# MiniMax-AI/VTP

Hardware: AMD Instinct MI355X
Metric: images/sec/node VTP-B f16d64 256x256 train step (higher is better)
Workload: dtype bf16

## Files before the change

include/vtp_hip.h:

```cpp
#ifndef VTP_HIP_H
#define VTP_HIP_H
#ifdef __cplusplus
extern "C" {
#endif

#define VTP_ABI_VERSION 1

int vtp_abi_version(void);
const char* vtp_last_error(void);

enum { VTP_EPI_BF16 = 0, VTP_EPI_F32 = 1, VTP_EPI_SWIGLU = 2, VTP_EPI_GELU = 3, VTP_EPI_F32_ATOMIC = 4, VTP_EPI_F32_SLAB = 5,
       VTP_EPI_QUICK_GELU = 8 };
int vtp_gemm_splits(int K, int splits);
int vtp_gemm_tn_splits(int M, int N, int K);
int vtp_gemm_tn(const void* A, int lda, const void* B, int ldb, void* C, int ldc, int ldc2, const float* resid, int M, int N,
                int K, int epilogue, int a_grp, int a_pre, int b_grp, int b_pre, int c_grp, int c_pre, int splits,
                float* a_colsum, void* stream);
int vtp_gemm_tn_grouped(const void* probs, int nprob, int ntiles, int K, int splits, void* part, void* ticket, void* stream);
int vtp_gemm_tn_grouped_items(const void* probs, int nprob, int ntiles, int K, const void* items, int nitems, int slots, void* part,
                              void* ticket, void* stream);
int vtp_set_gemm_tuning(int force_cfg, int xcd_swizzle);
int vtp_set_gemm_dynamic(int on);
int vtp_gemm_debug(void* timing, int grid_limit, int delay_ticks);
int vtp_cu_thief(int nwg, int ticks, void* out, void* stream);
int vtp_attn_debug(void* timing, int lds_pad, int waves_per_wg, int stagger_ticks);
int vtp_gemm_nt_config(int M, int N, int K, int epilogue);
int vtp_gemm_nt(const void* A, int lda, const void* B, int ldb, void* C, int ldc, void* C2, int ldc2,
                const float* bias, const float* gamma, const float* resid, int M, int N, int K, int epilogue,
                int a_grp, int a_pre, int c_grp, int c_pre, int splits, float alpha, void* stream);

int vtp_gemm_qkv_rope(const void* A, int lda, const void* W, int ldb, const float* bias, void* C, int ldc, int M, int N, int K,
                      const int* rope_pos, const void* rope_sin, const void* rope_cos, int rope_cols, void* stream);

int vtp_gather_image_rows(const float* src, const int* img_idx, float* dst, void* dst_bf16, int n_img, long N, int D, float scale,
                          void* stream);
int vtp_scatter_image_rows(const float* src, const int* img_idx, float* dst, int n_img, long N, int D, float alpha, int accumulate,
                           void* stream);
int vtp_layerscale_wgrad(const float* G, const float* W, const float* bias, const float* colsum, const float* gamma, float* dW,
                         float* db, float* dgamma, int N, int K, void* stream);
int vtp_scaled_transpose(const float* W, const float* gamma, void* dstT, int N, int K, void* stream);
int vtp_qk_norm_fwd(const void* qkv, const float* wq, const float* wk, void* out, float* inv, long M, int D, float eps, void* stream);
int vtp_qk_norm_bwd(void* dqkv, const void* qkv, const float* inv, const float* wq, const float* wk, float* dwq, float* dwk, long M, int D,
                    void* stream);

int vtp_norm_fwd(const float* x, const float* w, const float* b, void* y, float* stats, int M, int D, float eps,
                 int kind, void* stream);
int vtp_norm_bwd(const void* dy, const float* x, const float* w, const float* stats, const float* dres, float* dx,
                 void* dx_bf16, float* dw, float* db, float* dx_colsum, int M, int D, int kind, void* stream);
int vtp_norm_bwd_pvec(const void* dy, const float* x, const float* w, const float* stats, const float* dres, float* dx,
                      void* dx_bf16, float* dw, float* db, float* dx_colsum, const float* pvec, int prow0, int pB, int pN, int M,
                      int D, int kind, void* stream);
int vtp_pool_patch_rows(const void* x, float* out, int B, int N, int D, float scale, void* stream);

int vtp_rope_qk(void* qkv, const void* sin, const void* cos, int B, int N, int heads, int prefix, int inverse,
                void* stream);

int vtp_attn_fwd(const void* q, const void* k, const void* v, void* o, float* lse, int B, int N, int heads,
                 long sb_qkv, long sn_qkv, long sb_o, long sn_o, float scale, int causal, void* stream);
int vtp_attn_bwd(const void* q, const void* k, const void* v, const void* o, const void* d_o, const float* lse,
                 float* delta, void* dq, void* dk, void* dv, const void* rope_sin, const void* rope_cos, int rope_prefix,
                 int B, int N, int heads, long sb_qkv, long sn_qkv, long sb_o, long sn_o, float scale, int causal,
                 void* stream);

int vtp_im2col16(const float* img, void* patches, int B, int H, int W, void* stream);
int vtp_im2col16_rows(const float* img, void* rows, int B, int H, int W, int prefix, void* stream);
int vtp_col2im16(const float* dpatches, float* dimg, int B, int H, int W, void* stream);

int vtp_assemble_tokens(float* x, const float* cls, const float* mask_token, const unsigned char* masks, int B, int N,
                        int D, void* stream);

int vtp_transpose_bf16(const void* in, int ld_in, void* out, int ld_out, float* colsum, int colsum_swiglu_h, int in_grp,
                       int in_pre, int R, int C, void* stream);
int vtp_colsum_bf16(const void* in, int ld, float* out, int colsum_swiglu_h, int in_grp, int in_pre, int R, int C, void* stream);
int vtp_colsum_bf16_rows(const void* in, int ld, float* out, const int* n_rows_dev, int R_max, int C, void* stream);
int vtp_mask_rows_bwd(const float* dx, void* dx_bf16, const unsigned char* masks, float* d_mask_token, int B, int N, int D,
                      void* stream);
int vtp_token_rows_bwd(const float* dx, void* dx_bf16, const unsigned char* masks, float* d_mask_token, float* d_cls_token, int B, int N,
                       int D, void* stream);
int vtp_strided_rowsum(const float* in, long stride, float* out, int B, int D, void* stream);

int vtp_cast_f32_bf16(const float* in, void* out, long n, void* stream);
int vtp_cast_transpose_f32_bf16(const float* in, void* out, int R, int C, void* stream);
int vtp_prep_weights(const void* descs, int n, int total_tiles, void* stream);
int vtp_prep_weights_range(const void* descs, int n, int tile_base, int n_tiles, void* stream);

int vtp_swiglu_bwd(const void* dh, const void* x12, void* dx12, float* db12, int M, int H, void* stream);
int vtp_gemm_dgrad_swiglu(const void* A, int lda, const void* WT, int ldb, const void* x12, int ldx, void* dx12, int ldc, int M, int H,
                          int K, void* stream);
int vtp_gelu_bwd(const void* dy, const void* pre, void* dx, long n, void* stream);
int vtp_quick_gelu_bwd(const void* dy, const void* pre, void* dx, long n, void* stream);

int vtp_pixel_shuffle16(const void* t, float* img, int B, int h, int w, void* stream);
int vtp_pixel_unshuffle16(const float* d_img, void* dt, int B, int h, int w, void* stream);
int vtp_l1_loss_fwd_bwd(const void* t, const float* target, void* dt, float* loss_sum, int B, int h, int w,
                        float gscale, void* stream);

int vtp_adamw(float* p, const float* g, float* m, float* v, void* p_bf16, long n, float lr, float beta1, float beta2,
              float eps, float weight_decay, int step, float grad_scale, void* stream);
int vtp_adamw_dev(float* p, const float* g, float* m, float* v, void* p_bf16, long n, const float* hyper, void* stream);
int vtp_adamw_dev_masked(float* p, const float* g, float* m, float* v, void* p_bf16, const void* nodecay4, long n, const float* hyper,
                         void* stream);
int vtp_reduce_slabs(const float* slabs, long stride, int S, float* dst, long n, int accumulate, void* stream);
int vtp_ema(float* t, const float* s, long n, float momentum, void* stream);
int vtp_ema_dev(float* t, const float* s, long n, const float* momentum , void* stream);
int vtp_adamw_ema_dev(float* p, const float* g, float* m, float* v, float* teacher, const void* nodecay4, long n, const float* hyper,
                      void* stream);
int vtp_adamw_dev_grouped(float* p, const float* g, float* m, float* v, void* p_bf16, const void* group4, const float* group_tab,
                          int ngroups, long n, const float* hyper, void* stream);
int vtp_adamw_ema_dev_grouped(float* p, const float* g, float* m, float* v, float* teacher, const void* group4, const float* group_tab,
                              int ngroups, long n, const float* hyper, void* stream);
int vtp_sumsq_partials_count(long n);
int vtp_sumsq_partials(const float* g, long n, double* partials, void* stream);
int vtp_sum_partials(const double* partials, int count, double* sum, void* stream);
int vtp_grad_clip_finalize(const double* partials, int count, float* hyper, float* total_norm, float* coef, void* stream);
int vtp_grad_clip_finalize_guarded(const double* partials, int count, float* hyper, float* total_norm, float* coef, int* state,
                                   const double* betas, void* stream);
int vtp_adamw_dev_guarded(float* p, const float* g, float* m, float* v, void* p_bf16, const void* idx4, const float* group_tab,
                          int ngroups, long n, const float* hyper, const int* skip, void* stream);
int vtp_adamw_ema_dev_guarded(float* p, const float* g, float* m, float* v, float* teacher, const void* idx4, const float* group_tab,
                              int ngroups, long n, const float* hyper, const int* skip, void* stream);
int vtp_ema_dev_guarded(float* t, const float* s, long n, const float* momentum, const int* skip, void* stream);

int vtp_embed_tokens(const long* ids, const float* table, const float* pos, float* x, int* eot, int B, int T, int D,
                     void* stream);
int vtp_embed_tokens_bwd(const long* ids, const float* dx, float* d_table, float* d_pos, int B, int T, int D, void* stream);
int vtp_gather_rows(const float* x, const int* idx, float* out, int B, int T, int D, void* stream);
int vtp_scatter_rows(const float* dy, const int* idx, float* dx, void* dx_bf16, int B, int T, int D, void* stream);
int vtp_l2norm_fwd(const float* x, float* y, float* inv_norm, int B, int D, float eps, void* stream);
int vtp_l2norm_bwd(const float* dy, const float* y, const float* inv_norm, float* dx, int B, int D, void* stream);
int vtp_clip_loss(const float* img_local, const float* txt_local, const float* img_all, const float* txt_all,
                  const float* logit_scale, int B_local, int B_all, int D, int label_offset, float* loss_sum,
                  float* d_img_local, float* d_txt_local, float* d_img_all, float* d_txt_all, float* d_logit_scale,
                  float* scratch, void* stream);

int vtp_clip_logits(const float* A, const float* B, const float* logit_scale, float* logits, int M, int N, int D, void* stream);
int vtp_clip_grad_rows(const float* G, const float* B, const float* logit_scale, float* out, int M, int N, int D, int accumulate,
                       void* stream);
int vtp_clip_grad_cols(const float* G, const float* A, const float* logit_scale, float* out, int M, int N, int D, int accumulate,
                       void* stream);
int vtp_siglip_pairs(float* logits, const float* logit_bias, int B_local, int B_all, int label_offset, float weight,
                     float* loss_sum, float* d_logit_scale, float* d_logit_bias, void* stream);
int vtp_koleo(const float* xn, int* nn_scratch, float* d_xn, float* loss_sum, int B, int D, float weight, float eps, void* stream);
int vtp_sinkhorn_knopp(const void* logits, float inv_temp, void* probs, float* u, float* v, float* scratch, int T, int K, float count,
                       const float* count_dev, const int* n_rows_dev, int n_iters, int phase, void* stream);

int vtp_norm_fwd_e4m3(const float* x, const float* w, const float* b, void* y8, const float* q_scale, float* stats, int M, int D,
                      float eps, int kind, void* stream);
int vtp_quantize_e4m3(const void* src, int src_is_f32, void* dst, long n, const float* scale_dev, float scale, void* stream);
int vtp_amax(const void* src, int src_is_f32, long n, float* amax, void* stream);
int vtp_dequantize_e4m3(const void* src, float* dst, long n, float inv_scale, void* stream);
int vtp_gemm_nt_fp8(const void* A8, int lda, const void* B8, int ldb, void* C, int ldc, void* C2, int ldc2, const float* bias,
                    const float* resid, int M, int N, int K, int epilogue, float alpha, const int* rope_pos, const void* rope_sin,
                    const void* rope_cos, int rope_cols, void* stream);

int vtp_u8_to_images(const void* u8_nhwc, float* img_nchw, long B, int H, int W, const float* mean3, const float* std3, int flip,
                     void* stream);
int vtp_images_to_u8(const float* img_nchw, void* u8_nhwc, long B, int H, int W, const float* sub3, const float* div3, void* stream);
int vtp_latent_channel_stats(const float* latents, double* sums, long B, int C, int hw, void* stream);

int vtp_gather_token_rows(const void* src, const int* idx, void* dst, int T, int D, void* stream);
int vtp_scatter_token_rows(const void* d_dst, const int* idx, void* d_src, int T, int D, void* stream);
int vtp_weight_norm_prep(const float* v, const float* g, void* weff, void* weffT, float* inv_norm, int K, int C, void* stream);
int vtp_weight_norm_bwd(const float* dW, const float* v, const float* g, const float* inv_norm, float* dv, float* dg, int K, int C,
                        void* stream);
int vtp_softmax_center(const void* logits, const float* center, float inv_temp, void* probs, int T, int K, void* stream);
int vtp_softmax_center_dev(const void* logits, const float* center, const float* inv_temp, void* probs, int T, int K, void* stream);
int vtp_dino_ce(const void* student_logits, const void* teacher_probs, const int* t_idx0, const int* t_idx1,
                const float* row_weight, float inv_temp, float* loss_sum, void* d_student_logits, int T, int K, void* stream);
int vtp_center_ema(float* center, const float* col_sum, float inv_count, const float* count_ptr, float momentum, int K,
                   void* stream);

int vtp_conv3x3(const void* x, const void* w, const float* bias, void* y, const void* relu_mask, int NB, int H, int W, int Cin,
                int Cout, int taps, int mode, void* stream);
int vtp_lpips_unfold3(const void* tok, const float* img, void* out, int n, int H, int W, const float* shift, const float* scale,
                      void* stream);
int vtp_lpips_fold3_bwd(const void* dA, void* dt, int n, int H, int W, const float* scale, void* stream);
int vtp_maxpool2_fwd(const void* in, void* out, int NB, int H, int W, int C, void* stream);
int vtp_maxpool2_bwd(const void* Y, const void* dP, const void* tap, void* dY, int NB, int H, int W, int C, void* stream);
int vtp_lpips_tap(const void* f0, const void* f1, const float* w, float* val, void* df0, int n, int H, int W, int C,
                  float gscale, void* stream);

#ifdef __cplusplus
}
#endif
#endif
```

vtp_amd/_lib.py:

```python
import ctypes
import os
from ctypes import c_char_p, c_float, c_int, c_long, c_void_p

_HERE = os.path.dirname(os.path.abspath(__file__))
LIB_PATH = os.environ.get("VTP_HIP_LIB") or os.path.join(_HERE, "lib", "libvtp_hip.so")

_P, _I, _L, _F = c_void_p, c_int, c_long, c_float

SIGNATURES = {
    "vtp_gemm_nt": [_P, _I, _P, _I, _P, _I, _P, _I, _P, _P, _P, _I, _I, _I, _I, _I, _I, _I, _I, _I, _F, _P],
    "vtp_norm_fwd": [_P, _P, _P, _P, _P, _I, _I, _F, _I, _P],
    "vtp_norm_bwd": [_P, _P, _P, _P, _P, _P, _P, _P, _P, _P, _I, _I, _I, _P],
    "vtp_norm_bwd_pvec": [_P, _P, _P, _P, _P, _P, _P, _P, _P, _P, _P, _I, _I, _I, _I, _I, _I, _P],
    "vtp_pool_patch_rows": [_P, _P, _I, _I, _I, _F, _P],
    "vtp_rope_qk": [_P, _P, _P, _I, _I, _I, _I, _I, _P],
    "vtp_attn_fwd": [_P, _P, _P, _P, _P, _I, _I, _I, _L, _L, _L, _L, _F, _I, _P],
    "vtp_attn_bwd": [_P, _P, _P, _P, _P, _P, _P, _P, _P, _P, _P, _P, _I, _I, _I, _I, _L, _L, _L, _L, _F, _I, _P],
    "vtp_im2col16": [_P, _P, _I, _I, _I, _P],
    "vtp_im2col16_rows": [_P, _P, _I, _I, _I, _I, _P],
    "vtp_col2im16": [_P, _P, _I, _I, _I, _P],
    "vtp_assemble_tokens": [_P, _P, _P, _P, _I, _I, _I, _P],
    "vtp_transpose_bf16": [_P, _I, _P, _I, _P, _I, _I, _I, _I, _I, _P],
    "vtp_strided_rowsum": [_P, _L, _P, _I, _I, _P],
    "vtp_mask_rows_bwd": [_P, _P, _P, _P, _I, _I, _I, _P],
    "vtp_token_rows_bwd": [_P, _P, _P, _P, _P, _I, _I, _I, _P],
    "vtp_cast_f32_bf16": [_P, _P, _L, _P],
    "vtp_cast_transpose_f32_bf16": [_P, _P, _I, _I, _P],
    "vtp_prep_weights": [_P, _I, _I, _P],
    "vtp_prep_weights_range": [_P, _I, _I, _I, _P],
    "vtp_swiglu_bwd": [_P, _P, _P, _P, _I, _I, _P],
    "vtp_gemm_dgrad_swiglu": [_P, _I, _P, _I, _P, _I, _P, _I, _I, _I, _I, _P],
    "vtp_gelu_bwd": [_P, _P, _P, _L, _P],
    "vtp_quick_gelu_bwd": [_P, _P, _P, _L, _P],
    "vtp_pixel_shuffle16": [_P, _P, _I, _I, _I, _P],
    "vtp_pixel_unshuffle16": [_P, _P, _I, _I, _I, _P],
    "vtp_l1_loss_fwd_bwd": [_P, _P, _P, _P, _I, _I, _I, _F, _P],
    "vtp_adamw": [_P, _P, _P, _P, _P, _L, _F, _F, _F, _F, _F, _I, _F, _P],
    "vtp_adamw_dev": [_P, _P, _P, _P, _P, _L, _P, _P],
    "vtp_adamw_dev_masked": [_P, _P, _P, _P, _P, _P, _L, _P, _P],
    "vtp_reduce_slabs": [_P, _L, _I, _P, _L, _I, _P],
    "vtp_gemm_splits": [_I, _I],
    "vtp_gemm_tn_splits": [_I, _I, _I],
    "vtp_gemm_qkv_rope": [_P, _I, _P, _I, _P, _P, _I, _I, _I, _I, _P, _P, _P, _I, _P],
    "vtp_gemm_tn": [_P, _I, _P, _I, _P, _I, _I, _P, _I, _I, _I, _I, _I, _I, _I, _I, _I, _I, _I, _P, _P],
    "vtp_gemm_tn_grouped": [_P, _I, _I, _I, _I, _P, _P, _P],
    "vtp_gemm_tn_grouped_items": [_P, _I, _I, _I, _P, _I, _I, _P, _P, _P],
    "vtp_colsum_bf16": [_P, _I, _P, _I, _I, _I, _I, _I, _P],
    "vtp_colsum_bf16_rows": [_P, _I, _P, _P, _I, _I, _P],
    "vtp_gather_image_rows": [_P, _P, _P, _P, _I, _L, _I, _F, _P],
    "vtp_scatter_image_rows": [_P, _P, _P, _I, _L, _I, _F, _I, _P],
    "vtp_layerscale_wgrad": [_P, _P, _P, _P, _P, _P, _P, _P, _I, _I, _P],
    "vtp_scaled_transpose": [_P, _P, _P, _I, _I, _P],
    "vtp_qk_norm_fwd": [_P, _P, _P, _P, _P, _L, _I, _F, _P],
    "vtp_qk_norm_bwd": [_P, _P, _P, _P, _P, _P, _P, _L, _I, _P],
    "vtp_set_gemm_tuning": [_I, _I],
    "vtp_gemm_nt_config": [_I, _I, _I, _I],
    "vtp_gemm_debug": [_P, _I, _I],
    "vtp_attn_debug": [_P, _I, _I, _I],
    "vtp_cu_thief": [_I, _I, _P, _P],
    "vtp_set_gemm_dynamic": [_I],
    "vtp_norm_fwd_e4m3": [_P, _P, _P, _P, _P, _P, _I, _I, _F, _I, _P],
    "vtp_quantize_e4m3": [_P, _I, _P, _L, _P, _F, _P],
    "vtp_amax": [_P, _I, _L, _P, _P],
    "vtp_dequantize_e4m3": [_P, _P, _L, _F, _P],
    "vtp_gemm_nt_fp8": [_P, _I, _P, _I, _P, _I, _P, _I, _P, _P, _I, _I, _I, _I, _F, _P, _P, _P, _I, _P],
    "vtp_u8_to_images": [_P, _P, _L, _I, _I, _P, _P, _I, _P],
    "vtp_images_to_u8": [_P, _P, _L, _I, _I, _P, _P, _P],
    "vtp_latent_channel_stats": [_P, _P, _L, _I, _I, _P],
    "vtp_ema": [_P, _P, _L, _F, _P],
    "vtp_gather_token_rows": [_P, _P, _P, _I, _I, _P],
    "vtp_scatter_token_rows": [_P, _P, _P, _I, _I, _P],
    "vtp_weight_norm_prep": [_P, _P, _P, _P, _P, _I, _I, _P],
    "vtp_weight_norm_bwd": [_P, _P, _P, _P, _P, _P, _I, _I, _P],
    "vtp_softmax_center": [_P, _P, _F, _P, _I, _I, _P],
    "vtp_softmax_center_dev": [_P, _P, _P, _P, _I, _I, _P],
    "vtp_dino_ce": [_P, _P, _P, _P, _P, _F, _P, _P, _I, _I, _P],
    "vtp_center_ema": [_P, _P, _F, _P, _F, _I, _P],
    "vtp_conv3x3": [_P, _P, _P, _P, _P, _I, _I, _I, _I, _I, _I, _I, _P],
    "vtp_lpips_unfold3": [_P, _P, _P, _I, _I, _I, _P, _P, _P],
    "vtp_lpips_fold3_bwd": [_P, _P, _I, _I, _I, _P, _P],
    "vtp_maxpool2_fwd": [_P, _P, _I, _I, _I, _I, _P],
    "vtp_maxpool2_bwd": [_P, _P, _P, _P, _I, _I, _I, _I, _P],
    "vtp_lpips_tap": [_P, _P, _P, _P, _P, _I, _I, _I, _I, _F, _P],
    "vtp_ema_dev": [_P, _P, _L, _P, _P],
    "vtp_adamw_ema_dev": [_P, _P, _P, _P, _P, _P, _L, _P, _P],
    "vtp_adamw_dev_grouped": [_P, _P, _P, _P, _P, _P, _P, _I, _L, _P, _P],
    "vtp_adamw_ema_dev_grouped": [_P, _P, _P, _P, _P, _P, _P, _I, _L, _P, _P],
    "vtp_sumsq_partials_count": [_L],
    "vtp_sumsq_partials": [_P, _L, _P, _P],
    "vtp_sum_partials": [_P, _I, _P, _P],
    "vtp_grad_clip_finalize": [_P, _I, _P, _P, _P, _P],
    "vtp_grad_clip_finalize_guarded": [_P, _I, _P, _P, _P, _P, _P, _P],
    "vtp_adamw_dev_guarded": [_P, _P, _P, _P, _P, _P, _P, _I, _L, _P, _P, _P],
    "vtp_adamw_ema_dev_guarded": [_P, _P, _P, _P, _P, _P, _P, _I, _L, _P, _P, _P],
    "vtp_ema_dev_guarded": [_P, _P, _L, _P, _P, _P],
    "vtp_embed_tokens": [_P, _P, _P, _P, _P, _I, _I, _I, _P],
    "vtp_embed_tokens_bwd": [_P, _P, _P, _P, _I, _I, _I, _P],
    "vtp_gather_rows": [_P, _P, _P, _I, _I, _I, _P],
    "vtp_scatter_rows": [_P, _P, _P, _P, _I, _I, _I, _P],
    "vtp_l2norm_fwd": [_P, _P, _P, _I, _I, _F, _P],
    "vtp_l2norm_bwd": [_P, _P, _P, _P, _I, _I, _P],
    "vtp_clip_logits": [_P, _P, _P, _P, _I, _I, _I, _P],
    "vtp_clip_grad_rows": [_P, _P, _P, _P, _I, _I, _I, _I, _P],
    "vtp_clip_grad_cols": [_P, _P, _P, _P, _I, _I, _I, _I, _P],
    "vtp_siglip_pairs": [_P, _P, _I, _I, _I, _F, _P, _P, _P, _P],
    "vtp_koleo": [_P, _P, _P, _P, _I, _I, _F, _F, _P],
    "vtp_sinkhorn_knopp": [_P, _F, _P, _P, _P, _P, _I, _I, _F, _P, _P, _I, _I, _P],
    "vtp_clip_loss": [_P, _P, _P, _P, _P, _I, _I, _I, _I, _P, _P, _P, _P, _P, _P, _P, _P],
}

_lib = None


def load():
    global _lib
    if _lib is not None:
        return _lib
    if not os.path.exists(LIB_PATH):
        raise RuntimeError(
            f"vtp_amd: {LIB_PATH} not found. The HIP library is mandatory (there is no fallback path): "
            "run `python -c 'import __graft_entry__ as g; g.build()'` or `python vtp_amd/build.py`.")
    try:
        import torch
        if torch.cuda.is_available():
            torch.cuda.init()
    except ImportError:
        pass
    lib = ctypes.CDLL(LIB_PATH)
    lib.vtp_abi_version.restype = c_int
    lib.vtp_last_error.restype = c_char_p
    for name, args in SIGNATURES.items():
        fn = getattr(lib, name)
        fn.argtypes = args
        fn.restype = c_int
    if lib.vtp_abi_version() != 1:
        raise RuntimeError("vtp_amd: ABI version mismatch between vtp_amd/_lib.py and libvtp_hip.so")
    _lib = lib
    return lib


def check(rc: int, what: str):
    if rc != 0:
        msg = _lib.vtp_last_error().decode(errors="replace") if _lib is not None else ""
        raise RuntimeError(f"{what} failed (rc={rc}): {msg}")
```

vtp_amd/csrc/elementwise.hip:

```cpp
#include "common.h"
#include "vtp_hip.h"

namespace vtp {

template <bool INVERSE>
__global__ __launch_bounds__(256) void rope_qk_kernel(bf16* __restrict__ qkv, const bf16* __restrict__ sin_t,
                                                      const bf16* __restrict__ cos_t, int B, int N, int heads,
                                                      int prefix) {
  const int D = heads * 64;
  const long per_row = 2L * heads * 4;
  const long total = (long)B * N * per_row;
  for (long idx = blockIdx.x * 256L + threadIdx.x; idx < total; idx += (long)gridDim.x * 256L) {
    const long row = idx / per_row;
    const int rem = (int)(idx - row * per_row);
    const int n = (int)(row % N);
    if (n < prefix) continue;
    const int part = rem / (heads * 4);
    const int h = (rem / 4) % heads;
    const int g = rem & 3;
    bf16* p = qkv + row * (3L * D) + (long)part * D + h * 64 + g * 8;
    const long t = (long)(n - prefix) * 64 + g * 8;
    bf16x8 x1 = *(const bf16x8*)p, x2 = *(const bf16x8*)(p + 32);
    bf16x8 c1 = *(const bf16x8*)(cos_t + t), c2 = *(const bf16x8*)(cos_t + t + 32);
    bf16x8 s1 = *(const bf16x8*)(sin_t + t), s2 = *(const bf16x8*)(sin_t + t + 32);
// ... 79 lines not shown
        *(f32x4*)(img + ioff + 4 * q) = v;
      } else {
        f32x4 tg = *(const f32x4*)(target + ioff + 4 * q);
        f32x4 g;
#pragma unroll
        for (int e = 0; e < 4; ++e) {
          const float d = v[e] - tg[e];
          local += fabsf(d);
          g[e] = d > 0.f ? gscale : (d < 0.f ? -gscale : 0.f);
        }
        *(bf16x4*)(dt + toff + 4 * q) = __builtin_convertvector(g, bf16x4);
      }
    }
  }
  if (MODE == 1) {
    __shared__ float red[4];
    const float s = block_sum<4>(local, red);
    if (threadIdx.x == 0) unsafeAtomicAdd(loss_sum, s);
  }
}

__global__ __launch_bounds__(256) void assemble_tokens_kernel(float* __restrict__ x, const float* __restrict__ cls,
                                                              const float* __restrict__ mask_token,
                                                              const unsigned char* __restrict__ masks, int B, int N, int D) {
  const int d4 = D / 4;
  const long total = (long)B * N * d4;
  for (long idx = blockIdx.x * 256L + threadIdx.x; idx < total; idx += (long)gridDim.x * 256L) {
    const int c = (int)(idx % d4);
    const long row = idx / d4;
    const int n = (int)(row % N);
    const long b = row / N;
    if (n == 0) {
      *(f32x4*)(x + row * D + 4 * c) = *(const f32x4*)(cls + 4 * c);
    } else if (masks && masks[b * (N - 1) + (n - 1)]) {
      *(f32x4*)(x + row * D + 4 * c) = *(const f32x4*)(mask_token + 4 * c);
    }
  }
}

__global__ __launch_bounds__(256) void transpose_bf16_kernel(const bf16* __restrict__ in, int ld_in,
                                                             bf16* __restrict__ out, int ld_out,
                                                             float* __restrict__ colsum, int R, int C, int csum_H, int in_grp, int in_pre) {
  __shared__ bf16 tile[64][72];
  __shared__ float csum[64];
  const int r0 = blockIdx.y * 64, c0 = blockIdx.x * 64;
  const int tid = threadIdx.x;
  if (tid < 64) csum[tid] = 0.f;
  __syncthreads();
#pragma unroll
  for (int it = 0; it < 2; ++it) {
    const int chunk = tid + it * 256;
    const int r = chunk >> 3, cc = (chunk & 7) * 8;
    bf16x8 v;
    if (r0 + r < R && c0 + cc < C) {
      const int rr_ = r0 + r;
      const int rin = in_grp > 0 ? rr_ + (rr_ / in_grp + 1) * in_pre : rr_;
      v = *(const bf16x8*)(in + (size_t)rin * ld_in + c0 + cc);
    } else {
#pragma unroll
      for (int e = 0; e < 8; ++e) v[e] = (bf16)0.f;
    }
#pragma unroll
    for (int e = 0; e < 8; ++e) tile[cc + e][r] = v[e];
    if (colsum) {
#pragma unroll
      for (int e = 0; e < 8; ++e) {
        float s = bf2f(v[e]);
        s += __shfl_xor(s, 8, 64);
        s += __shfl_xor(s, 16, 64);
        s += __shfl_xor(s, 32, 64);
        if ((tid & 63) < 8) atomicAdd(&csum[cc + e], s);
      }
    }
  }
  __syncthreads();
#pragma unroll
  for (int it = 0; it < 2; ++it) {
    const int chunk = tid + it * 256;
    const int c = chunk >> 3, rr = (chunk & 7) * 8;
    if (c0 + c < C && r0 + rr < ld_out) {
      *(bf16x8*)(out + (size_t)(c0 + c) * ld_out + r0 + rr) = *(const bf16x8*)&tile[c][rr];
    }
  }
  if (colsum && tid < 64 && c0 + tid < C) {
    const int c = c0 + tid;
    const int dst = csum_H > 0 ? ((c >> 4) << 3) + (c & 7) + ((c & 8) ? csum_H : 0) : c;
    unsafeAtomicAdd(colsum + dst, csum[tid]);
  }
}

__global__ __launch_bounds__(256) void colsum_bf16_kernel(const bf16* __restrict__ in, int ld, float* __restrict__ out,
                                                          int R, int C, int csum_H, int in_grp, int in_pre,
                                                          const int* __restrict__ rows_dev) {
  __shared__ float part[32][65];
  if (rows_dev) R = min(R, rows_dev[0]);
  const int c0 = blockIdx.x * 64, r0 = blockIdx.y * 256;
  const int tid = threadIdx.x;
  const int cc = (tid & 7) * 8, rr = tid >> 3;
  float acc[8] = {0.f, 0.f, 0.f, 0.f, 0.f, 0.f, 0.f, 0.f};
  if (c0 + cc < C) {
#pragma unroll
    for (int k = 0; k < 8; ++k) {
      const int r = r0 + rr + 32 * k;
      if (r < R) {
        const int rin = in_grp > 0 ? r + (r / in_grp + 1) * in_pre : r;
        bf16x8 v = *(const bf16x8*)(in + (size_t)rin * ld + c0 + cc);
#pragma unroll
        for (int e = 0; e < 8; ++e) acc[e] += bf2f(v[e]);
      }
    }
  }
#pragma unroll
  for (int e = 0; e < 8; ++e) part[rr][cc + e] = acc[e];
  __syncthreads();
  if (tid < 64 && c0 + tid < C) {
    float s = 0.f;
#pragma unroll
    for (int k = 0; k < 32; ++k) s += part[k][tid];
    const int c = c0 + tid;
    const int dst = csum_H > 0 ? ((c >> 4) << 3) + (c & 7) + ((c & 8) ? csum_H : 0) : c;
    unsafeAtomicAdd(out + dst, s);
  }
}

__global__ __launch_bounds__(256) void cast_f32_bf16_kernel(const float* __restrict__ in, bf16* __restrict__ out, long n) {
  const long n4 = n / 4;
  for (long i = blockIdx.x * 256L + threadIdx.x; i < n4; i += (long)gridDim.x * 256L)
    *(bf16x4*)(out + 4 * i) = __builtin_convertvector(*(const f32x4*)(in + 4 * i), bf16x4);
  if (blockIdx.x == 0 && threadIdx.x < (n & 3)) out[n4 * 4 + threadIdx.x] = f2bf(in[n4 * 4 + threadIdx.x]);
}

__global__ __launch_bounds__(256) void cast_transpose_kernel(const float* __restrict__ in, bf16* __restrict__ out, int R, int C) {
  __shared__ float tile[64][65];
  const int r0 = blockIdx.y * 64, c0 = blockIdx.x * 64;
  const int tx = threadIdx.x & 63, ty = threadIdx.x >> 6;
  for (int r = ty; r < 64; r += 4)
    tile[r][tx] = (r0 + r < R && c0 + tx < C) ? in[(size_t)(r0 + r) * C + c0 + tx] : 0.f;
  __syncthreads();
  for (int c = ty; c < 64; c += 4)
    if (c0 + c < C && r0 + tx < R) out[(size_t)(c0 + c) * R + r0 + tx] = f2bf(tile[tx][c]);
}


struct PrepDesc {
  const float* src;
  const float* src2;
  void* dst;
  void* dstT;
  long R, C;
  long mode;
  long tile_start;
};

__global__ __launch_bounds__(256) void prep_weights_kernel(const PrepDesc* __restrict__ descs, int n, int tile_base) {
  __shared__ float tile[64][65];
  const long tile_id = (long)blockIdx.x + tile_base;
  int lo = 0, hi = n - 1;
  while (lo < hi) {
    const int mid = (lo + hi + 1) >> 1;
    if (descs[mid].tile_start <= tile_id) lo = mid; else hi = mid - 1;
  }
  const PrepDesc d = descs[lo];
  const int t = (int)(tile_id - d.tile_start);
  const int R = (int)d.R, C = (int)d.C;
  if (d.mode == 2) {
    const int g = t * 256 + threadIdx.x;
    if (g < R) {
      const int j = (g >> 4) * 8 + (g & 7);
      ((float*)d.dst)[g] = (g & 8) ? d.src2[j] : d.src[j];
    }
    return;
  }
  const int tiles_c = (C + 63) / 64;
  const int r0 = (t / tiles_c) * 64, c0 = (t % tiles_c) * 64;
  bf16* dst = (bf16*)d.dst;
  bf16* dstT = (bf16*)d.dstT;
  const bool aligned = ((((uintptr_t)d.src | (uintptr_t)d.src2) & 15) | (((uintptr_t)dst | (uintptr_t)dstT) & 7)) == 0;
  if ((C & 3) == 0 && (R & 3) == 0 && aligned) {
    const int q = threadIdx.x & 15, rr = threadIdx.x >> 4;
#pragma unroll
    for (int pass = 0; pass < 4; ++pass) {
      const int r = pass * 16 + rr, g = r0 + r, c = c0 + 4 * q;
      f32x4 v = {0.f, 0.f, 0.f, 0.f};
      if (g < R && c < C) {
        const float* src = d.src;
        int j = g;
        if (d.mode == 1) {
          j = (g >> 4) * 8 + (g & 7);
          src = (g & 8) ? d.src2 : d.src;
        }
        v = *(const f32x4*)(src + (size_t)j * C + c);
        if (dst) *(bf16x4*)(dst + (size_t)g * C + c) = __builtin_convertvector(v, bf16x4);
      }
#pragma unroll
      for (int e = 0; e < 4; ++e) tile[r][4 * q + e] = v[e];
    }
    if (!dstT) return;
    __syncthreads();
#pragma unroll
    for (int pass = 0; pass < 4; ++pass) {
      const int c = pass * 16 + rr, r = 4 * q;
      if (c0 + c < C && r0 + r < R) {
        const f32x4 v = {tile[r][c], tile[r + 1][c], tile[r + 2][c], tile[r + 3][c]};
        *(bf16x4*)(dstT + (size_t)(c0 + c) * R + r0 + r) = __builtin_convertvector(v, bf16x4);
      }
    }
    return;
  }
  const int tx = threadIdx.x & 63, ty = threadIdx.x >> 6;
  for (int r = ty; r < 64; r += 4) {
    float v = 0.f;
    const int g = r0 + r;
    if (g < R && c0 + tx < C) {
      if (d.mode == 1) {
        const int j = (g >> 4) * 8 + (g & 7);
        v = ((g & 8) ? d.src2 : d.src)[(size_t)j * C + c0 + tx];
      } else {
        v = d.src[(size_t)g * C + c0 + tx];
      }
      if (dst) dst[(size_t)g * C + c0 + tx] = f2bf(v);
    }
    tile[r][tx] = v;
  }
  if (!dstT) return;
  __syncthreads();
  for (int c = ty; c < 64; c += 4)
    if (c0 + c < C && r0 + tx < R) dstT[(size_t)(c0 + c) * R + r0 + tx] = f2bf(tile[tx][c]);
}

__global__ __launch_bounds__(256) void swiglu_bwd_kernel(const bf16* __restrict__ dh, const bf16* __restrict__ x12,
                                                         bf16* __restrict__ dx12, int M, int H) {
  const int g8 = H / 8;
  const long total = (long)M * g8;
  for (long idx = blockIdx.x * 256L + threadIdx.x; idx < total; idx += (long)gridDim.x * 256L) {
    const int g = (int)(idx % g8);
    const long m = idx / g8;
    bf16x8 d = *(const bf16x8*)(dh + m * H + 8 * g);
    bf16x8 x1 = *(const bf16x8*)(x12 + m * 2L * H + 16 * g);
    bf16x8 x2 = *(const bf16x8*)(x12 + m * 2L * H + 16 * g + 8);
    bf16x8 o1, o2;
    swiglu_bwd8(x1, x2, d, o1, o2);
    *(bf16x8*)(dx12 + m * 2L * H + 16 * g) = o1;
    *(bf16x8*)(dx12 + m * 2L * H + 16 * g + 8) = o2;
  }
}

__global__ __launch_bounds__(256) void swiglu_bwd_rows_kernel(const bf16* __restrict__ dh, const bf16* __restrict__ x12,
                                                              bf16* __restrict__ dx12, float* __restrict__ db12, int M, int H) {
  __shared__ float red[4][64 * 16];
  const int lane = threadIdx.x & 63, wv = threadIdx.x >> 6;
  const int g = blockIdx.y * 64 + lane;
  const bool live = g < H / 8;
  float s1[8], s2[8];
#pragma unroll
  for (int e = 0; e < 8; ++e) s1[e] = s2[e] = 0.f;
  const int step = gridDim.x * 4;
  if (live) {
    for (int m0 = blockIdx.x * 4 + wv; m0 < M; m0 += 2 * step) {
      bf16x8 d[2], x1[2], x2[2];
#pragma unroll
      for (int r = 0; r < 2; ++r) {
        const long m = min(m0 + r * step, M - 1);
        d[r] = *(const bf16x8*)(dh + m * H + 8 * g);
        x1[r] = *(const bf16x8*)(x12 + m * 2L * H + 16 * g);
        x2[r] = *(const bf16x8*)(x12 + m * 2L * H + 16 * g + 8);
      }
#pragma unroll
      for (int r = 0; r < 2; ++r) {
        const long m = m0 + r * step;
        if (m >= M) break;
        bf16x8 o1, o2;
        swiglu_bwd8(x1[r], x2[r], d[r], o1, o2);
#pragma unroll
        for (int e = 0; e < 8; ++e) {
          s1[e] += bf2f(o1[e]);
          s2[e] += bf2f(o2[e]);
        }
        *(bf16x8*)(dx12 + m * 2L * H + 16 * g) = o1;
        *(bf16x8*)(dx12 + m * 2L * H + 16 * g + 8) = o2;
      }
    }
  }
#pragma unroll
  for (int e = 0; e < 8; ++e) {
    red[wv][lane * 16 + e] = s1[e];
    red[wv][lane * 16 + 8 + e] = s2[e];
  }
  __syncthreads();
  for (int i = threadIdx.x; i < 64 * 16; i += 256) {
    const int l = i >> 4, e = i & 15, gg = blockIdx.y * 64 + l;
    if (gg < H / 8) {
      const float t = red[0][i] + red[1][i] + red[2][i] + red[3][i];
      unsafeAtomicAdd(db12 + (e < 8 ? 8 * gg + e : H + 8 * gg + e - 8), t);
    }
  }
}

template <bool QUICK>
__global__ __launch_bounds__(256) void gelu_bwd_kernel(const bf16* __restrict__ dy, const bf16* __restrict__ pre,
                                                       bf16* __restrict__ dx, long n) {
  const long n8 = n / 8;
  for (long i = blockIdx.x * 256L + threadIdx.x; i < n8; i += (long)gridDim.x * 256L) {
    bf16x8 g = *(const bf16x8*)(dy + 8 * i), p = *(const bf16x8*)(pre + 8 * i), o;
#pragma unroll
    for (int e = 0; e < 8; ++e) o[e] = f2bf(bf2f(g[e]) * (QUICK ? quick_gelu_grad(bf2f(p[e])) : gelu_erf_grad(bf2f(p[e]))));
    *(bf16x8*)(dx + 8 * i) = o;
  }
}

__device__ __forceinline__ float2 fold_group_row(float2 row, float lr, float wd, float bc1) {
  const float lr_g = lr * row.x, wd_g = wd * row.y;
  return make_float2(1.f - lr_g * wd_g, lr_g / bc1);
}

template <bool TABLE>
__global__ __launch_bounds__(256) void adamw_kernel(float* __restrict__ p, const float* __restrict__ g,
                                                    float* __restrict__ m, float* __restrict__ v,
                                                    bf16* __restrict__ pb, long n, float lr, float b1, float b2, float eps,
                                                    float wd, float bc1, float bc2_sqrt, float gs,
                                                    const float* __restrict__ hyper, const uint8_t* __restrict__ idx4,
                                                    const float2* __restrict__ group_tab, int ngroups,
                                                    const int* __restrict__ skip) {
  __shared__ float2 tab[TABLE ? 256 : 1];
  if (skip && *skip) return;
  if (TABLE || hyper) {
    lr = hyper[0]; b1 = hyper[1]; b2 = hyper[2]; eps = hyper[3]; wd = hyper[4]; bc1 = hyper[5]; bc2_sqrt = hyper[6]; gs = hyper[7];
  }
  if constexpr (TABLE) {
    if ((int)threadIdx.x < ngroups) tab[threadIdx.x] = fold_group_row(group_tab[threadIdx.x], lr, wd, bc1);
    __syncthreads();
  }
  const long n4 = n / 4;
  for (long i = blockIdx.x * 256L + threadIdx.x; i < n4; i += (long)gridDim.x * 256L) {
    f32x4 pv = *(const f32x4*)(p + 4 * i), gv = *(const f32x4*)(g + 4 * i);
    f32x4 mv = *(const f32x4*)(m + 4 * i), vv = *(const f32x4*)(v + 4 * i);
    float keep, step;
    if constexpr (TABLE) {
      const float2 row = tab[min((int)idx4[i], ngroups - 1)];
      keep = row.x, step = row.y;
    } else {
      keep = (idx4 && idx4[i]) ? 1.f : 1.f - lr * wd, step = lr / bc1;
    }
#pragma unroll
    for (int e = 0; e < 4; ++e) {
      const float gg = gv[e] * gs;
      pv[e] *= keep;
      mv[e] = b1 * mv[e] + (1.f - b1) * gg;
      vv[e] = b2 * vv[e] + (1.f - b2) * gg * gg;
      const float denom = sqrtf(vv[e]) / bc2_sqrt + eps;
      pv[e] -= step * (mv[e] / denom);
    }
    *(f32x4*)(p + 4 * i) = pv;
    *(f32x4*)(m + 4 * i) = mv;
    *(f32x4*)(v + 4 * i) = vv;
    if (pb) *(bf16x4*)(pb + 4 * i) = __builtin_convertvector(pv, bf16x4);
  }
}

__global__ __launch_bounds__(256) void reduce_slabs_kernel(const float* __restrict__ slabs, long stride, int S,
                                                           float* __restrict__ dst, long n, int accumulate) {
  const long n4 = n / 4;
  for (long i = blockIdx.x * 256L + threadIdx.x; i < n4; i += (long)gridDim.x * 256L) {
    f32x4 a = accumulate ? *(const f32x4*)(dst + 4 * i) : (f32x4){0.f, 0.f, 0.f, 0.f};
    for (int s = 0; s < S; ++s) a += *(const f32x4*)(slabs + (long)s * stride + 4 * i);
    *(f32x4*)(dst + 4 * i) = a;
  }
}

__global__ __launch_bounds__(256) void ema_kernel(float* __restrict__ t, const float* __restrict__ s, long n, float mom,
                                                  const float* __restrict__ mom_ptr, const int* __restrict__ skip) {
  if (skip && *skip) return;
  if (mom_ptr) mom = mom_ptr[0];
  const long n4 = n / 4;
  for (long i = blockIdx.x * 256L + threadIdx.x; i < n4; i += (long)gridDim.x * 256L) {
    f32x4 tv = *(const f32x4*)(t + 4 * i), sv = *(const f32x4*)(s + 4 * i);
    *(f32x4*)(t + 4 * i) = tv * mom + sv * (1.f - mom);
  }
}

template <bool TABLE>
__global__ __launch_bounds__(256) void adamw_ema_kernel(float* __restrict__ p, const float* __restrict__ g, float* __restrict__ m,
                                                        float* __restrict__ v, float* __restrict__ t, long n4,
                                                        const float* __restrict__ hyper, const uint8_t* __restrict__ idx4,
                                                        const float2* __restrict__ group_tab, int ngroups,
                                                        const int* __restrict__ skip) {
  __shared__ float2 tab[TABLE ? 256 : 1];
  if (skip && *skip) return;
  const float lr = hyper[0], b1 = hyper[1], b2 = hyper[2], eps = hyper[3], wd = hyper[4], bc1 = hyper[5], bc2_sqrt = hyper[6], gs = hyper[7];
  const float mom = hyper[9];
  const long base = blockIdx.x * 1024L + threadIdx.x;
  float2 row = make_float2(1.f, 1.f);
  if constexpr (TABLE)
    if ((int)threadIdx.x < ngroups) row = group_tab[threadIdx.x];
  f32x4 pv[4], gv[4], mv[4], vv[4], tv[4];
  int gi[4];
  bool nd[4];
#pragma unroll
  for (int u = 0; u < 4; ++u) {
    const long i = base + u * 256;
    if (i < n4) {
      pv[u] = *(const f32x4*)(p + 4 * i);
      gv[u] = *(const f32x4*)(g + 4 * i);
      mv[u] = *(const f32x4*)(m + 4 * i);
      vv[u] = *(const f32x4*)(v + 4 * i);
      if (t) tv[u] = *(const f32x4*)(t + 4 * i);
      if constexpr (TABLE) gi[u] = idx4[i];
      else nd[u] = idx4 && idx4[i];
    }
  }
  if constexpr (TABLE) {
    if ((int)threadIdx.x < ngroups) tab[threadIdx.x] = fold_group_row(row, lr, wd, bc1);
    __syncthreads();
  }
#pragma unroll
  for (int u = 0; u < 4; ++u) {
    const long i = base + u * 256;
    if (i >= n4) continue;
    float keep, step;
    if constexpr (TABLE) {
      const float2 r = tab[min(gi[u], ngroups - 1)];
      keep = r.x, step = r.y;
    } else {
      keep = nd[u] ? 1.f : 1.f - lr * wd, step = lr / bc1;
    }
#pragma unroll
    for (int e = 0; e < 4; ++e) {
      const float gg = gv[u][e] * gs;
      pv[u][e] *= keep;
      mv[u][e] = b1 * mv[u][e] + (1.f - b1) * gg;
      vv[u][e] = b2 * vv[u][e] + (1.f - b2) * gg * gg;
      const float denom = sqrtf(vv[u][e]) / bc2_sqrt + eps;
      pv[u][e] -= step * (mv[u][e] / denom);
    }
    *(f32x4*)(p + 4 * i) = pv[u];
    *(f32x4*)(m + 4 * i) = mv[u];
    *(f32x4*)(v + 4 * i) = vv[u];
    if (t) *(f32x4*)(t + 4 * i) = tv[u] * mom + pv[u] * (1.f - mom);
  }
}

__global__ __launch_bounds__(256) void strided_rowsum_kernel(const float* __restrict__ in, long stride, float* __restrict__ out, int B, int D) {
  __shared__ float part[4][64];
  const int lane = threadIdx.x & 63, wave = threadIdx.x >> 6;
  const int d = blockIdx.x * 64 + lane;
  float s = 0.f;
  if (d < D)
    for (int b = wave; b < B; b += 4) s += in[(long)b * stride + d];
  part[wave][lane] = s;
  __syncthreads();
  if (wave == 0 && d < D) out[d] += (part[0][lane] + part[1][lane]) + (part[2][lane] + part[3][lane]);
}

__global__ __launch_bounds__(256) void token_rows_bwd_kernel(const float* __restrict__ dx, bf16* __restrict__ dxb,
                                                             const unsigned char* __restrict__ masks, float* __restrict__ d_mask,
                                                             float* __restrict__ d_cls, int B, int N, int D, int rpb) {
  extern __shared__ float part[];
  const int lane = threadIdx.x & 63, wave = threadIdx.x >> 6;
  const long rows = (long)B * N;
  const int rpw = (rpb + 3) >> 2;
  const long w0 = (long)blockIdx.x * rpb + (long)wave * rpw;
  long w1 = w0 + rpw;
  const long b1 = (long)(blockIdx.x + 1) * rpb;
  if (w1 > b1) w1 = b1;
  if (w1 > rows) w1 = rows;
  bool f_mask = false, f_cls = false;
  {
    const long r = w0 + lane;
    if (r < w1) {
      const int n = (int)(r % N);
      f_cls = d_cls != nullptr && n == 0;
      f_mask = masks != nullptr && n != 0 && masks[(r / N) * (N - 1) + (n - 1)] != 0;
    }
  }
  const unsigned long long hit[2] = {__ballot(f_mask), __ballot(f_cls)};
#pragma unroll
  for (int k = 0; k < 2; ++k) {
    float* out = part + (size_t)k * 4 * D + (size_t)wave * D;
    for (int d0 = 0; d0 < D; d0 += 1024) {
      float acc[16];
#pragma unroll
      for (int c = 0; c < 16; ++c) acc[c] = 0.f;
      unsigned long long m = hit[k];
      while (m) {
        const int i = __builtin_ctzll(m);
        m &= m - 1;
        const long o = (w0 + i) * D + d0 + lane;
        float v[16];
#pragma unroll
        for (int c = 0; c < 16; ++c) v[c] = (d0 + c * 64 + lane < D) ? dx[o + c * 64] : 0.f;
#pragma unroll
        for (int c = 0; c < 16; ++c) {
          acc[c] += v[c];
          if (d0 + c * 64 + lane < D) dxb[o + c * 64] = (bf16)0.f;
        }
      }
#pragma unroll
      for (int c = 0; c < 16; ++c)
        if (d0 + c * 64 + lane < D) out[d0 + c * 64 + lane] = acc[c];
    }
  }
  __syncthreads();
  const bool any_mask = __syncthreads_or(hit[0] != 0ull), any_cls = __syncthreads_or(hit[1] != 0ull);
  if (any_mask)
    for (int d = threadIdx.x; d < D; d += 256) unsafeAtomicAdd(d_mask + d, (part[d] + part[D + d]) + (part[2 * D + d] + part[3 * D + d]));
  if (any_cls) {
    const float* pc = part + (size_t)4 * D;
    for (int d = threadIdx.x; d < D; d += 256) unsafeAtomicAdd(d_cls + d, (pc[d] + pc[D + d]) + (pc[2 * D + d] + pc[3 * D + d]));
  }
}

static inline int grid_for(long items, int cap = 4096) {
  long b = (items + 255) / 256;
  if (b > cap) b = cap;
  if (b < 1) b = 1;
  return (int)b;
}

}
using namespace vtp;

extern "C" int vtp_rope_qk(void* qkv, const void* sin, const void* cos, int B, int N, int heads, int prefix,
                           int inverse, void* stream) {
  VTP_REQUIRE(qkv && sin && cos, "vtp_rope_qk: null pointer");
  VTP_REQUIRE(B > 0 && N > 0 && heads > 0 && prefix >= 0 && prefix <= N, "vtp_rope_qk: bad shape (prefix must be in [0,N])");
  const long items = (long)B * N * 2 * heads * 4;
  if (inverse)
    hipLaunchKernelGGL(rope_qk_kernel<true>, dim3(grid_for(items)), dim3(256), 0, (hipStream_t)stream, (bf16*)qkv,
                       (const bf16*)sin, (const bf16*)cos, B, N, heads, prefix);
  else
    hipLaunchKernelGGL(rope_qk_kernel<false>, dim3(grid_for(items)), dim3(256), 0, (hipStream_t)stream, (bf16*)qkv,
                       (const bf16*)sin, (const bf16*)cos, B, N, heads, prefix);
  return check_launch("rope_qk");
}

extern "C" int vtp_im2col16(const float* img, void* patches, int B, int H, int W, void* stream) {
  VTP_REQUIRE(img && patches, "vtp_im2col16: null pointer");
  VTP_REQUIRE(B > 0 && H > 0 && W > 0 && H % 16 == 0 && W % 16 == 0, "vtp_im2col16: H and W must be positive multiples of 16");
  const long items = (long)B * (H / 16) * (W / 16) * 48;
  hipLaunchKernelGGL(im2col16_kernel, dim3(grid_for(items)), dim3(256), 0, (hipStream_t)stream, img, (bf16*)patches, B, H, W, 0);
  return check_launch("im2col16");
}

extern "C" int vtp_im2col16_rows(const float* img, void* rows, int B, int H, int W, int prefix, void* stream) {
  VTP_REQUIRE(img && rows, "vtp_im2col16_rows: null pointer");
  VTP_REQUIRE(B > 0 && H > 0 && W > 0 && H % 16 == 0 && W % 16 == 0 && prefix >= 0, "vtp_im2col16_rows: H and W must be positive multiples of 16, prefix >= 0");
  const long items = (long)B * (H / 16) * (W / 16) * 48;
  hipLaunchKernelGGL(im2col16_kernel, dim3(grid_for(items)), dim3(256), 0, (hipStream_t)stream, img, (bf16*)rows, B, H, W, prefix);
  return check_launch("im2col16_rows");
}

extern "C" int vtp_col2im16(const float* dpatches, float* dimg, int B, int H, int W, void* stream) {
  VTP_REQUIRE(dpatches && dimg, "vtp_col2im16: null pointer");
  VTP_REQUIRE(B > 0 && H > 0 && W > 0 && H % 16 == 0 && W % 16 == 0, "vtp_col2im16: H and W must be positive multiples of 16");
  const long items = (long)B * (H / 16) * (W / 16) * 48;
  hipLaunchKernelGGL(col2im16_kernel, dim3(grid_for(items)), dim3(256), 0, (hipStream_t)stream, dpatches, dimg, B, H, W);
  return check_launch("col2im16");
}

extern "C" int vtp_assemble_tokens(float* x, const float* cls, const float* mask_token, const unsigned char* masks,
                                   int B, int N, int D, void* stream) {
  VTP_REQUIRE(x && cls, "vtp_assemble_tokens: null pointer");
  VTP_REQUIRE(!masks || mask_token, "vtp_assemble_tokens: masks given without mask_token");
  VTP_REQUIRE(B > 0 && N > 1 && D % 4 == 0, "vtp_assemble_tokens: bad shape");
  const long items = (long)B * N * (D / 4);
  hipLaunchKernelGGL(assemble_tokens_kernel, dim3(grid_for(items)), dim3(256), 0, (hipStream_t)stream, x, cls, mask_token, masks, B, N, D);
  return check_launch("assemble_tokens");
}

extern "C" int vtp_transpose_bf16(const void* in, int ld_in, void* out, int ld_out, float* colsum, int colsum_swiglu_h,
                                  int in_grp, int in_pre, int R, int C, void* stream) {
  VTP_REQUIRE(in && out, "vtp_transpose_bf16: null pointer");
  VTP_REQUIRE(R > 0 && C > 0 && C % 8 == 0 && ld_in % 8 == 0 && ld_out % 8 == 0 && ld_out >= R && ld_in >= C,
              "vtp_transpose_bf16: need C, ld_in, ld_out multiples of 8, ld_out >= R");
  dim3 grid(cdiv(C, 64), cdiv(ld_out, 64));
  hipLaunchKernelGGL(transpose_bf16_kernel, grid, dim3(256), 0, (hipStream_t)stream, (const bf16*)in, ld_in, (bf16*)out, ld_out, colsum, R, C, colsum_swiglu_h, in_grp, in_pre);
  return check_launch("transpose_bf16");
}

extern "C" int vtp_colsum_bf16(const void* in, int ld, float* out, int colsum_swiglu_h, int in_grp, int in_pre, int R, int C,
                               void* stream) {
  VTP_REQUIRE(in && out && R > 0 && C > 0 && C % 8 == 0 && ld % 8 == 0, "vtp_colsum_bf16: bad argument (C, ld %% 8 == 0)");
  hipLaunchKernelGGL(colsum_bf16_kernel, dim3(cdiv(C, 64), cdiv(R, 256)), dim3(256), 0, (hipStream_t)stream, (const bf16*)in, ld,
                     out, R, C, colsum_swiglu_h, in_grp, in_pre, (const int*)nullptr);
  return check_launch("colsum_bf16");
}

extern "C" int vtp_colsum_bf16_rows(const void* in, int ld, float* out, const int* n_rows_dev, int R_max, int C, void* stream) {
  VTP_REQUIRE(in && out && n_rows_dev && R_max > 0 && C > 0 && C % 8 == 0 && ld % 8 == 0, "vtp_colsum_bf16_rows: bad argument");
  hipLaunchKernelGGL(colsum_bf16_kernel, dim3(cdiv(C, 64), cdiv(R_max, 256)), dim3(256), 0, (hipStream_t)stream, (const bf16*)in,
                     ld, out, R_max, C, 0, 0, 0, n_rows_dev);
// ... 65 lines not shown
    hipLaunchKernelGGL(swiglu_bwd_rows_kernel, dim3(gx, gy), dim3(256), 0, (hipStream_t)stream, (const bf16*)dh,
                       (const bf16*)x12, (bf16*)dx12, db12, M, H);
  else
    hipLaunchKernelGGL(swiglu_bwd_kernel, dim3(grid_for((long)M * (H / 8))), dim3(256), 0, (hipStream_t)stream,
                       (const bf16*)dh, (const bf16*)x12, (bf16*)dx12, M, H);
  return check_launch("swiglu_bwd");
}

extern "C" int vtp_gelu_bwd(const void* dy, const void* pre, void* dx, long n, void* stream) {
  VTP_REQUIRE(dy && pre && dx && n > 0 && n % 8 == 0, "vtp_gelu_bwd: bad argument (n %% 8 == 0)");
  hipLaunchKernelGGL(gelu_bwd_kernel<false>, dim3(grid_for(n / 8)), dim3(256), 0, (hipStream_t)stream, (const bf16*)dy, (const bf16*)pre, (bf16*)dx, n);
  return check_launch("gelu_bwd");
}

extern "C" int vtp_quick_gelu_bwd(const void* dy, const void* pre, void* dx, long n, void* stream) {
  VTP_REQUIRE(dy && pre && dx && n > 0 && n % 8 == 0, "vtp_quick_gelu_bwd: bad argument (n %% 8 == 0)");
  hipLaunchKernelGGL(gelu_bwd_kernel<true>, dim3(grid_for(n / 8)), dim3(256), 0, (hipStream_t)stream, (const bf16*)dy, (const bf16*)pre, (bf16*)dx, n);
  return check_launch("quick_gelu_bwd");
}

extern "C" int vtp_pixel_shuffle16(const void* t, float* img, int B, int h, int w, void* stream) {
  VTP_REQUIRE(t && img && B > 0 && h > 0 && w > 0, "vtp_pixel_shuffle16: bad argument");
  hipLaunchKernelGGL(shuffle16_kernel<0>, dim3(grid_for((long)B * h * w * 48)), dim3(256), 0, (hipStream_t)stream,
                     (const bf16*)t, img, nullptr, nullptr, nullptr, B, h, w, 0.f);
  return check_launch("pixel_shuffle16");
}

extern "C" int vtp_pixel_unshuffle16(const float* d_img, void* dt, int B, int h, int w, void* stream) {
  VTP_REQUIRE(d_img && dt && B > 0 && h > 0 && w > 0, "vtp_pixel_unshuffle16: bad argument");
  hipLaunchKernelGGL(shuffle16_kernel<2>, dim3(grid_for((long)B * h * w * 48)), dim3(256), 0, (hipStream_t)stream,
                     (const bf16*)nullptr, const_cast<float*>(d_img), nullptr, (bf16*)dt, nullptr, B, h, w, 0.f);
  return check_launch("pixel_unshuffle16");
}

extern "C" int vtp_l1_loss_fwd_bwd(const void* t, const float* target, void* dt, float* loss_sum, int B, int h, int w,
                                   float gscale, void* stream) {
  VTP_REQUIRE(t && target && dt && loss_sum && B > 0 && h > 0 && w > 0, "vtp_l1_loss_fwd_bwd: bad argument");
  hipLaunchKernelGGL(shuffle16_kernel<1>, dim3(grid_for((long)B * h * w * 48, 1024)), dim3(256), 0, (hipStream_t)stream,
                     (const bf16*)t, nullptr, target, (bf16*)dt, loss_sum, B, h, w, gscale);
  return check_launch("l1_loss_fwd_bwd");
}

extern "C" int vtp_adamw(float* p, const float* g, float* m, float* v, void* p_bf16, long n, float lr, float beta1,
                         float beta2, float eps, float weight_decay, int step, float grad_scale, void* stream) {
  VTP_REQUIRE(p && g && m && v && n > 0 && n % 4 == 0 && step >= 1, "vtp_adamw: bad argument (n %% 4 == 0, step >= 1)");
  const float bc1 = 1.f - powf(beta1, (float)step);
  const float bc2s = sqrtf(1.f - powf(beta2, (float)step));
  hipLaunchKernelGGL(adamw_kernel<false>, dim3(grid_for(n / 4)), dim3(256), 0, (hipStream_t)stream, p, g, m, v, (bf16*)p_bf16, n, lr,
                     beta1, beta2, eps, weight_decay, bc1, bc2s, grad_scale, (const float*)nullptr, (const uint8_t*)nullptr,
                     (const float2*)nullptr, 0, (const int*)nullptr);
  return check_launch("adamw");
}

extern "C" int vtp_adamw_dev(float* p, const float* g, float* m, float* v, void* p_bf16, long n, const float* hyper,
                             void* stream) {
  VTP_REQUIRE(p && g && m && v && hyper && n > 0 && n % 4 == 0, "vtp_adamw_dev: bad argument (n %% 4 == 0)");
  hipLaunchKernelGGL(adamw_kernel<false>, dim3(grid_for(n / 4)), dim3(256), 0, (hipStream_t)stream, p, g, m, v, (bf16*)p_bf16, n, 0.f,
                     0.f, 0.f, 0.f, 0.f, 1.f, 1.f, 1.f, hyper, (const uint8_t*)nullptr, (const float2*)nullptr, 0, (const int*)nullptr);
  return check_launch("adamw_dev");
}

extern "C" int vtp_adamw_dev_masked(float* p, const float* g, float* m, float* v, void* p_bf16, const void* nodecay4, long n,
                                    const float* hyper, void* stream) {
  VTP_REQUIRE(p && g && m && v && hyper && nodecay4 && n > 0 && n % 4 == 0, "vtp_adamw_dev_masked: bad argument (n %% 4 == 0)");
  hipLaunchKernelGGL(adamw_kernel<false>, dim3(grid_for(n / 4)), dim3(256), 0, (hipStream_t)stream, p, g, m, v, (bf16*)p_bf16, n, 0.f,
                     0.f, 0.f, 0.f, 0.f, 1.f, 1.f, 1.f, hyper, (const uint8_t*)nodecay4, (const float2*)nullptr, 0, (const int*)nullptr);
  return check_launch("adamw_dev_masked");
}

extern "C" int vtp_reduce_slabs(const float* slabs, long stride, int S, float* dst, long n, int accumulate, void* stream) {
  VTP_REQUIRE(slabs && dst && S >= 1 && n > 0 && n % 4 == 0 && stride % 4 == 0, "vtp_reduce_slabs: bad argument (n, stride %% 4 == 0)");
  hipLaunchKernelGGL(reduce_slabs_kernel, dim3(grid_for(n / 4, 2048)), dim3(256), 0, (hipStream_t)stream, slabs, stride, S, dst, n, accumulate);
  return check_launch("reduce_slabs");
}

extern "C" int vtp_ema(float* t, const float* s, long n, float momentum, void* stream) {
  VTP_REQUIRE(t && s && n > 0 && n % 4 == 0, "vtp_ema: bad argument (n %% 4 == 0)");
  hipLaunchKernelGGL(ema_kernel, dim3(grid_for(n / 4)), dim3(256), 0, (hipStream_t)stream, t, s, n, momentum, (const float*)nullptr,
                     (const int*)nullptr);
  return check_launch("ema");
}

extern "C" int vtp_ema_dev(float* t, const float* s, long n, const float* momentum, void* stream) {
  VTP_REQUIRE(t && s && momentum && n > 0 && n % 4 == 0, "vtp_ema_dev: bad argument (n %% 4 == 0)");
  hipLaunchKernelGGL(ema_kernel, dim3(grid_for(n / 4)), dim3(256), 0, (hipStream_t)stream, t, s, n, 0.f, momentum,
                     (const int*)nullptr);
  return check_launch("ema_dev");
}

extern "C" int vtp_adamw_ema_dev(float* p, const float* g, float* m, float* v, float* teacher, const void* nodecay4, long n,
                                 const float* hyper, void* stream) {
  VTP_REQUIRE(p && g && m && v && hyper && n > 0 && n % 4 == 0, "vtp_adamw_ema_dev: bad argument (n %% 4 == 0)");
  VTP_REQUIRE(n / 4096 < 0x7fffffffL, "vtp_adamw_ema_dev: range too long for one launch");
  hipLaunchKernelGGL(adamw_ema_kernel<false>, dim3((unsigned)((n / 4 + 1023) / 1024)), dim3(256), 0, (hipStream_t)stream, p, g, m, v,
                     teacher, n / 4, hyper, (const uint8_t*)nodecay4, (const float2*)nullptr, 0, (const int*)nullptr);
  return check_launch("adamw_ema_dev");
}

extern "C" int vtp_adamw_dev_grouped(float* p, const float* g, float* m, float* v, void* p_bf16, const void* group4,
                                     const float* group_tab, int ngroups, long n, const float* hyper, void* stream) {
  VTP_REQUIRE(p && g && m && v && hyper && n > 0 && n % 4 == 0, "vtp_adamw_dev_grouped: bad argument (n %% 4 == 0)");
  VTP_REQUIRE(group4 && group_tab && ngroups >= 1 && ngroups <= 256, "vtp_adamw_dev_grouped: bad group table (1 <= ngroups <= 256)");
  hipLaunchKernelGGL(adamw_kernel<true>, dim3(grid_for(n / 4)), dim3(256), 0, (hipStream_t)stream, p, g, m, v, (bf16*)p_bf16, n, 0.f,
                     0.f, 0.f, 0.f, 0.f, 1.f, 1.f, 1.f, hyper, (const uint8_t*)group4, (const float2*)group_tab, ngroups, (const int*)nullptr);
  return check_launch("adamw_dev_grouped");
}

extern "C" int vtp_adamw_ema_dev_grouped(float* p, const float* g, float* m, float* v, float* teacher, const void* group4,
                                         const float* group_tab, int ngroups, long n, const float* hyper, void* stream) {
  VTP_REQUIRE(p && g && m && v && hyper && n > 0 && n % 4 == 0, "vtp_adamw_ema_dev_grouped: bad argument (n %% 4 == 0)");
  VTP_REQUIRE(group4 && group_tab && ngroups >= 1 && ngroups <= 256, "vtp_adamw_ema_dev_grouped: bad group table (1 <= ngroups <= 256)");
  VTP_REQUIRE(n / 4096 < 0x7fffffffL, "vtp_adamw_ema_dev_grouped: range too long for one launch");
  hipLaunchKernelGGL(adamw_ema_kernel<true>, dim3((unsigned)((n / 4 + 1023) / 1024)), dim3(256), 0, (hipStream_t)stream, p, g, m, v,
                     teacher, n / 4, hyper, (const uint8_t*)group4, (const float2*)group_tab, ngroups, (const int*)nullptr);
  return check_launch("adamw_ema_dev_grouped");
}

extern "C" int vtp_adamw_dev_guarded(float* p, const float* g, float* m, float* v, void* p_bf16, const void* idx4,
                                     const float* group_tab, int ngroups, long n, const float* hyper, const int* skip, void* stream) {
  VTP_REQUIRE(p && g && m && v && hyper && skip && n > 0 && n % 4 == 0, "vtp_adamw_dev_guarded: bad argument (n %% 4 == 0)");
  if (group_tab) {
    VTP_REQUIRE(idx4 && ngroups >= 1 && ngroups <= 256, "vtp_adamw_dev_guarded: bad group table (1 <= ngroups <= 256)");
    hipLaunchKernelGGL(adamw_kernel<true>, dim3(grid_for(n / 4)), dim3(256), 0, (hipStream_t)stream, p, g, m, v, (bf16*)p_bf16, n, 0.f,
                       0.f, 0.f, 0.f, 0.f, 1.f, 1.f, 1.f, hyper, (const uint8_t*)idx4, (const float2*)group_tab, ngroups, skip);
  } else {
    hipLaunchKernelGGL(adamw_kernel<false>, dim3(grid_for(n / 4)), dim3(256), 0, (hipStream_t)stream, p, g, m, v, (bf16*)p_bf16, n, 0.f,
                       0.f, 0.f, 0.f, 0.f, 1.f, 1.f, 1.f, hyper, (const uint8_t*)idx4, (const float2*)nullptr, 0, skip);
  }
  return check_launch("adamw_dev_guarded");
}

extern "C" int vtp_adamw_ema_dev_guarded(float* p, const float* g, float* m, float* v, float* teacher, const void* idx4,
                                         const float* group_tab, int ngroups, long n, const float* hyper, const int* skip,
                                         void* stream) {
  VTP_REQUIRE(p && g && m && v && hyper && skip && n > 0 && n % 4 == 0, "vtp_adamw_ema_dev_guarded: bad argument (n %% 4 == 0)");
  VTP_REQUIRE(n / 4096 < 0x7fffffffL, "vtp_adamw_ema_dev_guarded: range too long for one launch");
  const dim3 grid((unsigned)((n / 4 + 1023) / 1024));
  if (group_tab) {
    VTP_REQUIRE(idx4 && ngroups >= 1 && ngroups <= 256, "vtp_adamw_ema_dev_guarded: bad group table (1 <= ngroups <= 256)");
    hipLaunchKernelGGL(adamw_ema_kernel<true>, grid, dim3(256), 0, (hipStream_t)stream, p, g, m, v, teacher, n / 4, hyper,
                       (const uint8_t*)idx4, (const float2*)group_tab, ngroups, skip);
  } else {
    hipLaunchKernelGGL(adamw_ema_kernel<false>, grid, dim3(256), 0, (hipStream_t)stream, p, g, m, v, teacher, n / 4, hyper,
                       (const uint8_t*)idx4, (const float2*)nullptr, 0, skip);
  }
  return check_launch("adamw_ema_dev_guarded");
}

extern "C" int vtp_ema_dev_guarded(float* t, const float* s, long n, const float* momentum, const int* skip, void* stream) {
  VTP_REQUIRE(t && s && momentum && skip && n > 0 && n % 4 == 0, "vtp_ema_dev_guarded: bad argument (n %% 4 == 0)");
  hipLaunchKernelGGL(ema_kernel, dim3(grid_for(n / 4)), dim3(256), 0, (hipStream_t)stream, t, s, n, 0.f, momentum, skip);
  return check_launch("ema_dev_guarded");
}
```

vtp_amd/engine.py:

```python
from __future__ import annotations

import math
import os
from typing import Dict, List, NamedTuple, Optional, Tuple

import torch

from . import ops
from .ops import EPI_BF16, EPI_F32, EPI_F32_SLAB, EPI_GELU, EPI_SWIGLU


class Lin:
    __slots__ = ("N", "K", "w", "wT", "bias", "gw", "gb", "w32", "wTs")


class SwiGLULin:
    __slots__ = ("H", "K", "w12", "w12T", "b12", "gw1", "gb1")


def _flat_order(names: List[str]) -> List[str]:
    out, seen = [], set()
    for n in names:
        if n in seen:
            continue
        if n.endswith("mlp.w1.weight") or n.endswith("mlp.w1.bias"):
            sib = n.replace("mlp.w1.", "mlp.w2.")
            out += [n, sib]
            seen.update((n, sib))
        else:
            out.append(n)
            seen.add(n)
    return out


class ParamStore:
    def __init__(self, module: torch.nn.Module, device: torch.device):
        self.device = device
        params = dict(module.named_parameters())
        order = _flat_order(list(params.keys()))
        self.offsets: Dict[str, Tuple[int, int]] = {}
        off = 0
        for n in order:
            k = params[n].numel()
            self.offsets[n] = (off, k)
            off += (k + 3) // 4 * 4
        self.numel = off
        self.flat_p = torch.zeros(off, dtype=torch.float32, device=device)
        self.flat_g = torch.zeros(off, dtype=torch.float32, device=device)
        self.params = params
        with torch.no_grad():
            for n in order:
                o, k = self.offsets[n]
                prm = params[n]
                view = self.flat_p[o:o + k].view(prm.shape)
                view.copy_(prm.detach().to(device=device, dtype=torch.float32))
                prm.data = view
                prm.grad = self.flat_g[o:o + k].view(prm.shape)
        self._descs: List[List[int]] = []
        self._bf16_elems = 0
        self._bf16_allocs: List[Tuple[object, str, int, tuple]] = []
        self._f32_extra: List[Tuple[object, str, int]] = []
        self._desc_dev = None
        self._tiles = 0
        self._keep = []

    def p(self, name: str) -> torch.Tensor:
        o, k = self.offsets[name]
        return self.flat_p[o:o + k]

    def g(self, name: str) -> torch.Tensor:
        o, k = self.offsets[name]
        return self.flat_g[o:o + k]

    def has(self, name: str) -> bool:
        return name in self.offsets

    def _want_bf16(self, obj, attr, n_elems, shape):
        self._bf16_allocs.append((obj, attr, self._bf16_elems, shape))
        self._bf16_elems += (n_elems + 7) // 8 * 8

    def lin(self, wname: str, bname: Optional[str], N: int, K: int, need_T: bool = True) -> Lin:
        L = Lin()
        L.N, L.K = N, K
        assert self.offsets[wname][1] == N * K, (wname, N, K)
        L.bias = self.p(bname) if bname and self.has(bname) else None
        L.gw = self.g(wname)
        L.gb = self.g(bname) if bname and self.has(bname) else None
        L.wT = None
        L.w32, L.wTs = self.p(wname).view(N, K), None
        self._want_bf16(L, "w", N * K, (N, K))
        if need_T:
            self._want_bf16(L, "wT", N * K, (K, N))
        self._descs.append(["lin", L, wname, need_T])
        return L

    def swiglu(self, prefix: str, H: int, K: int) -> SwiGLULin:
        S = SwiGLULin()
        S.H, S.K = H, K
        o1, k1 = self.offsets[prefix + "w1.weight"]
        o2, _ = self.offsets[prefix + "w2.weight"]
        assert o2 == o1 + k1 and k1 == H * K
        ob1, kb1 = self.offsets[prefix + "w1.bias"]
        ob2, _ = self.offsets[prefix + "w2.bias"]
        assert ob2 == ob1 + kb1 and kb1 == H
        S.gw1 = self.flat_g[o1:o1 + 2 * k1]
        S.gb1 = self.flat_g[ob1:ob1 + 2 * H]
        self._want_bf16(S, "w12", 2 * H * K, (2 * H, K))
        self._want_bf16(S, "w12T", 2 * H * K, (K, 2 * H))
        self._descs.append(["swiglu", S, prefix])
        return S

    def finalize(self):
        self.flat_bf16 = torch.zeros(max(self._bf16_elems, 8), dtype=torch.bfloat16, device=self.device)
        for obj, attr, off, shape in self._bf16_allocs:
            n = shape[0] * shape[1]
            setattr(obj, attr, self.flat_bf16[off:off + n].view(shape))
        rows, tiles = [], 0
        self._desc_src = []

        def add(src, src2, dst, dstT, R, C, mode, name):
            nonlocal tiles
            rows.append([src, src2, dst, dstT, R, C, mode, tiles])
            self._desc_src.append(self.offsets[name][0])
            tiles += (R + 255) // 256 if mode == 2 else ((R + 63) // 64) * ((C + 63) // 64)

        for d in self._descs:
            if d[0] == "lin":
                _, L, wname, need_T = d
                add(self.p(wname).data_ptr(), 0, L.w.data_ptr(), L.wT.data_ptr() if need_T else 0, L.N, L.K, 0, wname)
            else:
                _, S, prefix = d
                b12 = torch.zeros(2 * S.H, dtype=torch.float32, device=self.device)
                S.b12 = b12
                self._keep.append(b12)
                add(self.p(prefix + "w1.weight").data_ptr(), self.p(prefix + "w2.weight").data_ptr(), S.w12.data_ptr(),
                    S.w12T.data_ptr(), 2 * S.H, S.K, 1, prefix + "w1.weight")
                add(self.p(prefix + "w1.bias").data_ptr(), self.p(prefix + "w2.bias").data_ptr(), b12.data_ptr(), 0,
                    2 * S.H, 1, 2, prefix + "w1.bias")
        self._desc_dev = torch.tensor(rows, dtype=torch.int64, device=self.device)
        self._ndesc = len(rows)
        self._tiles = tiles
        self._desc_tile0 = [r[7] for r in rows] + [tiles]
        self.prep()

    def prep(self):
        ops.prep_weights(self._desc_dev, self._ndesc, self._tiles)
        for hook in getattr(self, "prep_hooks", ()):
            hook()
        self._prepped_version = self.flat_p._version

    def desc_runs(self, ranges):
        hit = [i for i, o in enumerate(self._desc_src) if any(lo <= o < hi for lo, hi in ranges)]
        runs = []
        for i in hit:
            if runs and runs[-1][1] == i:
                runs[-1][1] = i + 1
            else:
                runs.append([i, i + 1])
        return [tuple(r) for r in runs]

    def prep_runs(self, runs):
        for d0, d1 in runs:
            ops.prep_weights_range(self._desc_dev[d0:], d1 - d0, self._desc_tile0[d0], self._desc_tile0[d1] - self._desc_tile0[d0])

    def mark_prepped(self, done=()):
        for hook in getattr(self, "prep_hooks", ()):
            if hook not in done:
                hook()
        self._prepped_version = self.flat_p._version

    def ensure_fresh(self):
        if self.flat_p._version != self._prepped_version:
            self.prep()

    def zero_grad(self):
        self.flat_g.zero_()

    def sync_grad_views(self):
        for n, prm in self.params.items():
            if prm.grad is None and prm.requires_grad:
                o, k = self.offsets[n]
                view = self.flat_g[o:o + k].view(prm.shape)
                view.zero_()
                prm.grad = view


class Workspace:

    def __init__(self, device):
        self.device = device
        self._bufs: Dict[tuple, torch.Tensor] = {}

    def get(self, name: str, shape, dtype, zero: bool = False) -> torch.Tensor:
        key = (name, tuple(shape), dtype)
        t = self._bufs.get(key)
        if t is None:
            t = (torch.zeros if zero else torch.empty)(shape, dtype=dtype, device=self.device)
            self._bufs[key] = t
        return t

    def nbytes(self) -> int:
        return sum(t.numel() * t.element_size() for t in self._bufs.values())


BF, F32 = torch.bfloat16, torch.float32


def _env_flag(name: str, default: str = "1") -> bool:
    return os.environ.get(name, default) not in ("0", "false", "off")


class Overlap:

    enabled = _env_flag("VTP_OVERLAP")

    def __init__(self):
        self._sides = {}
        self._lane = 0
        self._deferred = []

    @property
    def side(self):
        return self._sides.get(self._lane)

    def _side(self):
        if self._lane not in self._sides:
            self._sides[self._lane] = torch.cuda.Stream()
        return self._sides[self._lane]

    def fork(self):
        self._side().wait_stream(torch.cuda.current_stream())

    def join(self):
        self.run_deferred()
        if self.side is not None:
            torch.cuda.current_stream().wait_stream(self.side)

    def defer(self, fn):
        self._deferred.append(fn)

    def run_deferred(self):
        while self._deferred:
            self._deferred.pop(0)()

    def lane(self, k: int):
        import contextlib

        @contextlib.contextmanager
        def ctx():
            prev, self._lane = self._lane, k
            try:
                yield
            finally:
                self._lane = prev
        return ctx()


OVERLAP = Overlap()


def linear_bwd(ws: Workspace, tag: str, L, dy_b, x_b, M: int, d_in, *, need_dx: bool = True, dy_remap=(0, 0),
               x_remap=(0, 0), dx_remap=(0, 0), gw=None, gb=None, N=None, K=None, wT=None, swiglu_h: int = 0,
               bias_grad_done: bool = False, ls=None, dgrad_swiglu=None, defer=None):
    if L is not None:
        N = L.N if N is None else N
        K = L.K if K is None else K
        gw = L.gw if gw is None else gw
        gb = L.gb if gb is None else gb
        wT = L.wT if wT is None else wT
    if ls is not None:
        gamma, g_gamma = ls
        assert L is not None and not swiglu_h and dy_remap == (0, 0) and x_remap == (0, 0)
        cs = ws.get("T.ls_cs", (N,), F32)
        cs.zero_()
        G = ws.get("T.ls_G", (N * K,), F32)

        def wgrad_ls():
            kw = dict(M=N, N=K, K=M, lda=dy_b.stride(0), ldb=x_b.stride(0), ldc=K, a_colsum=cs)
            St = ops.gemm_tn_splits(N, K, M)
            if St == 1:
                ops.gemm_tn(dy_b, x_b, G, epi=EPI_F32, **kw)
            else:
                slab = ws.get("T.slab", (St * N * K,), F32)
                ops.gemm_tn(dy_b, x_b, slab, ldc2=N * K // 4, epi=EPI_F32_SLAB, splits=St, **kw)
                ops.reduce_slabs(slab, N * K, St, G, N * K, accumulate=False)
            ops.layerscale_wgrad(G, L.w32, L.bias, cs, gamma, gw, gb, g_gamma, N, K)

        OVERLAP.join()
        wgrad_ls()
        if need_dx:
            ops.gemm_nt(dy_b, L.wTs, d_in, M=M, N=K, K=N, lda=dy_b.stride(0), ldb=N, ldc=d_in.stride(0), epi=EPI_BF16,
                        c_remap=dx_remap)
        return
    if bias_grad_done:
        gb = None
    c_remap = (-1, swiglu_h) if swiglu_h else (0, 0)

    def wgrad():
        if gb is not None:
            ops.colsum_bf16(dy_b, dy_b.stride(0), gb, M, N, swiglu_h=swiglu_h, in_remap=dy_remap)
        kw = dict(M=N, N=K, K=M, lda=dy_b.stride(0), ldb=x_b.stride(0), ldc=K, a_remap=dy_remap, b_remap=x_remap, c_remap=c_remap)
        St = ops.gemm_tn_splits(N, K, M)
        if St == 1:
            ops.gemm_tn(dy_b, x_b, gw, resid=gw, epi=EPI_F32, **kw)
        else:
            n_el = N * K
            slab = ws.get("T.slab", (St * n_el,), F32)
            ops.gemm_tn(dy_b, x_b, slab, ldc2=n_el // 4, epi=EPI_F32_SLAB, splits=St, **kw)
            ops.reduce_slabs(slab, n_el, St, gw, n_el, accumulate=True)

    if defer is not None:
        assert dy_remap == (0, 0) and x_remap == (0, 0)
        defer.append(dict(dy=dy_b, x=x_b, gw=gw, gb=gb, N=N, K=K, swiglu_h=swiglu_h))
    elif OVERLAP.enabled and need_dx:
        OVERLAP.join()
        OVERLAP.fork()
        with torch.cuda.stream(OVERLAP.side):
            wgrad()
    else:
        OVERLAP.join()
        wgrad()
    if need_dx and dgrad_swiglu is not None:
        assert dy_remap == (0, 0) and dx_remap == (0, 0)
        ops.gemm_dgrad_swiglu(dy_b, wT, dgrad_swiglu, d_in, M, K, N)
    elif need_dx:
        ops.gemm_nt(dy_b, wT, d_in, M=M, N=K, K=N, lda=dy_b.stride(0), ldb=N, ldc=d_in.stride(0), epi=EPI_BF16,
                    a_remap=dy_remap, c_remap=dx_remap)


class BlockW:
    pass


class BlockSaved(NamedTuple):
    attn_in: torch.Tensor
    xn1: torch.Tensor
    st1: torch.Tensor
    qkv: torch.Tensor
    o: torch.Tensor
    lse: torch.Tensor
    ffn_in: torch.Tensor
    xn2: torch.Tensor
    st2: torch.Tensor
    pre: torch.Tensor
    hid: torch.Tensor


ATTN_SCALE = 1.0 / math.sqrt(64.0)


_NAMES = {
    "vit": dict(n1="norm1", n2="norm2", qkv_w="attn.qkv.weight", qkv_b="attn.qkv.bias", proj_w="attn.proj.weight",
                proj_b="attn.proj.bias", ls1="ls1.gamma", ls2="ls2.gamma"),
    "text": dict(n1="ln_1", n2="ln_2", qkv_w="attn.in_proj_weight", qkv_b="attn.in_proj_bias",
                 proj_w="attn.out_proj.weight", proj_b="attn.out_proj.bias", ls1="ls_1.gamma", ls2="ls_2.gamma"),
}


class Stack:

    def __init__(self, store: ParamStore, prefix: str, depth: int, D: int, heads: int, H: int, norm: str,
                 style: str = "vit", ffn: str = "swiglu"):
        self.store, self.depth, self.D, self.heads, self.H, self.style = store, depth, D, heads, H, style
        self.swiglu = style == "vit" and ffn != "mlp"
        self.quick_gelu = False
        self.kind = ops.NORM_RMS if norm == "rmsnorm" else ops.NORM_LN
        if style == "text":
            self.eps = 1e-5
        else:
            self.eps = 1e-5 if norm == "rmsnorm" else 1e-6
        self.causal = style == "text"
        nm = _NAMES[style]
        self.blocks: List[BlockW] = []
        for i in range(depth):
            b = BlockW()
            pre = f"{prefix}{i}."
            b.n1w, b.gn1w = store.p(pre + nm["n1"] + ".weight"), store.g(pre + nm["n1"] + ".weight")
            b.n2w, b.gn2w = store.p(pre + nm["n2"] + ".weight"), store.g(pre + nm["n2"] + ".weight")
            if self.kind == ops.NORM_LN:
                b.n1b, b.gn1b = store.p(pre + nm["n1"] + ".bias"), store.g(pre + nm["n1"] + ".bias")
                b.n2b, b.gn2b = store.p(pre + nm["n2"] + ".bias"), store.g(pre + nm["n2"] + ".bias")
            else:
                b.n1b = b.gn1b = b.n2b = b.gn2b = None
            b.qkv = store.lin(pre + nm["qkv_w"], pre + nm["qkv_b"], 3 * D, D)
            b.proj = store.lin(pre + nm["proj_w"], pre + nm["proj_b"], D, D)
            if self.swiglu:
                b.w12 = store.swiglu(pre + "mlp.", H, D)
                b.w3 = store.lin(pre + "mlp.w3.weight", pre + "mlp.w3.bias", D, H)
            else:
                n1, n2 = ("fc1", "fc2") if style == "vit" else ("c_fc", "c_proj")
                b.fc = store.lin(f"{pre}mlp.{n1}.weight", f"{pre}mlp.{n1}.bias", H, D)
                b.w3 = store.lin(f"{pre}mlp.{n2}.weight", f"{pre}mlp.{n2}.bias", D, H)
            b.ls1 = store.p(pre + nm["ls1"]) if store.has(pre + nm["ls1"]) else None
            b.ls2 = store.p(pre + nm["ls2"]) if store.has(pre + nm["ls2"]) else None
            b.gls1 = store.g(pre + nm["ls1"]) if b.ls1 is not None else None
            b.gls2 = store.g(pre + nm["ls2"]) if b.ls2 is not None else None
            qn = pre + "attn.q_norm.weight"
            if store.has(qn):
                b.qn_w, b.kn_w = store.p(qn), store.p(pre + "attn.k_norm.weight")
                b.g_qn, b.g_kn = store.g(qn), store.g(pre + "attn.k_norm.weight")
            else:
                b.qn_w = b.kn_w = b.g_qn = b.g_kn = None
            for L, gam in ((b.proj, b.ls1), (b.w3, b.ls2)):
                if gam is not None:
                    L.wTs = torch.empty(L.K, L.N, dtype=BF, device=store.device)
                    if not hasattr(store, "prep_hooks"):
                        store.prep_hooks = []
                    store.prep_hooks.append(lambda L=L, gam=gam: ops.scaled_transpose(L.w32, gam, L.wTs, L.N, L.K))
            self.blocks.append(b)
        self.qk_norm = any(b.qn_w is not None for b in self.blocks)
        self.drop_plan = None
        self.wgrad_overwrite = False

    def _rope_plan(self, ws: Workspace, segs, prefix_tokens: int, M: int):
        if self.style != "vit" or all(rp is None for _, _, rp in segs) or (2 * self.D) % 128 or self.qk_norm:
            return None
        hit = getattr(ws, "_rope_plan", None)
        aug = [rp for _, _, rp in segs if isinstance(rp, RopeAugTabs)]
        key = tuple((b, n, None if rp is None else (rp.sin_all.data_ptr(), rp.off) if isinstance(rp, RopeAugTabs) else rp[0].data_ptr())
                    for b, n, rp in segs) + (prefix_tokens,)
        if hit is not None and hit[0] == key:
            return hit[1]
        pos, tabs_s, tabs_c, base = [], [], [], 0
        for Bs, Ns, rp in segs:
            if rp is None:
                pos.append(torch.full((Bs * Ns,), -1, dtype=torch.int32))
                continue
            hw = _rope_hw(rp)
            assert Ns - prefix_tokens == hw, (Ns, prefix_tokens, hw)
            if aug:
                assert isinstance(rp, RopeAugTabs) and rp.sin_all is aug[0].sin_all, "augmented and plain RoPE tables cannot be mixed in one pass"
                base = rp.off
            one = torch.cat([torch.full((prefix_tokens,), -1, dtype=torch.int32), torch.arange(hw, dtype=torch.int32) + base])
            pos.append(one.repeat(Bs))
            if not aug:
                tabs_s.append(rp[0])
                tabs_c.append(rp[1])
                base += hw
        dev = self.store.device
        if aug:
            plan = (torch.cat(pos).to(dev), aug[0].sin_all, aug[0].cos_all)
        else:
            plan = (torch.cat(pos).to(dev), torch.cat(tabs_s).contiguous(), torch.cat(tabs_c).contiguous())
        assert plan[0].numel() == M
        ws._rope_plan = (key, plan)
        return plan

    @staticmethod
    def _plan_tabs(plan, i: int):
        if plan[1].ndim == 3:
            i = min(i, plan[1].shape[0] - 1)
            return plan[1][i], plan[2][i]
        return plan[1], plan[2]

    @staticmethod
    def drop_allocation(b: int, ratio: float, world: int = 1, rank: int = 0):
        if world <= 1:
            keep = max(int(b * (1 - ratio)), 1)
            return keep, b / keep
        gb = b * world
        gkeep = max(int(gb * (1 - ratio)), world)
        base, extra = gkeep // world, gkeep % world
        alloc = [min(base + (1 if i < extra else 0), b) for i in range(world)]
        return alloc[rank], gb / max(sum(alloc), 1)

    def make_drop_plan(self, segs, ratio, generator: Optional[torch.Generator] = None, world: int = 1, rank: int = 0):
        ratios = list(ratio) if isinstance(ratio, (list, tuple)) else [ratio] * len(segs)
        assert len(ratios) == len(segs)
        keeps, scales = [], []
        for (B, _, _), r in zip(segs, ratios):
            k, sc = self.drop_allocation(B, r, world, rank)
            keeps.append(k)
            scales.append(sc)
        per = sum(keeps)
        idx = torch.empty(self.depth * 2 * per, dtype=torch.int32)
        o = 0
        for _ in range(self.depth * 2):
            for (B, _, _), k in zip(segs, keeps):
                idx[o:o + k] = torch.randperm(B, generator=generator)[:k].to(torch.int32)
                o += k
        return dict(idx=idx, keeps=keeps, scales=scales, per=per, ratio=ratio, batches=[B for B, _, _ in segs])

    def set_drop_plan(self, plan, ws_key="drop"):
        if plan is not None and self.style != "vit":
            raise NotImplementedError("stochastic depth is a property of the ViT blocks (block.py:207-289); the text tower has none")
        if plan is None:
            if self.drop_plan is not None:
                self.last_drop_plan = self.drop_plan
            self.drop_plan = None
            return
        bufs = self.__dict__.setdefault("_drop_bufs", {})
        n = plan["idx"].numel()
        buf = bufs.get(n)
        if buf is None:
            buf = bufs[n] = torch.empty(n, dtype=torch.int32, device=self.store.device)
        buf.copy_(plan["idx"], non_blocking=True)
        cur = dict(plan)
        cur["idx_dev"] = buf
        self.drop_plan = cur

    @staticmethod
    def _check_drop_plan(p, segs):
        got = [B for B, _, _ in segs]
        if p.get("batches") != got:
            raise RuntimeError(f"stochastic-depth plan drawn for item batch sizes {p.get('batches')} used on a pass with {got}")

    def _drop_idx(self, i: int, branch: int, s: int):
        p = self.drop_plan
        o = (i * 2 + branch) * p["per"] + sum(p["keeps"][:s])
        return p["idx_dev"][o:o + p["keeps"][s]]

    def _drop_segs(self, segs):
        self._check_drop_plan(self.drop_plan, segs)
        csegs = [(k, N, rp) for (_, N, rp), k in zip(segs, self.drop_plan["keeps"])]
        return csegs, sum(k * N for k, N, _ in csegs)

    def _gather(self, x, segs, csegs, i, branch, dst, dst_b, scale_by_seg):
        D = self.D
        r_full, r_c = 0, 0
        for s, ((B, N, _), (k, _, _)) in enumerate(zip(segs, csegs)):
            sc = scale_by_seg[s] if isinstance(scale_by_seg, (list, tuple)) else scale_by_seg
            ops.gather_image_rows(x[r_full:], self._drop_idx(i, branch, s), None if dst is None else dst[r_c:],
                                  None if dst_b is None else dst_b[r_c:], k, N, D, sc)
            r_full += B * N
            r_c += k * N

    def _scatter(self, src, x, segs, csegs, i, branch, alpha_by_seg, accumulate):
        D = self.D
        r_full, r_c = 0, 0
        for s, ((B, N, _), (k, _, _)) in enumerate(zip(segs, csegs)):
            al = alpha_by_seg[s] if isinstance(alpha_by_seg, (list, tuple)) else alpha_by_seg
            ops.scatter_image_rows(src[r_c:], self._drop_idx(i, branch, s), x[r_full:], k, N, D, al, accumulate)
            r_full += B * N
            r_c += k * N

    @staticmethod
    def _rows(segs):
        r0 = 0
        for B, N, rope in segs:
            yield r0, B, N, rope
            r0 += B * N

    @staticmethod
    def _attn_rows(segs):
        out = []
        for r0, B, N, rope in Stack._rows(segs):
            same = out and (out[-1][3] is rope or (isinstance(out[-1][3], tuple) and isinstance(rope, tuple)
                                                   and out[-1][3][0] is rope[0] and out[-1][3][1] is rope[1]))
            if out and out[-1][2] == N and same:
                out[-1] = (out[-1][0], out[-1][1] + B, N, rope)
            else:
                out.append((r0, B, N, rope))
        return out

    def _attention(self, qkv, o, lse, rows, i: int, prefix_tokens: int, rope_qk: bool):
        D, heads = self.D, self.heads
        for r0, Bs, Ns, rp in rows:
            q_s, o_s = qkv[r0:r0 + Bs * Ns], o[r0:r0 + Bs * Ns]
            if rp is not None and rope_qk:
                rs, rc = rope_at(rp, i)
                ops.rope_qk(q_s, rs, rc, Bs, Ns, heads, prefix_tokens)
            ops.attn_fwd(q_s, q_s[:, D:], q_s[:, 2 * D:], o_s, lse[r0 * heads:], Bs, Ns, heads, Ns * 3 * D, 3 * D, Ns * D, D,
                         ATTN_SCALE, self.causal)

    def _attn_fwd(self, ws: Workspace, t: str, i: int, x, out, resid, M: int, rows, prefix_tokens: int, rope_plan):
# ... 34 lines not shown
                 bias_done: bool = False, probs=None, dx_colsum=None):
        D, H, b = self.D, self.H, self.blocks[i]
        dh, dxn = ws.get(bt + "dh", (M, H), BF), ws.get(bt + "dxn", (M, D), BF)
        linear_bwd(ws, "w3", b.w3, dy_b, s.hid, M, dpre if fused else dh, bias_grad_done=bias_done,
                   ls=(b.ls2, b.gls2) if b.ls2 is not None else None, dgrad_swiglu=s.pre if fused else None, defer=probs)
        OVERLAP.run_deferred()
        if self.swiglu:
            if not fused:
                ops.swiglu_bwd(dh, s.pre, dpre, M, H)
            linear_bwd(ws, "w12", None, dpre, s.xn2, M, dxn, N=2 * H, K=D, gw=b.w12.gw1, gb=b.w12.gb1, wT=b.w12.w12T, swiglu_h=H,
                       defer=probs)
        else:
            ops.gelu_bwd(dh, s.pre, dpre, M * H, quick=self.quick_gelu)
            linear_bwd(ws, "fc", b.fc, dpre, s.xn2, M, dxn, defer=probs)
        ops.norm_bwd(dxn, s.ffn_in, b.n2w, s.st2, dy, dx, dx_b, b.gn2w, b.gn2b, M, D, self.kind, dx_colsum=dx_colsum)

    def _attn_bwd(self, ws: Workspace, t: str, i: int, s: BlockSaved, dy, dy_b, dx, dx_b, M: int, bt: str, dqkv, rows,
                  prefix_tokens: int, *, bias_done: bool = False, probs=None, join: bool = False, dx_colsum=None):
        D, heads, b = self.D, self.heads, self.blocks[i]
        d_o, dxn = ws.get(bt + "do", (M, D), BF), ws.get(bt + "dxn", (M, D), BF)
        delta = ws.get(bt + "delta", (M * heads,), F32)
        linear_bwd(ws, "proj", b.proj, dy_b, s.o, M, d_o, bias_grad_done=bias_done, ls=(b.ls1, b.gls1) if b.ls1 is not None else None,
                   defer=probs)
        for r0, Bs, Ns, rp in rows:
            r1 = r0 + Bs * Ns
            q_s, dq_s = s.qkv[r0:r1], dqkv[r0:r1]
            ops.attn_bwd(q_s, q_s[:, D:], q_s[:, 2 * D:], s.o[r0:r1], d_o[r0:r1], s.lse[r0 * heads:], delta[r0 * heads:], dq_s,
                         dq_s[:, D:], dq_s[:, 2 * D:], Bs, Ns, heads, Ns * 3 * D, 3 * D, Ns * D, D, ATTN_SCALE, self.causal,
                         rope=None if rp is None else rope_at(rp, i), rope_prefix=prefix_tokens)
        if b.qn_w is not None:
            ops.qk_norm_bwd(dqkv, ws.get(t + "qkv_pre", (M, 3 * D), BF), ws.get(t + "qinv", (M, 2 * heads), F32), b.qn_w, b.kn_w,
                            b.g_qn, b.g_kn, M, D)
        linear_bwd(ws, "qkv", b.qkv, dqkv, s.xn1, M, dxn, defer=probs)
        if join:
            OVERLAP.join()
        ops.norm_bwd(dxn, s.attn_in, b.n1w, s.st1, dy, dx, dx_b, b.gn1w, b.gn1b, M, D, self.kind, dx_colsum=dx_colsum)

    def forward(self, ws: Workspace, x, segs, prefix_tokens: int, train: bool):
        D = self.D
        M = sum(b * n for b, n, _ in segs)
        fp8 = getattr(self, "fp8", None)
        if fp8 is not None and fp8["ready"] and not train:
            return self._forward_fp8(ws, x, segs, prefix_tokens, M)
        calib = fp8["amax"] if (fp8 is not None and not fp8["ready"] and not train) else None
        drop = train and self.drop_plan is not None
        if drop:
            csegs, Mb = self._drop_segs(segs)
            rows, scales = list(self._rows(csegs)), self.drop_plan["scales"]
        else:
            csegs, Mb, rows = segs, M, self._attn_rows(segs)
        rope_plan = self._rope_plan(ws, csegs, prefix_tokens, Mb)
        saved_all = []
        for i in range(self.depth):
            if drop:
                t = f"{i}.d."
                x1, x2 = ws.get(t + "xs1", (Mb, D), F32), ws.get(t + "xs2", (Mb, D), F32)
                delta = ws.get("d.delta", (Mb, D), F32)
                self._gather(x, segs, csegs, i, 0, x1, None, 1.0)
                a = self._attn_fwd(ws, t, i, x1, delta, None, Mb, rows, prefix_tokens, rope_plan)
                self._scatter(delta, x, segs, csegs, i, 0, scales, accumulate=True)
                self._gather(x, segs, csegs, i, 1, x2, None, 1.0)
                f = self._ffn_fwd(ws, t, i, x2, delta, None, Mb, True)
                self._scatter(delta, x, segs, csegs, i, 1, scales, accumulate=True)
            else:
                t = f"{i}." if train else ""
                x1, x2 = x, ws.get(t + "xmid", (M, D), F32)
                xout = ws.get((f"{i}.xout" if train else f"xout{i & 1}"), (M, D), F32)
                a = self._attn_fwd(ws, t, i, x1, x2, x1, M, rows, prefix_tokens, rope_plan)
                f = self._ffn_fwd(ws, t, i, x2, xout, x2, M, train)
                if calib is not None:
                    for j, tns in enumerate((a[0], a[3], f[0], f[3])):
                        ops.amax(tns, calib[i, j:j + 1])
                x = xout
            if train:
                saved_all.append(BlockSaved(x1, *a, x2, *f))
        self.last_saved = saved_all
        return x

    def fp8_begin_calibration(self):
        if not self.swiglu or self.D % 16 or self.H % 16 or any(b.ls1 is not None or b.ls2 is not None for b in self.blocks):
            raise NotImplementedError("fp8 forward: SwiGLU ViT blocks with D, H multiples of 16, no LayerScale")
        dev = self.store.device
        self.fp8 = {"ready": False, "amax": torch.zeros(self.depth, 4, dtype=F32, device=dev)}

    def fp8_finalize(self):
        f, dev = self.fp8, self.store.device
        amax = f["amax"].clamp_min(1e-12)
        f["act_scale"] = (ops.E4M3_MAX / amax).contiguous()
        act_inv = (amax / ops.E4M3_MAX).cpu().tolist()
        f["w"], f["alpha"] = [], []
        for i, b in enumerate(self.blocks):
            ws8, al = [], []
            for j, w in enumerate((b.qkv.w, b.proj.w, b.w12.w12, b.w3.w)):
                wa = float(w.float().abs().max().clamp_min(1e-12))
                q = torch.empty(w.shape, dtype=torch.uint8, device=dev)
                ops.quantize_e4m3(w.contiguous(), q, ops.E4M3_MAX / wa)
                ws8.append(q)
                al.append(act_inv[i][j] * wa / ops.E4M3_MAX)
            f["w"].append(ws8)
            f["alpha"].append(al)
        f["ready"] = True

    def _forward_fp8(self, ws: Workspace, x, segs, prefix_tokens: int, M: int):
        D, H, heads, f = self.D, self.H, self.heads, self.fp8
        a8 = ws.get("f8.a", (M, max(D, H)), torch.uint8)
        qkv = ws.get("qkv", (M, 3 * D), BF)
        o = ws.get("o", (M, D), BF)
        lse = ws.get("lse", (M * heads,), F32)
        xmid = ws.get("xmid", (M, D), F32)
        hid = ws.get("hid", (M, H), BF)
        rope_plan = self._rope_plan(ws, segs, prefix_tokens, M)
        rope_arg = None if rope_plan is None else (rope_plan[0], rope_plan[1], rope_plan[2], 2 * D)
        rows = self._attn_rows(segs)
        for i, b in enumerate(self.blocks):
            w8, al, sc = f["w"][i], f["alpha"][i], f["act_scale"][i]
            xout = ws.get(f"xout{i & 1}", (M, D), F32)
            ops.norm_fwd_e4m3(x, b.n1w, b.n1b, a8, sc[0:1], None, M, D, self.eps, self.kind)
            if b.qn_w is not None:
                qkv_pre = ws.get("f8.qkv_pre", (M, 3 * D), BF)
                ops.gemm_nt_fp8(a8, w8[0], qkv_pre, M=M, N=3 * D, K=D, alpha=al[0], bias=b.qkv.bias, epi=EPI_BF16)
                ops.qk_norm_fwd(qkv_pre, b.qn_w, b.kn_w, qkv, ws.get("f8.qinv", (M, 2 * heads), F32), M, D)
            else:
                ops.gemm_nt_fp8(a8, w8[0], qkv, M=M, N=3 * D, K=D, alpha=al[0], bias=b.qkv.bias, epi=EPI_BF16, rope=rope_arg)
            self._attention(qkv, o, lse, rows, i, prefix_tokens, rope_arg is None)
            ops.quantize_e4m3(o, a8, sc[1:2])
            ops.gemm_nt_fp8(a8, w8[1], xmid, M=M, N=D, K=D, alpha=al[1], bias=b.proj.bias, resid=x, epi=EPI_F32)
            ops.norm_fwd_e4m3(xmid, b.n2w, b.n2b, a8, sc[2:3], None, M, D, self.eps, self.kind)
            ops.gemm_nt_fp8(a8, w8[2], hid, M=M, N=2 * H, K=D, alpha=al[2], bias=b.w12.b12, epi=EPI_SWIGLU)
            ops.quantize_e4m3(hid, a8, sc[3:4])
            ops.gemm_nt_fp8(a8, w8[3], xout, M=M, N=D, K=H, alpha=al[3], bias=b.w3.bias, resid=xmid, epi=EPI_F32)
            x = xout
        return x

    def w3_colsum_target(self, i: int):
        b = self.blocks[i]
        return b.w3.gb if (b.ls2 is None and self.drop_plan is None) else None

    def backward(self, ws: Workspace, dy, dy_b, segs, prefix_tokens: int, saved=None, dy_colsum_done: bool = False,
                 hold_last: bool = False, extra_last=None):
        D, H = self.D, self.H
        M = sum(b * n for b, n, _ in segs)
        saved = self.last_saved if saved is None else saved
        drop = self.drop_plan is not None
        if drop:
            csegs, Mb = self._drop_segs(segs)
            rows, scales, bt = list(self._rows(csegs)), self.drop_plan["scales"], "b.d."
            gdy, gdy_b = ws.get(bt + "gdy", (Mb, D), F32), ws.get(bt + "gdy_b", (Mb, D), BF)
            dxc = ws.get(bt + "dxc", (Mb, D), F32)
        else:
            Mb, rows, bt = M, self._attn_rows(segs), "b."
            dmid = ws.get("b.dmid", (M, D), F32)
        grouped = not drop and M >= 256 and all(b.ls1 is None and b.ls2 is None for b in self.blocks) \
            and ops.wgrad_group_fits(M, max(3 * D, 2 * H if self.swiglu else H)) and D % 8 == 0 and H % 8 == 0
        par = (lambda i: f".{i & 1}") if grouped else (lambda i: "")
        groups = ws.__dict__.setdefault("_wgrad_groups", {})
        scratch = self.__dict__.setdefault("_wgrad_scratch", {})
        pending = None

        def launch_pending():
            if pending is None:
                return
            if OVERLAP.enabled:
                OVERLAP.fork()
                side, grp = OVERLAP.side, pending[1]

                def issue():
                    with torch.cuda.stream(side):
                        grp.launch()
                OVERLAP.defer(issue)
            else:
                pending[1].launch()

        for i in range(self.depth - 1, -1, -1):
            b, s = self.blocks[i], saved[i]
            t = f"{i}.d." if drop else f"{i}."
            dpre = ws.get(bt + "dx12" + par(i), (Mb, 2 * H if self.swiglu else H), BF)
            dqkv = ws.get(bt + "dqkv" + par(i), (Mb, 3 * D), BF)
            if drop:
                self._gather(dy, segs, csegs, i, 1, gdy, gdy_b, scales)
                self._ffn_bwd(ws, i, s, gdy, gdy_b, dxc, None, Mb, bt, dpre, fused=False)
                self._scatter(dxc, dy, segs, csegs, i, 1, 1.0, accumulate=False)
                self._gather(dy, segs, csegs, i, 0, gdy, gdy_b, scales)
                self._attn_bwd(ws, t, i, s, gdy, gdy_b, dxc, None, Mb, bt, dqkv, rows, prefix_tokens)
                self._scatter(dxc, dy, segs, csegs, i, 0, 1.0, accumulate=False)
                OVERLAP.join()
                yield ("block", i)
                continue
            dxo = ws.get(f"b.dx{i & 1}", (M, D), F32)
            dxo_b = ws.get(f"b.dx_b{i & 1}", (M, D), BF)
            dmid_b = ws.get("b.dmid_b" + par(i), (M, D), BF)
            probs = [] if grouped else None
            if grouped:
                launch_pending()
            self._ffn_bwd(ws, i, s, dy, dy_b, dmid, dmid_b, M, bt, dpre, fused=self.swiglu and b.ls2 is None,
                          bias_done=dy_colsum_done if i == self.depth - 1 else self.w3_colsum_target(i) is not None, probs=probs,
                          dx_colsum=b.proj.gb if b.ls1 is None else None)
            self._attn_bwd(ws, t, i, s, dmid, dmid_b, dxo, dxo_b, M, bt, dqkv, rows, prefix_tokens, bias_done=b.proj.gb is not None,
                           probs=probs, join=grouped, dx_colsum=self.w3_colsum_target(i - 1) if i > 0 else None)
            dy, dy_b = dxo, dxo_b
            if not grouped:
                OVERLAP.join()
                yield ("block", i)
                continue
            extra = [dict(pr, dy=dy_b) for pr in extra_last] if (i == 0 and hold_last and extra_last) else []
            gkey = (i, bool(self.wgrad_overwrite), len(extra))
            grp = groups.get(gkey)
            if grp is None:
                grp = ops.WgradGroup(M)
                for pr in probs + extra:
                    grp.add(pr["dy"], pr["x"], pr["gw"], pr["gb"], pr["N"], pr["K"], pr["swiglu_h"], accumulate=not self.wgrad_overwrite)
                groups[gkey] = grp.finalize(self.store.device, scratch)
            if pending is not None:
                yield ("block", pending[0])
            pending = (i, grp)
        self.held = None
        if drop:
            ops.cast_f32_bf16(dy, dy_b, M * D)
        elif pending is not None and hold_last:
            OVERLAP.run_deferred()
            self.held = pending
        elif pending is not None:
            pending[1].launch()
            yield ("block", pending[0])
        return dy, dy_b


_ROPE_CACHE: Dict[tuple, Tuple[torch.Tensor, torch.Tensor]] = {}


def _rope_host(per: torch.Tensor, H: int, W: int, aug=None) -> Tuple[torch.Tensor, torch.Tensor]:
    dd = {"dtype": per.dtype}
    ch = torch.arange(0.5, H, **dd) / H
    cw = torch.arange(0.5, W, **dd) / W
    coords = torch.stack(torch.meshgrid(ch, cw, indexing="ij"), dim=-1).flatten(0, 1)
    coords = 2.0 * coords - 1.0
    if aug is not None:
        if aug.get("shift") is not None:
            coords += aug["shift"][None, :]
        if aug.get("jitter") is not None:
            coords *= aug["jitter"][None, :]
        if aug.get("rescale") is not None:
            coords *= aug["rescale"]
    ang = 2 * math.pi * coords[:, :, None] / per[None, None, :]
    ang = ang.flatten(1, 2).tile(2)
    return torch.sin(ang).to(torch.bfloat16).contiguous(), torch.cos(ang).to(torch.bfloat16).contiguous()


def rope_tables(periods: torch.Tensor, H: int, W: int, device) -> Tuple[torch.Tensor, torch.Tensor]:
    per = periods.detach().to("cpu")
    key = (H, W, str(device), per.dtype, tuple(per.float().tolist()))
    hit = _ROPE_CACHE.get(key)
    if hit is not None:
        return hit
    sin, cos = _rope_host(per, H, W)
    sin, cos = sin.to(device), cos.to(device)
    _ROPE_CACHE[key] = (sin, cos)
    return sin, cos


class RopeAugTabs:
    __slots__ = ("sin_all", "cos_all", "off", "hw")

    def __init__(self, sin_all, cos_all, off, hw):
        self.sin_all, self.cos_all, self.off, self.hw = sin_all, cos_all, off, hw

    def at(self, i: int):
        i = min(i, self.sin_all.shape[0] - 1)
        return self.sin_all[i, self.off:self.off + self.hw], self.cos_all[i, self.off:self.off + self.hw]


def rope_at(rp, i: int):
    return rp.at(i) if isinstance(rp, RopeAugTabs) else rp


def _rope_hw(rp) -> int:
    return rp.hw if isinstance(rp, RopeAugTabs) else rp[0].shape[0]


class RopeAugmenter:

    def __init__(self, periods: torch.Tensor, depth: int, per_block: bool, shift, jitter, rescale, seed: int = 0):
        self.per, self.depth, self.per_block = periods.detach().to("cpu"), depth, per_block
        self.cfg = (shift, jitter, rescale)
        self.engine_id = int(seed)
        self.gen = torch.Generator().manual_seed(int(seed))
        self.records: Dict[tuple, dict] = {}
        self.touched = set()
        self.last_draws = None

    def reseed(self, base_seed: int, rank: int = 0):
        self.gen.manual_seed((int(base_seed) * 1000003 + int(rank)) * 8 + self.engine_id)

    def get_state(self) -> torch.Tensor:
        return self.gen.get_state().clone()

    def set_state(self, state: torch.Tensor):
        self.gen.set_state(state.to("cpu", torch.uint8))

    @property
    def active(self) -> bool:
        return any(v is not None for v in self.cfg)

    def _draw(self):
        import numpy as np
        shift, jitter, rescale = self.cfg
        dd = {"dtype": self.per.dtype}
        d = {"shift": None, "jitter": None, "rescale": None}
        if shift is not None:
            d["shift"] = torch.empty(2, **dd).uniform_(-shift, shift, generator=self.gen)
        if jitter is not None:
            jm = float(np.log(jitter))
            d["jitter"] = torch.empty(2, **dd).uniform_(-jm, jm, generator=self.gen).exp()
        if rescale is not None:
            rm = float(np.log(rescale))
            d["rescale"] = torch.empty(1, **dd).uniform_(-rm, rm, generator=self.gen).exp()
        return d

    def record(self, key, hws, device):
        rec = self.records.get(key)
        if rec is None:
            P = sum(h * w for h, w in hws)
            nb = self.depth if self.per_block else 1
            rec = dict(hws=list(hws), sin=torch.zeros(nb, P, 64, dtype=torch.bfloat16, device=device),
                       cos=torch.zeros(nb, P, 64, dtype=torch.bfloat16, device=device),
                       host=torch.zeros(2, nb, P, 64, dtype=torch.bfloat16).pin_memory(), event=None, fresh=False)
            self.records[key] = rec
        return rec

    def refresh(self, rec):
        if rec["event"] is not None:
            rec["event"].synchronize()
        nb = rec["sin"].shape[0]
        draws = []
        for i in range(nb):
            row, off = [], 0
            for h, w in rec["hws"]:
                d = self._draw()
                sin, cos = _rope_host(self.per, h, w, d)
                rec["host"][0, i, off:off + h * w].copy_(sin)
                rec["host"][1, i, off:off + h * w].copy_(cos)
                off += h * w
                row.append(d)
            draws.append(row)
        rec["sin"].copy_(rec["host"][0], non_blocking=True)
        rec["cos"].copy_(rec["host"][1], non_blocking=True)
        ev = torch.cuda.Event()
        ev.record()
        rec["event"], rec["fresh"] = ev, True
        self.last_draws = draws

    def tables(self, key, hws, device):
        rec = self.record(key, hws, device)
        self.touched.add(key)
        if torch.cuda.is_current_stream_capturing():
            if not rec["fresh"]:
                raise RuntimeError("RoPE augmentation tables must exist before stream capture (run the step eagerly once)")
        else:
            self.refresh(rec)
        return rec

    def refresh_all(self, keys=None):
        for k, rec in self.records.items():
            if keys is None or k in keys:
                self.refresh(rec)
# ... 226 lines not shown
```

vtp_amd/ops.py:

```python
from __future__ import annotations

import torch

from . import _lib

EPI_BF16, EPI_F32, EPI_SWIGLU, EPI_GELU, EPI_F32_ATOMIC, EPI_F32_SLAB = 0, 1, 2, 3, 4, 5
EPI_QUICK_GELU = 8
NORM_RMS, NORM_LN = 0, 1


def _s():
    return torch.cuda.current_stream().cuda_stream


def _p(t):
    return 0 if t is None else t.data_ptr()


def _lib_():
    return _lib.load()


def pad8(n: int) -> int:
    return (n + 7) // 8 * 8
# ... 322 lines not shown


def embed_tokens_bwd(ids, dx, d_table, d_pos, B, T, D):
    _lib.check(_lib_().vtp_embed_tokens_bwd(_p(ids), _p(dx), _p(d_table), _p(d_pos), B, T, D, _s()), "vtp_embed_tokens_bwd")


def gather_rows(x, idx, out, B, T, D):
    _lib.check(_lib_().vtp_gather_rows(_p(x), _p(idx), _p(out), B, T, D, _s()), "vtp_gather_rows")


def scatter_rows(dy, idx, dx, dxb, B, T, D):
    _lib.check(_lib_().vtp_scatter_rows(_p(dy), _p(idx), _p(dx), _p(dxb), B, T, D, _s()), "vtp_scatter_rows")


def l2norm_fwd(x, y, inv, B, D, eps=1e-12):
    _lib.check(_lib_().vtp_l2norm_fwd(_p(x), _p(y), _p(inv), B, D, eps, _s()), "vtp_l2norm_fwd")


def l2norm_bwd(dy, y, inv, dx, B, D):
    _lib.check(_lib_().vtp_l2norm_bwd(_p(dy), _p(y), _p(inv), _p(dx), B, D, _s()), "vtp_l2norm_bwd")


def clip_loss(img_l, txt_l, img_all, txt_all, logit_scale, Bl, Bg, D, label_offset, loss_sum, d_img_l, d_txt_l, d_img_all,
              d_txt_all, d_logit_scale, scratch):
    _lib.check(_lib_().vtp_clip_loss(_p(img_l), _p(txt_l), _p(img_all), _p(txt_all), _p(logit_scale), Bl, Bg, D, label_offset,
                                     _p(loss_sum), _p(d_img_l), _p(d_txt_l), _p(d_img_all), _p(d_txt_all), _p(d_logit_scale),
                                     _p(scratch), _s()), "vtp_clip_loss")


def qk_norm_fwd(qkv, wq, wk, out, inv, M, D, eps=1e-5):
    _lib.check(_lib_().vtp_qk_norm_fwd(_p(qkv), _p(wq), _p(wk), _p(out), _p(inv), M, D, eps, _s()), "vtp_qk_norm_fwd")


def qk_norm_bwd(dqkv, qkv, inv, wq, wk, dwq, dwk, M, D):
    _lib.check(_lib_().vtp_qk_norm_bwd(_p(dqkv), _p(qkv), _p(inv), _p(wq), _p(wk), _p(dwq), _p(dwk), M, D, _s()), "vtp_qk_norm_bwd")


def gemm_dgrad_swiglu(dy, wT, x12, dx12, M, H, K):
    _lib.check(_lib_().vtp_gemm_dgrad_swiglu(_p(dy), dy.stride(0), _p(wT), wT.stride(0), _p(x12), x12.stride(0), _p(dx12), dx12.stride(0),
                                             M, H, K, _s()), "vtp_gemm_dgrad_swiglu")


def clip_logits(a, b, logit_scale, out, M, N, D):
    _lib.check(_lib_().vtp_clip_logits(_p(a), _p(b), _p(logit_scale), _p(out), M, N, D, _s()), "vtp_clip_logits")


def siglip_loss(img_l, txt_all, logit_scale, logit_bias, Bl, Bg, D, label_offset, loss_sum, d_img_l, d_txt_all, d_logit_scale,
                d_logit_bias, scratch):
    L, s = _lib_(), _s()
    _lib.check(L.vtp_clip_logits(_p(img_l), _p(txt_all), _p(logit_scale), _p(scratch), Bl, Bg, D, s), "vtp_clip_logits")
    _lib.check(L.vtp_siglip_pairs(_p(scratch), _p(logit_bias), Bl, Bg, label_offset, 1.0 / Bl, _p(loss_sum), _p(d_logit_scale),
                                  _p(d_logit_bias), s), "vtp_siglip_pairs")
    _lib.check(L.vtp_clip_grad_rows(_p(scratch), _p(txt_all), _p(logit_scale), _p(d_img_l), Bl, Bg, D, 0, s), "vtp_clip_grad_rows")
    _lib.check(L.vtp_clip_grad_cols(_p(scratch), _p(img_l), _p(logit_scale), _p(d_txt_all), Bl, Bg, D, 0, s), "vtp_clip_grad_cols")


def koleo(xn, nn_scratch, d_xn, loss_sum, B, D, weight, eps=1e-8):
    _lib.check(_lib_().vtp_koleo(_p(xn), _p(nn_scratch), _p(d_xn), _p(loss_sum), B, D, weight, eps, _s()), "vtp_koleo")


def sinkhorn_knopp(logits, inv_temp, probs, u, v, scratch, T, K, count, n_iters=3, phase=-1, count_dev=None, n_rows_dev=None):
    _lib.check(_lib_().vtp_sinkhorn_knopp(_p(logits), inv_temp, _p(probs), _p(u), _p(v), _p(scratch), T, K, float(count), _p(count_dev),
                                          _p(n_rows_dev), n_iters, phase, _s()), "vtp_sinkhorn_knopp")


def gather_token_rows(src, idx, dst, T, D):
    _lib.check(_lib_().vtp_gather_token_rows(_p(src), _p(idx), _p(dst), T, D, _s()), "vtp_gather_token_rows")


def scatter_token_rows(d_dst, idx, d_src, T, D):
    _lib.check(_lib_().vtp_scatter_token_rows(_p(d_dst), _p(idx), _p(d_src), T, D, _s()), "vtp_scatter_token_rows")


def weight_norm_prep(v, g, weff, weffT, inv_norm, K, C):
    _lib.check(_lib_().vtp_weight_norm_prep(_p(v), _p(g), _p(weff), _p(weffT), _p(inv_norm), K, C, _s()), "vtp_weight_norm_prep")


def weight_norm_bwd(dW, v, g, inv_norm, dv, dg, K, C):
    _lib.check(_lib_().vtp_weight_norm_bwd(_p(dW), _p(v), _p(g), _p(inv_norm), _p(dv), _p(dg), K, C, _s()), "vtp_weight_norm_bwd")


def softmax_center(logits, center, inv_temp, probs, T, K):
    if isinstance(inv_temp, torch.Tensor):
        _lib.check(_lib_().vtp_softmax_center_dev(_p(logits), _p(center), _p(inv_temp), _p(probs), T, K, _s()), "vtp_softmax_center_dev")
    else:
        _lib.check(_lib_().vtp_softmax_center(_p(logits), _p(center), inv_temp, _p(probs), T, K, _s()), "vtp_softmax_center")


def dino_ce(s_logits, t_probs, t0, t1, w, inv_temp, loss_sum, d_logits, T, K):
    _lib.check(_lib_().vtp_dino_ce(_p(s_logits), _p(t_probs), _p(t0), _p(t1), _p(w), inv_temp, _p(loss_sum), _p(d_logits), T, K,
                                   _s()), "vtp_dino_ce")


def center_ema(center, col_sum, inv_count, momentum, K, count=None):
    _lib.check(_lib_().vtp_center_ema(_p(center), _p(col_sum), inv_count, _p(count), momentum, K, _s()), "vtp_center_ema")


def ema_dev(t, s, n, momentum_dev):
    _lib.check(_lib_().vtp_ema_dev(_p(t), _p(s), n, _p(momentum_dev), _s()), "vtp_ema_dev")


def adamw_ema_dev(p, g, m, v, teacher, n, hyper, nodecay4=None):
    _lib.check(_lib_().vtp_adamw_ema_dev(_p(p), _p(g), _p(m), _p(v), _p(teacher), _p(nodecay4), n, _p(hyper), _s()), "vtp_adamw_ema_dev")



def adamw_dev_grouped(p, g, m, v, p_bf16, n, hyper, group4, group_tab, ngroups):
    _lib.check(_lib_().vtp_adamw_dev_grouped(_p(p), _p(g), _p(m), _p(v), _p(p_bf16), _p(group4), _p(group_tab), ngroups, n, _p(hyper),
                                             _s()), "vtp_adamw_dev_grouped")


def adamw_ema_dev_grouped(p, g, m, v, teacher, n, hyper, group4, group_tab, ngroups):
    _lib.check(_lib_().vtp_adamw_ema_dev_grouped(_p(p), _p(g), _p(m), _p(v), _p(teacher), _p(group4), _p(group_tab), ngroups, n,
                                                 _p(hyper), _s()), "vtp_adamw_ema_dev_grouped")


def sumsq_partials_count(n: int) -> int:
    return int(_lib_().vtp_sumsq_partials_count(n))


def sumsq_partials(g, n, partials):
    _lib.check(_lib_().vtp_sumsq_partials(_p(g), n, _p(partials), _s()), "vtp_sumsq_partials")


def sum_partials(partials, count, out):
    _lib.check(_lib_().vtp_sum_partials(_p(partials), count, _p(out), _s()), "vtp_sum_partials")


def grad_clip_finalize(partials, count, hyper, total_norm, coef):
    _lib.check(_lib_().vtp_grad_clip_finalize(_p(partials), count, _p(hyper), _p(total_norm), _p(coef), _s()), "vtp_grad_clip_finalize")


def grad_clip_finalize_guarded(partials, count, hyper, total_norm, coef, state, betas):
    import ctypes
    b = (ctypes.c_double * 2)(float(betas[0]), float(betas[1]))
    _lib.check(_lib_().vtp_grad_clip_finalize_guarded(_p(partials), count, _p(hyper), _p(total_norm), _p(coef), _p(state), b, _s()),
               "vtp_grad_clip_finalize_guarded")


def adamw_dev_guarded(p, g, m, v, p_bf16, n, hyper, skip, idx4=None, group_tab=None, ngroups=0):
    _lib.check(_lib_().vtp_adamw_dev_guarded(_p(p), _p(g), _p(m), _p(v), _p(p_bf16), _p(idx4), _p(group_tab), ngroups, n, _p(hyper),
                                             _p(skip), _s()), "vtp_adamw_dev_guarded")


def adamw_ema_dev_guarded(p, g, m, v, teacher, n, hyper, skip, idx4=None, group_tab=None, ngroups=0):
    _lib.check(_lib_().vtp_adamw_ema_dev_guarded(_p(p), _p(g), _p(m), _p(v), _p(teacher), _p(idx4), _p(group_tab), ngroups, n,
                                                 _p(hyper), _p(skip), _s()), "vtp_adamw_ema_dev_guarded")


def ema_dev_guarded(t, s, n, momentum_dev, skip):
    _lib.check(_lib_().vtp_ema_dev_guarded(_p(t), _p(s), n, _p(momentum_dev), _p(skip), _s()), "vtp_ema_dev_guarded")


def _f3(v):
    import ctypes
    return (ctypes.c_float * 3)(*[float(x) for x in v])


def conv3x3(x, w, bias, y, NB, H, W, Cin, Cout, taps=9, mode=0, relu_mask=None):
    _lib.check(_lib_().vtp_conv3x3(_p(x), _p(w), _p(bias), _p(y), _p(relu_mask), NB, H, W, Cin, Cout, taps, mode, _s()), "vtp_conv3x3")


def lpips_unfold3(tok, img, out, n, H, W, shift, scale):
    _lib.check(_lib_().vtp_lpips_unfold3(_p(tok), _p(img), _p(out), n, H, W, _f3(shift), _f3(scale), _s()), "vtp_lpips_unfold3")


def lpips_fold3_bwd(dA, dt, n, H, W, scale):
    _lib.check(_lib_().vtp_lpips_fold3_bwd(_p(dA), _p(dt), n, H, W, _f3(scale), _s()), "vtp_lpips_fold3_bwd")


def maxpool2_fwd(x, y, NB, H, W, C):
    _lib.check(_lib_().vtp_maxpool2_fwd(_p(x), _p(y), NB, H, W, C, _s()), "vtp_maxpool2_fwd")


def maxpool2_bwd(Y, dP, tap, dY, NB, H, W, C):
    _lib.check(_lib_().vtp_maxpool2_bwd(_p(Y), _p(dP), _p(tap), _p(dY), NB, H, W, C, _s()), "vtp_maxpool2_bwd")


def lpips_tap(f0, f1, w, val, df0, n, H, W, C, gscale):
    _lib.check(_lib_().vtp_lpips_tap(_p(f0), _p(f1), _p(w), _p(val), _p(df0), n, H, W, C, float(gscale), _s()), "vtp_lpips_tap")


def _f3(vals):
    import ctypes
    return (ctypes.c_float * 3)(*[float(v) for v in vals])


def u8_to_images(u8_nhwc, img_nchw, mean, std, flip=False):
    B, H, W, _ = u8_nhwc.shape
    m, s = _f3(mean), _f3(std)
    _lib.check(_lib_().vtp_u8_to_images(_p(u8_nhwc), _p(img_nchw), B, H, W, m, s, int(bool(flip)), _s()), "vtp_u8_to_images")


def images_to_u8(img_nchw, u8_nhwc, sub, div):
    B, _, H, W = img_nchw.shape
    a, d = _f3(sub), _f3(div)
    _lib.check(_lib_().vtp_images_to_u8(_p(img_nchw), _p(u8_nhwc), B, H, W, a, d, _s()), "vtp_images_to_u8")


def latent_channel_stats(latents, sums):
    B, C = latents.shape[:2]
    hw = latents[0, 0].numel()
    _lib.check(_lib_().vtp_latent_channel_stats(_p(latents), _p(sums), B, C, hw, _s()), "vtp_latent_channel_stats")


E4M3_MAX = 448.0


def quantize_e4m3(src, dst, scale):
    n = src.numel()
    sd, sf = (scale, 0.0) if isinstance(scale, torch.Tensor) else (None, float(scale))
    _lib.check(_lib_().vtp_quantize_e4m3(_p(src), int(src.dtype == torch.float32), _p(dst), n, _p(sd), sf, _s()), "vtp_quantize_e4m3")


def norm_fwd_e4m3(x, w, b, y8, q_scale, stats, M, D, eps, kind):
    _lib.check(_lib_().vtp_norm_fwd_e4m3(_p(x), _p(w), _p(b), _p(y8), _p(q_scale), _p(stats), M, D, eps, kind, _s()), "vtp_norm_fwd_e4m3")


def amax(src, out):
    _lib.check(_lib_().vtp_amax(_p(src), int(src.dtype == torch.float32), src.numel(), _p(out), _s()), "vtp_amax")


def dequantize_e4m3(src, dst, inv_scale):
    _lib.check(_lib_().vtp_dequantize_e4m3(_p(src), _p(dst), src.numel(), float(inv_scale), _s()), "vtp_dequantize_e4m3")


def gemm_nt_fp8(a8, b8, c, *, M, N, K, alpha, lda=None, ldb=None, ldc=None, c2=None, ldc2=0, bias=None, resid=None, epi=EPI_BF16,
                rope=None):
    lda = K if lda is None else lda
    ldb = K if ldb is None else ldb
    ldc = c.stride(0) if ldc is None else ldc
    rp = (None, None, None, 0) if rope is None else rope
    _lib.check(_lib_().vtp_gemm_nt_fp8(_p(a8), lda, _p(b8), ldb, _p(c), ldc, _p(c2), ldc2, _p(bias), _p(resid), M, N, K, epi, float(alpha),
                                       _p(rp[0]), _p(rp[1]), _p(rp[2]), rp[3], _s()), "vtp_gemm_nt_fp8")
```

vtp_amd/train.py:

```python
from __future__ import annotations

import math
import os
from typing import List, Optional, Sequence, Tuple

import torch

from . import ops
from .engine import BF, F32, OVERLAP


class GradBucketer:

    def __init__(self, flat_g: torch.Tensor, group=None, shard: bool = False, grad_dtype: torch.dtype = torch.float32,
                 force: bool = False):
        import torch.distributed as dist
        self.dist = dist
        self.flat_g = flat_g
        self.group = group
        self.world = dist.get_world_size(group) if dist.is_available() and dist.is_initialized() else 1
        self.rank = dist.get_rank(group) if self.world > 1 else 0
        self.active = self.world > 1 or (bool(force) and dist.is_available() and dist.is_initialized())
        self.works = []
        self.reduced_elems = 0
# ... 14 lines not shown
            rec.chunk = (n + W * 8 - 1) // (W * 8) * 8
            rec.a = min(lo + self.rank * rec.chunk, hi)
            rec.b = min(rec.a + rec.chunk, hi)
            rec.send = torch.zeros(rec.chunk * W, dtype=self.grad_dtype, device=dev)
            rec.g_out = torch.zeros(rec.chunk, dtype=self.grad_dtype, device=dev)
            rec.g32 = rec.g_out if self.grad_dtype == torch.float32 else torch.zeros(rec.chunk, dtype=torch.float32, device=dev)
            rec.p_send = torch.zeros(rec.chunk, dtype=torch.float32, device=dev)
            rec.p_recv = torch.zeros(rec.chunk * W, dtype=torch.float32, device=dev)
            self.shards[(lo, hi)] = rec
        return rec

    def native(self) -> bool:
        return self.dist.get_backend(self.group) == "nccl"

    def reduce_scatter_range(self, lo: int, hi: int):
        rec = self._rec(lo, hi)
        n = hi - lo
        direct = self.grad_dtype == torch.float32 and n == rec.chunk * self.world and self.native()
        if direct:
            src = self.flat_g[lo:hi]
        elif self.grad_dtype == torch.float32:
            rec.send[:n].copy_(self.flat_g[lo:hi])
            src = rec.send
        else:
            ops.cast_f32_bf16(self.flat_g[lo:hi], rec.send, n)
            src = rec.send
        if self.native():
            w = self.dist.reduce_scatter_tensor(rec.g_out, src, op=self.dist.ReduceOp.SUM, group=self.group, async_op=True)
            self.works.append((w, None))
        else:
            tmp = rec.send.float()
            w = self.dist.all_reduce(tmp, op=self.dist.ReduceOp.SUM, group=self.group, async_op=True)
            self.works.append((w, lambda: rec.g_out.copy_(tmp[self.rank * rec.chunk:(self.rank + 1) * rec.chunk])))
        self.reduced_elems += n
        self.comm_bytes += n * rec.send.element_size()

    def reduce_range(self, lo: int, hi: int):
        if not self.active or hi <= lo:
            return
        if self.shard:
            return self.reduce_scatter_range(lo, hi)
        w = self.dist.all_reduce(self.flat_g[lo:hi], op=self.dist.ReduceOp.SUM, group=self.group, async_op=True)
        self.works.append((w, None))
        self.reduced_elems += hi - lo
        self.comm_bytes += (hi - lo) * 4

    def wait(self, works=None):
        mine = works is None
        for w, after in (self.works if mine else works):
            w.wait()
            if after is not None:
                after()
        if mine:
            self.works = []

    def all_gather_params(self, flat_p: torch.Tensor, recs):
        works = []
        for rec in recs:
            if self.native():
                works.append((self.dist.all_gather_into_tensor(rec.p_recv, rec.p_send, group=self.group, async_op=True), None))
            else:
                rec.p_recv.zero_()
                rec.p_recv[self.rank * rec.chunk:(self.rank + 1) * rec.chunk].copy_(rec.p_send)
                works.append((self.dist.all_reduce(rec.p_recv, group=self.group, async_op=True), None))
            self.comm_bytes += rec.p_recv.numel() * 4
        for w, _ in works:
            w.wait()


class HostStager:

    def __init__(self, device, slots: int = 4):
        self.device, self.n, self.i = device, slots, 0
        self.host = [None] * slots
        self.events = [None] * slots
        self.wait_s = 0.0

    def upload(self, arrays: dict) -> dict:
        import numpy as np
        plan, off = [], 0
        for k, a in arrays.items():
            a = np.ascontiguousarray(a)
            plan.append((k, a, off))
            off += (a.nbytes + 15) // 16 * 16
        total = max(off, 16)
        slot = self.i
        self.i = (self.i + 1) % self.n
        if self.events[slot] is not None:
            import time
            t0 = time.perf_counter()
            self.events[slot].synchronize()
            self.wait_s += time.perf_counter() - t0
        if self.host[slot] is None or self.host[slot].numel() < total:
            self.host[slot] = torch.empty(max(total * 2, 1 << 16), dtype=torch.uint8).pin_memory()
        h = self.host[slot]
        hn = h.numpy()
        for k, a, o in plan:
            hn[o:o + a.nbytes] = a.view(np.uint8).reshape(-1)
        d = torch.empty(total, dtype=torch.uint8, device=self.device)
        d.copy_(h[:total], non_blocking=True)
        ev = torch.cuda.Event()
        ev.record()
        self.events[slot] = ev
        out = {}
        for k, a, o in plan:
            t = d[o:o + a.nbytes]
            out[k] = t.view(_NP2TORCH[a.dtype.name]).view(a.shape)
        out["_packed"] = (d, tuple((k, o, a.nbytes, a.dtype.name, tuple(a.shape)) for k, a, o in plan))
        return out


_NP2TORCH = {"int32": torch.int32, "float32": torch.float32, "uint8": torch.uint8, "int64": torch.int64}


def merge_ranges(ranges: Sequence[Tuple[int, int]]) -> List[Tuple[int, int]]:
    out: List[Tuple[int, int]] = []
    for lo, hi in sorted(ranges):
        if out and lo <= out[-1][1]:
            out[-1] = (out[-1][0], max(out[-1][1], hi))
        else:
            out.append((lo, hi))
    return out


def uncovered(lo: int, hi: int, covered: Sequence[Tuple[int, int]]) -> List[Tuple[int, int]]:
    out, x = [], lo
    for a, b in covered:
        if b <= x or a >= hi:
            continue
        if a > x:
            out.append((x, a))
        x = max(x, b)
    if x < hi:
        out.append((x, hi))
    return out


def param_ranges(offsets, prefixes: Sequence[str]) -> List[Tuple[int, int]]:
    r = []
    for name, (o, k) in offsets.items():
        if any(name.startswith(p) for p in prefixes):
            r.append((o, o + (k + 3) // 4 * 4))
    return merge_ranges(r)


def lane_pieces(ranges: Sequence[Tuple[int, int]], pairs: Sequence[Tuple[int, int, int]]) -> List[Tuple[int, int, Optional[int]]]:
    pieces = []
    for lo, hi in ranges:
        cuts = sorted({lo, hi} | {x for _, slo, shi in pairs for x in (slo, shi) if lo < x < hi})
        for a, b in zip(cuts, cuts[1:]):
            tl = next((tlo + (a - slo) for tlo, slo, shi in pairs if slo <= a and b <= shi), None)
            pieces.append((a, b, tl))
    return pieces


NO_DECAY_NAMES = ("logit_scale", "logit_bias", "cls_token", "mask_token", "positional_embedding", "storage_tokens")


def default_no_decay(name: str, shape: tuple) -> bool:
    return len(shape) < 2 or name.rsplit(".", 1)[-1] in NO_DECAY_NAMES


def _max_norm_value(value) -> float:
    try:
        f = float(value)
    except (TypeError, ValueError):
        f = None
    if f is None or isinstance(value, bool) or not f > 0:
        raise ValueError(f"max_grad_norm must be None or a number > 0 (float('inf') allowed), got {value!r}")
    return f


def _skip_nonfinite_value(value, max_grad_norm) -> bool:
    if not isinstance(value, bool):
        raise ValueError(f"skip_nonfinite must be True or False, got {value!r}")
    if value and max_grad_norm is None:
        raise ValueError("skip_nonfinite=True needs max_grad_norm to be a number: the decision is taken on the global gradient norm "
                         "(max_grad_norm=float('inf') measures it without clipping)")
    return value


MAX_PARAM_GROUPS = 128


def _group_scale(group: dict, key: str) -> float:
    value = group.get(key, 1.0)
    try:
        f = float(value)
    except (TypeError, ValueError):
        f = float("nan")
    if isinstance(value, bool) or not (math.isfinite(f) and f >= 0):
        raise ValueError(f"param group {group.get('name')!r}: {key} must be a finite number >= 0, got {value!r}")
    return f


def resolve_param_groups(param_groups, shapes: dict, no_decay=None):
    user = []
    for g in param_groups:
        if not isinstance(g, dict) or "name" not in g or "match" not in g:
            raise ValueError(f"a param group is a dict with 'name' and 'match', got {g!r}")
        unknown = set(g) - {"name", "match", "lr_scale", "wd_scale"}
        if unknown:
            raise ValueError(f"param group {g['name']!r}: unknown keys {sorted(unknown)}")
        match = g["match"]
        if isinstance(match, str):
            match = (match,)
        if not callable(match):
            match = tuple(match)
            if not match or not all(isinstance(x, str) for x in match):
                raise ValueError(f"param group {g['name']!r}: match must be a tuple of name prefixes or a callable (name, shape) -> bool")
        user.append(({"name": str(g["name"]), "lr_scale": _group_scale(g, "lr_scale"), "wd_scale": _group_scale(g, "wd_scale")}, match))
    names = [g["name"] for g, _ in user]
    dup = sorted({n for n in names if names.count(n) > 1})
    if dup:
        raise ValueError(f"duplicate param group names: {dup}")
    if len(user) > MAX_PARAM_GROUPS:
        raise ValueError(f"{len(user)} param groups: at most {MAX_PARAM_GROUPS} are supported")
    rows, hit, rest = {}, [False] * len(user), False
    for name, shape in shapes.items():
        shape = tuple(shape)
        gi = next((i for i, (_, match) in enumerate(user)
                   if (match(name, shape) if callable(match) else name.startswith(match))), len(user))
        if gi < len(user):
            hit[gi] = True
        else:
            rest = True
        rows[name] = 2 * gi + (1 if no_decay is not None and no_decay(name, shape) else 0)
    empty = [g["name"] for (g, _), h in zip(user, hit) if not h]
    if empty:
        raise ValueError(f"param groups that match no parameter: {empty}")
    groups = [g for g, _ in user]
    if rest:
        if "default" in names:
            raise ValueError("duplicate param group names: ['default'] (the implicit group of the unmatched parameters)")
        if len(groups) == MAX_PARAM_GROUPS:
            raise ValueError(f"{MAX_PARAM_GROUPS} param groups and unmatched parameters: the implicit 'default' group would be one too many")
        groups.append({"name": "default", "lr_scale": 1.0, "wd_scale": 1.0})
    return groups, rows


def group_table(groups) -> List[float]:
    vals = []
    for g in groups:
        ls, ws = _group_scale(g, "lr_scale"), _group_scale(g, "wd_scale")
        vals += [ls, ws, ls, 0.0]
    return vals


_LAYER0 = ("cls_token", "mask_token", "storage_tokens", "register_tokens", "pos_embed", "positional_embedding", "rope_embed.")


def layerwise_lr_decay(names, depth: int, decay: float, patch_embed_lr_mult: float = 1.0, prefix: str = "trunk."):
    import re
    by_scale: dict = {}
    for name in names:
        if not name.startswith(prefix):
            continue
        local = name[len(prefix):]
        blk = re.match(r"blocks\.(\d+)\.", local)
        patch = local.startswith("patch_embed.")
        if patch or local.startswith(_LAYER0):
            layer = 0
        elif blk:
            layer = int(blk.group(1)) + 1
        else:
            layer = depth + 1
        scale = decay ** (depth + 1 - layer)
        if patch:
            scale *= patch_embed_lr_mult
        label = f"layer{layer}" + (".patch_embed" if patch else "")
        labels, members = by_scale.setdefault(scale, ([], set()))
        if label not in labels:
            labels.append(label)
        members.add(name)
    return [{"name": prefix + "+".join(labels), "match": (lambda name, shape, members=frozenset(members): name in members),
             "lr_scale": scale, "wd_scale": 1.0} for scale, (labels, members) in by_scale.items()]


CLIP_PREFIXES = ("visual_proj.", "text_transformer.", "token_embedding.", "positional_embedding", "ln_final.",
                 "text_projection", "logit_scale", "logit_bias")


class VTPTrainer:

    def __init__(self, model, lr: float = 1e-4, betas=(0.9, 0.95), eps: float = 1e-8, weight_decay: float = 0.05,
                 group=None, bucket_blocks: int = 3, use_graphs: bool = False, clip_weight: float = 1.0,
                 rec_weight: float = 1.0, dino_weight: float = 1.0, ibot_weight: float = 1.0, student_temp: float = 0.1,
                 teacher_temp: float = 0.07, center_momentum: float = 0.9, teacher_momentum: float = 0.994,
                 lpips=None, perceptual_weight: float = 0.0, drop_rate: float = 0.0, decoder_drop_rate: float = 0.0,
                 clip_drop_rate: Optional[float] = None, ssl_drop_rate: Optional[float] = None, rec_drop_rate: Optional[float] = None,
                 drop_seed: int = 0, centering: str = "softmax", koleo_weight: float = 0.0, sk_iterations: int = 3,
                 shard_optimizer: Optional[bool] = None, grad_dtype: str = "fp32", no_decay="default",
                 force_collectives: bool = False, max_grad_norm: Optional[float] = None, param_groups=None,
                 skip_nonfinite: bool = False):
        self._skip = _skip_nonfinite_value(skip_nonfinite, max_grad_norm)
        self.model = model
        self.drop_rate, self.decoder_drop_rate = float(drop_rate), float(decoder_drop_rate)
        self.clip_drop_rate = self.drop_rate if clip_drop_rate is None else float(clip_drop_rate)
        self.ssl_drop_rate = self.drop_rate if ssl_drop_rate is None else float(ssl_drop_rate)
        self.rec_drop_rate = self.drop_rate if rec_drop_rate is None else float(rec_drop_rate)
        self._drop_gen = torch.Generator().manual_seed(int(drop_seed))
        if centering not in ("softmax", "sinkhorn_knopp"):
            raise ValueError(f"centering must be 'softmax' or 'sinkhorn_knopp', got {centering!r}")
        self.centering, self.koleo_weight, self.sk_iterations = centering, float(koleo_weight), int(sk_iterations)
        self.koleo_loss_sum = None
        self.lpips, self.perceptual_weight = lpips, float(perceptual_weight)
        if self.perceptual_weight > 0 and lpips is None:
            raise ValueError("perceptual_weight > 0 needs an LPIPS module")
        self.lpips_val = None
        self._text_stream = None
        self.store = model._engine()
        self.trunk, self.decoder = model._trunk, model._decoder
        self.text, self.clip = model._text, model._clip
        if self.decoder is None:
            raise RuntimeError("VTPTrainer needs train_reconstruction=True")
        self.lr, self.betas, self.eps, self.wd = lr, betas, eps, weight_decay
        self._skip_betas = (float(betas[0]), float(betas[1]))
        self.clip_weight, self.rec_weight = clip_weight, rec_weight
        self.dino_weight, self.ibot_weight = dino_weight, ibot_weight
        self.student_temp, self.teacher_temp = student_temp, teacher_temp
        self.center_momentum, self.teacher_momentum = center_momentum, teacher_momentum
        self.ssl_head = getattr(model, "_head", None)
        st = self.store
        self.ranges_rec = param_ranges(st.offsets, ("trunk.", "pixel_decoder."))
        self.ranges_all = param_ranges(st.offsets, ("trunk.", "pixel_decoder.") + CLIP_PREFIXES)
        self.ranges_ssl = param_ranges(st.offsets, ("dino_head.",))
        if self.ssl_head is not None:
            K = self.ssl_head.K
            self.center_dino = torch.zeros(K, dtype=F32, device=st.device)
            self.center_ibot = torch.zeros(K, dtype=F32, device=st.device)
            self.center_stats = torch.zeros(2 * K + 8, dtype=F32, device=st.device)
            self.ssl_loss_sum = torch.zeros(1, dtype=F32, device=st.device)
            self.koleo_loss_sum = torch.zeros(1, dtype=F32, device=st.device)
        self._ssl_static = {}
        self._stager = None
        self.ssl_bucket = int(os.environ.get("VTP_SSL_BUCKET", "512"))
        self.m = torch.zeros_like(st.flat_p)
        self.v = torch.zeros_like(st.flat_p)
        if no_decay == "default":
            no_decay = default_no_decay
        self.nodecay4 = None
        if no_decay is not None:
            flags = torch.zeros(st.numel // 4, dtype=torch.uint8)
            for name, (o, k) in st.offsets.items():
                if no_decay(name, tuple(st.params[name].shape)):
                    flags[o // 4:(o + (k + 3) // 4 * 4) // 4] = 1
            self.nodecay4 = flags.to(st.device)
        self.param_groups = self.group_tab = self._group4 = self._group_ring = None
        if param_groups is not None:
            shapes = {name: tuple(st.params[name].shape) for name in st.offsets}
            self.param_groups, rows = resolve_param_groups(param_groups, shapes, no_decay)
            idx = torch.zeros(st.numel // 4, dtype=torch.uint8)
            for name, (o, k) in st.offsets.items():
                idx[o // 4:(o + (k + 3) // 4 * 4) // 4] = rows[name]
            self._group4 = idx.to(st.device)
            self.group_tab = torch.tensor(group_table(self.param_groups), dtype=F32, device=st.device).view(-1, 2)
        self.step_no = 0
        self.loss_sum = torch.zeros(1, dtype=F32, device=st.device)
        self.clip_loss_sum = torch.zeros(1, dtype=F32, device=st.device)
        if shard_optimizer is None:
            shard_optimizer = os.environ.get("VTP_SHARD_OPT", "0") == "1"
        if grad_dtype not in ("fp32", "bf16"):
            raise ValueError(f"grad_dtype must be 'fp32' or 'bf16', got {grad_dtype!r}")
        if grad_dtype == "bf16" and not shard_optimizer:
            raise ValueError("grad_dtype='bf16' needs shard_optimizer=True (the all-reduce path reduces the flat fp32 buffer in place)")
        self.bucketer = GradBucketer(st.flat_g, group, shard=shard_optimizer, grad_dtype=BF if grad_dtype == "bf16" else F32,
                                     force=force_collectives)
        self.shard_optimizer = self.bucketer.shard
        self._shard_layout = None
        self.overlap_opt = (not self.shard_optimizer) and os.environ.get("VTP_OPT_OVERLAP", "1") not in ("0", "false", "off")
        self._opt_stream = self._zero_stream = None
        self._opt_plans = {}
        self._opt_busy = self._zero_busy = False
        self.head_overlap = os.environ.get("VTP_HEAD_OVERLAP", "1") not in ("0", "false", "off")
        self._head_stream, self._head_keys = None, []
        self._works_prev = []
        self.collectives = self.bucketer.active
        if self.collectives:
            from . import _lib
            _lib.load().vtp_set_gemm_dynamic(1)
        self.time_comm = False
        self._comm_events = []
        self.world, self.rank, self.group = self.bucketer.world, self.bucketer.rank, group
        for eng in self._aug_engines():
            eng.rope_aug.reseed(drop_seed, self.rank)
        self._graph_aug = {}
        self.bucket_blocks = bucket_blocks
        self._bucket_plan = self._plan_buckets()
        self.hyper = torch.zeros(16, dtype=F32, device=st.device)
        self.momentum_dev = self.hyper[9:10]
        self._clip = max_grad_norm is not None
        self._max_grad_norm = _max_norm_value(max_grad_norm) if self._clip else None
        self.grad_norm = self.grad_clip_coef = self._clip_partials = self._clip_sum = None
        self._clip_ranges, self._clip_cursor, self._clip_keys = {}, 0, []
        if self._clip:
            self.grad_norm = torch.zeros(1, dtype=F32, device=st.device)
            self.grad_clip_coef = torch.zeros(1, dtype=F32, device=st.device)
            cap = ops.sumsq_partials_count(st.numel) + len(st.offsets)
            self._clip_partials = torch.zeros(cap, dtype=torch.float64, device=st.device)
            self._clip_sum = torch.zeros(1, dtype=torch.float64, device=st.device)
        self._skip_state = self.step_skipped = self.skipped_steps = None
        if self._skip:
            self._skip_state = torch.zeros(4, dtype=torch.int32, device=st.device)
            self.skipped_steps = self._skip_state[1:2]
            self.step_skipped = self._skip_state[2:3]
        self._hyper_ring = None
        self.use_graphs = use_graphs
        self._graphs = {}
        self.single_graph = (not self.collectives) and os.environ.get("VTP_SINGLE_GRAPH", "1") in ("1", "true", "on")
        if self.text is not None and model.config.text_pool_type == "none":
            self._clip_unsupported = "the contrastive objective needs pooled text features (text_pool_type argmax | first | last)"
        elif self.text is not None and model.config.vision_clip_feat == "pooled" and model.config.vision_embed_dim > 1024:
            self._clip_unsupported = (f"vision_clip_feat='pooled' needs vision_embed_dim <= 1024 on the fused step "
                                      f"(got {model.config.vision_embed_dim}); the autograd path (model(...); loss.backward()) has no limit")
        else:
            self._clip_unsupported = None
        self.sync_replicas()

    @property
    def max_grad_norm(self) -> Optional[float]:
        return self._max_grad_norm

    @max_grad_norm.setter
    def max_grad_norm(self, value):
        if (value is None) != (self._max_grad_norm is None):
            raise ValueError("max_grad_norm: clipping cannot be switched on or off after construction; build the trainer with "
                             "max_grad_norm=None or with a number")
        self._max_grad_norm = None if value is None else _max_norm_value(value)

    @property
    def skip_nonfinite(self) -> bool:
        return self._skip

    def sync_replicas(self):
        if not self.collectives:
            return
        dist, st = self.bucketer.dist, self.store
        bufs = [st.flat_p, self.m, self.v]
        if self._skip:
            bufs.append(self._skip_state)
        if self.ssl_head is not None:
            bufs += [self.center_dino, self.center_ibot]
        for b in bufs:
            dist.broadcast(b, src=dist.get_global_rank(self.group, 0) if self.group is not None else 0, group=self.group)
        st.prep()
        self.model._pver = self.model._param_version()

    def _plan_buckets(self):
        off = self.store.offsets

        def rng(*prefixes):
            return param_ranges(off, prefixes)

        plan = {"dec_tail": rng("pixel_decoder.norm.", "pixel_decoder.proj_out."),
                "dec_head": rng("pixel_decoder.proj_in."),
                "trunk_tail": rng("trunk.norm.", "trunk.feature_bottleneck."),
                "trunk_head": rng("trunk.cls_token", "trunk.mask_token", "trunk.patch_embed."),
                "text_tail": rng("ln_final.", "text_projection"),
                "text_head": rng("token_embedding.", "positional_embedding"),
                "clip_head": rng("visual_proj.", "logit_scale", "logit_bias"), "dino_head": rng("dino_head.")}
        towers = [("dec", "pixel_decoder.blocks.", self.decoder.depth), ("trunk", "trunk.blocks.", self.trunk.depth)]
        if self.text is not None:
            towers.append(("text", "text_transformer.resblocks.", self.text.depth))
        for key, prefix, depth in towers:
            for i in range(depth):
                plan[f"{key}.{i}"] = rng(f"{prefix}{i}.")
        return plan

    def _reduce(self, keys: Sequence[str]):
        if not self.collectives or not keys:
            return
        rs = merge_ranges([r for k in keys for r in self._bucket_plan[k]])
        for lo, hi in rs:
            self.bucketer.reduce_range(lo, hi)

    def _tower_backward(self, tower: str, gen, depth: int):
        nb = self.bucket_blocks
        result = None
        try:
            while True:
                ev = next(gen)
                if ev == "tail":
                    yield [f"{tower}_tail"]
                elif ev[0] == "block" and ev[1] % nb == 0:
                    i = ev[1]
                    yield [f"{tower}.{j}" for j in range(i, min(i + nb, depth))]
        except StopIteration as stop:
            result = stop.value
        return result

    def _ssl_gen(self, P, lead_images=None):
        from .vtp import ssl_forward
        out = ssl_forward(self.model, P["global"], P["local"], P["masks"], P["plan"], P["dev"], train=True, lead_images=lead_images)
        self._zero_join()
        if not (self.head_overlap and not self.collectives and OVERLAP.enabled):
            yield from self._ssl_tail(out, P)
            return out
        main = torch.cuda.current_stream()
        self.trunk.d_xnf_buffer(out["ctx"]).zero_()
        if self._head_stream is None:
            self._head_stream = torch.cuda.Stream()
        self._head_stream.wait_stream(main)
        with torch.cuda.stream(self._head_stream), OVERLAP.lane(2):
            was, OVERLAP.enabled = OVERLAP.enabled, False
            try:
                for ev in self._ssl_tail(out, P, zero_dxnf=False):
                    if callable(ev):
                        raise RuntimeError("head stream: the SSL tail asked for a collective")
                    self._head_keys += ev
            finally:
                OVERLAP.enabled = was
        return out

    def _ssl_tail(self, out, P, zero_dxnf: bool = True):
        model, st, head = self.model, self.store, self.ssl_head
        dist = self.bucketer.dist
        K, D = head.K, self.trunk.D
        Tt, Ts, Tm, B2, nl = out["Tt"], out["Ts"], out["Tm"], out["B2"], out["nl"]
        ws = out["ws"]
        t_logits, s_logits = out["teacher_logits"], out["student_logits"]
        probs = ws.get("probs", (Tt, K), BF)
        if self.centering == "sinkhorn_knopp":
            yield from self._sinkhorn_targets(ws, t_logits, probs, P, B2, Tm, K)
        else:
            inv_tt = self.hyper[8:9]
            ops.softmax_center(t_logits, self.center_dino, inv_tt, probs, B2, K)
            ops.softmax_center(t_logits[B2:], self.center_ibot, inv_tt, probs[B2:], Tm, K)
            stats = self.center_stats
            stats.zero_()
            ops.colsum_bf16(t_logits, K, stats, B2, K)
            ops.colsum_bf16_rows(t_logits[B2:], K, stats[K:], P["dev"]["n_masked_i"], Tm, K)
            stats[2 * K:2 * K + 1].copy_(P["dev"]["n_masked_f"])

            def apply_centers():
                ops.center_ema(self.center_dino, stats, 1.0 / (B2 * self.world), self.center_momentum, K)
                ops.center_ema(self.center_ibot, stats[K:], 0.0, self.center_momentum, K, count=stats[2 * K:])
            if self.collectives:
                yield lambda: self.bucketer.works.append((dist.all_reduce(stats, group=self.group, async_op=True), None))
                self._deferred.append(apply_centers)
            else:
                apply_centers()
        d_logits = ws.get("d_logits", (Ts, K), BF)
        ops.dino_ce(s_logits, probs, P["dev"]["t0"], P["dev"]["t1"], P["dev"]["w"], 1.0 / self.student_temp, self.ssl_loss_sum,
                    d_logits, Ts, K)
        dX = head.backward(d_logits, out["head_ctx"])
        if self.koleo_weight > 0:
            self._koleo(ws, out["Hs"], dX, nl, B2, head.Din)
        yield ["dino_head"]
        from .vtp import ssl_head_input_bwd
        dX = ssl_head_input_bwd(model, out, dX)
        ctx = out["ctx"]
        d_xnf = self.trunk.d_xnf_buffer(ctx)
        if zero_dxnf:
            d_xnf.zero_()
        seg_g, seg_l = ctx.segs[-2], ctx.segs[-1]
        ops.scatter_token_rows(dX, P["dev"]["student_local_src"], d_xnf[seg_l.row0:], nl, D)
        ops.scatter_token_rows(dX[nl:], P["dev"]["student_global_src"], d_xnf[seg_g.row0:], Ts - nl, D)

    def _sinkhorn_targets(self, ws, t_logits, probs, P, B2, Tm, K):
        dist = self.bucketer.dist
        it = self.sk_iterations
        inv_t = 1.0 / self.teacher_temp
        for tag, lg, pr, T, cnt_dev, rows_dev, count in (("cls", t_logits, probs, B2, None, None, float(B2 * self.world)),
                                                         ("patch", t_logits[B2:], probs[B2:], Tm, P["dev"]["n_masked_f"],
                                                          P["dev"]["n_masked_i"], 0.0)):
            u, v = ws.get(f"sk.u.{tag}", (T,), F32), ws.get(f"sk.v.{tag}", (K,), F32)
            scr = ws.get(f"sk.s.{tag}", (8 + K + T,), F32)
            if not self.collectives:
                ops.sinkhorn_knopp(lg, inv_t, pr, u, v, scr, T, K, count, it, -1, cnt_dev, rows_dev)
                continue
            if cnt_dev is not None:
                gcnt = ws.get("sk.cnt", (1,), F32)
                gcnt.copy_(cnt_dev)
                yield lambda gcnt=gcnt: dist.all_reduce(gcnt, group=self.group)
                cnt_dev = gcnt
            ops.sinkhorn_knopp(lg, inv_t, pr, u, v, scr, T, K, count, 0, 0, cnt_dev, rows_dev)
            yield lambda scr=scr: dist.all_reduce(scr[:1], op=dist.ReduceOp.MAX, group=self.group)
            for i in range(it):
                ops.sinkhorn_knopp(lg, inv_t, pr, u, v, scr, T, K, count, i, 1, cnt_dev, rows_dev)
                yield lambda scr=scr: dist.all_reduce(scr[8:8 + K], group=self.group)
                ops.sinkhorn_knopp(lg, inv_t, pr, u, v, scr, T, K, count, i, 2, cnt_dev, rows_dev)
            ops.sinkhorn_knopp(lg, inv_t, pr, u, v, scr, T, K, count, it, 3, cnt_dev, rows_dev)

    def _koleo(self, ws, Xs, dX, nl, B2, D):
        B = B2 // 2
        self.koleo_loss_sum.zero_()
        x32 = ws.get("kl.x", (B2, D), F32)
        x32.copy_(Xs[nl:nl + B2])
        xn, inv = ws.get("kl.xn", (B2, D), F32), ws.get("kl.inv", (B2,), F32)
        ops.l2norm_fwd(x32, xn, inv, B2, D, 1e-8)
        d_xn = ws.get("kl.dxn", (B2, D), F32)
        d_xn.zero_()
        nn = ws.get("kl.nn", (B2,), torch.int32)
        for v in range(2):
            ops.koleo(xn[v * B:], nn[v * B:], d_xn[v * B:], self.koleo_loss_sum, B, D, self.koleo_weight / B)
        dx = ws.get("kl.dx", (B2, D), F32)
        ops.l2norm_bwd(d_xn, xn, inv, dx, B2, D)
        dxb = ws.get("kl.dxb", (B2, D), BF)
        dxb.copy_(dx)
        dX[nl:nl + B2].add_(dxb)

    def prepare_ssl(self, global_crops: torch.Tensor, local_crops: torch.Tensor, masks, pad_to: Optional[int] = None,
                    upperbound: Optional[int] = None) -> dict:
        from .ssl_engine import build_ssl_indices
        from .vtp import plan_to_device
        import numpy as np
        B = global_crops.shape[0] // 2
        hw = (global_crops.shape[-2] // 16) * (global_crops.shape[-1] // 16)
        hw_l = (local_crops.shape[-2] // 16) * (local_crops.shape[-1] // 16)
        n_local = local_crops.shape[0] // B
        m = masks.detach().cpu().numpy().astype(bool) if torch.is_tensor(masks) else np.asarray(masks, bool)
        plan = build_ssl_indices(m, B, hw, n_local, hw_l, self.dino_weight, self.ibot_weight,
                                 pad_to=int(pad_to or self.ssl_bucket), upperbound=upperbound)
        if self._stager is None:
            self._stager = HostStager(self.store.device)
        arrays = {k: plan[k].astype(np.int32, copy=False) for k in ("teacher_src", "student_local_src", "student_global_src", "t0", "t1")}
        arrays["w"] = plan["w"].astype(np.float32, copy=False)
        arrays["n_masked_i"] = np.array([plan["n_masked"]], np.int32)
        arrays["n_masked_f"] = np.array([float(plan["n_masked"])], np.float32)
        arrays["masks"] = m.astype(np.uint8)
        up = self._stager.upload(arrays)
        masks_dev = up.pop("masks")
        packed = up.pop("_packed")
        return dict(**{"global": global_crops, "local": local_crops}, masks=masks_dev, plan=plan, dev=up, packed=packed)

    def _step_gen(self, images: torch.Tensor, text: Optional[torch.Tensor], ssl: Optional[dict] = None, rec_images=None):
        self._reduced_ranges = []
        self._head_keys = []
        self._opt_queue, self._opt_done, self._hooks_done = [], [], set()
        self._clip_cursor, self._clip_keys = 0, []
        del OVERLAP._deferred[:]
        del self.trunk.bott_wgrads[:]
        self._opt_ema = ssl is not None
        lag = 2 if self.collectives else 1
        lazy_join = not self.collectives and (self.single_graph or not self.use_graphs)
        stacks = [e.stack for e in (self.trunk, self.decoder, getattr(self, "text", None)) if e is not None and hasattr(e, "stack")]
        if os.environ.get("VTP_WGRAD_OVERWRITE", "1") not in ("0", "false", "off"):
            for sk in stacks:
                sk.wgrad_overwrite = True
        try:
            for ev in self._step_body(images, text, ssl, rec_images):
                if not lazy_join or callable(ev) or "FINAL" in ev:
                    self._opt_join()
                if callable(ev):
                    yield ev
                    continue
                keys = [k for k in ev if k != "FINAL"]
                self._reduced_ranges += merge_ranges([r for k in keys for r in self._bucket_plan[k]])
                yield ev
                if self.overlap_opt and "FINAL" not in ev:
                    self._opt_queue.append(keys)
                    while len(self._opt_queue) >= lag:
                        self._opt_launch(self._opt_queue.pop(0))
                elif self.overlap_opt:
                    self._opt_queue.append(keys)
        finally:
            for sk in stacks:
                sk.wgrad_overwrite = False

    def _opt_plan(self, keys, ema: bool):
        ck = (tuple(keys), ema)
        plan = self._opt_plans.get(ck)
        if plan is None:
            st = self.store
            rs = merge_ranges([r for k in keys for r in self._bucket_plan[k]])
            pairs = []
            if ema:
                from .vtp import _range
                for t_pref, s_pref in self.model.ema_pairs():
                    (tlo, thi), (slo, shi) = _range(st, t_pref), _range(st, s_pref)
                    assert thi - tlo == shi - slo
                    pairs.append((tlo, slo, shi))
            pieces = lane_pieces(rs, pairs)
            runs = st.desc_runs(rs) + st.desc_runs([(tl, tl + b - a) for a, b, tl in pieces if tl is not None])
            plan = self._opt_plans[ck] = (pieces, runs)
        return plan

    def _opt_update(self, keys):
        st = self.store
        pieces, runs = self._opt_plan(keys, self._opt_ema)
        tab = self.group_tab
        for a, b, tl in pieces:
            teacher = None if tl is None else st.flat_p[tl:tl + b - a]
            if self._skip:
                idx4 = self._group4 if tab is not None else self.nodecay4
                ops.adamw_ema_dev_guarded(st.flat_p[a:b], st.flat_g[a:b], self.m[a:b], self.v[a:b], teacher, b - a, self.hyper,
                                          self.step_skipped, None if idx4 is None else idx4[a // 4:b // 4], tab,
                                          0 if tab is None else tab.shape[0])
            elif tab is not None:
                ops.adamw_ema_dev_grouped(st.flat_p[a:b], st.flat_g[a:b], self.m[a:b], self.v[a:b], teacher, b - a, self.hyper,
                                          self._group4[a // 4:b // 4], tab, tab.shape[0])
            else:
                ops.adamw_ema_dev(st.flat_p[a:b], st.flat_g[a:b], self.m[a:b], self.v[a:b], teacher,
                                  b - a, self.hyper, None if self.nodecay4 is None else self.nodecay4[a // 4:b // 4])
        st.prep_runs(runs)
        touched = [(a, b) for a, b, _ in pieces] + [(tl, tl + b - a) for a, b, tl in pieces if tl is not None]
        for hook, deps in getattr(st, "hook_deps", {}).items():
            if hook not in self._hooks_done and all(any(a <= lo and hi <= b for a, b in touched) for lo, hi in deps):
                hook()
                self._hooks_done.add(hook)
        self._opt_done += [(a, b) for a, b, _ in pieces]

    def _adamw(self, lo, hi, g):
        st, tab = self.store, self.group_tab
        if self._skip:
            idx4 = self._group4 if tab is not None else self.nodecay4
            ops.adamw_dev_guarded(st.flat_p[lo:hi], g, self.m[lo:hi], self.v[lo:hi], None, hi - lo, self.hyper, self.step_skipped,
                                  None if idx4 is None else idx4[lo // 4:hi // 4], tab, 0 if tab is None else tab.shape[0])
        elif tab is not None:
            ops.adamw_dev_grouped(st.flat_p[lo:hi], g, self.m[lo:hi], self.v[lo:hi], None, hi - lo, self.hyper,
                                  self._group4[lo // 4:hi // 4], tab, tab.shape[0])
        else:
            ops.adamw_dev(st.flat_p[lo:hi], g, self.m[lo:hi], self.v[lo:hi], None, hi - lo, self.hyper,
                          None if self.nodecay4 is None else self.nodecay4[lo // 4:hi // 4])

    def _opt_launch(self, keys):
        if not keys:
            return
        if self._clip:
            self._clip_keys.append(keys)
            plan = self._clip_plan(self._clip_views(keys))
            work = lambda: self._clip_sumsq(plan)
        else:
            work = lambda: self._opt_update(keys)
        if not OVERLAP.enabled:
            return work()
        main = torch.cuda.current_stream()
        if self._opt_stream is None:
            self._opt_stream = torch.cuda.Stream()
        OVERLAP.run_deferred()
        self._opt_stream.wait_stream(main)

        def issue():
            with torch.cuda.stream(self._opt_stream):
                work()
        OVERLAP.defer(issue)
        self._opt_busy = True

    def _clip_views(self, keys):
        rs = self._clip_ranges.get(tuple(keys))
        if rs is None:
            rs = self._clip_ranges[tuple(keys)] = merge_ranges([r for k in keys for r in self._bucket_plan[k]])
        return [(self.store.flat_g[lo:hi], hi - lo) for lo, hi in rs]

    def _clip_plan(self, views):
        plan = []
        for g, n in views:
            plan.append((g, n, self._clip_cursor))
            self._clip_cursor += ops.sumsq_partials_count(n)
        if self._clip_cursor > self._clip_partials.numel():
            raise RuntimeError(f"gradient clipping: {self._clip_cursor} partials exceed the buffer ({self._clip_partials.numel()})")
        return plan

    def _clip_sumsq(self, plan):
        for g, n, base in plan:
            ops.sumsq_partials(g, n, self._clip_partials[base:])

    def _clip_finalize(self, partials=None, count=None):
        if partials is None:
            partials, count = self._clip_partials, self._clip_cursor
        if self._skip:
            ops.grad_clip_finalize_guarded(partials, count, self.hyper, self.grad_norm, self.grad_clip_coef, self._skip_state,
                                           self._skip_betas)
        else:
            ops.grad_clip_finalize(partials, count, self.hyper, self.grad_norm, self.grad_clip_coef)

    def _ema(self, t, s, n):
        if self._skip:
            ops.ema_dev_guarded(t, s, n, self.momentum_dev, self.step_skipped)
        else:
            ops.ema_dev(t, s, n, self.momentum_dev)

    def _clip_shards(self, recs):
        views = []
        for rec in recs:
            n = rec.b - rec.a
            if n > 0:
                if rec.g32 is not rec.g_out:
                    rec.g32.copy_(rec.g_out)
                views.append((rec.g32, n))
        if views:
            self._clip_sumsq(self._clip_plan(views))
            ops.sum_partials(self._clip_partials, self._clip_cursor, self._clip_sum)
        else:
            self._clip_sum.zero_()
        dist, total = self.bucketer.dist, self._clip_sum
        yield lambda: dist.all_reduce(total, group=self.group)
        self._clip_finalize(total, 1)

    def _opt_join(self):
        OVERLAP.run_deferred()
        if self._opt_busy:
            torch.cuda.current_stream().wait_stream(self._opt_stream)
            self._opt_busy = False

    def _zero_grads_async(self):
        if not (self.overlap_opt and OVERLAP.enabled):
            self.store.zero_grad()
            return
        main = torch.cuda.current_stream()
        if self._zero_stream is None:
            self._zero_stream = torch.cuda.Stream()
        self._zero_stream.wait_stream(main)
        with torch.cuda.stream(self._zero_stream):
            self.store.zero_grad()
        self._zero_busy = True

    def _zero_join(self):
        if self._zero_busy:
            torch.cuda.current_stream().wait_stream(self._zero_stream)
            self._zero_busy = False

    def _separate_rec(self, images, text, rec_images) -> bool:
        return text is not None and (rec_images is not None and rec_images is not images or self.clip_drop_rate != self.rec_drop_rate)

    def _step_body(self, images: torch.Tensor, text: Optional[torch.Tensor], ssl: Optional[dict] = None, rec_images=None):
        st = self.store
        dist = self.bucketer.dist
        sep = self._separate_rec(images, text, rec_images)
        rec_img = images if rec_images is None else rec_images
        leads = [images, rec_img] if sep else [rec_img]
        rec_seg = 1 if sep else 0
        Bc, Nc = images.shape[0], (images.shape[2] // 16) * (images.shape[3] // 16) + 1
        B, _, H, W = rec_img.shape
        h, w = H // 16, W // 16
        N = h * w + 1
        self._zero_grads_async()
        self.loss_sum.zero_()
        self.clip_loss_sum.zero_()
        self._deferred = []
        if ssl is not None:
            self.ssl_loss_sum.zero_()
            xnf_all = (yield from self._ssl_gen(ssl, lead_images=leads))["xnf"]
        else:
            xnf_all = self.trunk.forward_list([(im, None) for im in leads], train=True)
            self._zero_join()
        xnf = xnf_all[:Bc * Nc]
        par_text = text is not None and OVERLAP.enabled
        par_fwd = par_bwd = par_text
        main = torch.cuda.current_stream()
        if par_text:
            if self._text_stream is None:
                self._text_stream = torch.cuda.Stream()
            T = self._text_stream
        if par_fwd:
            T.wait_stream(main)
            with torch.cuda.stream(T), OVERLAP.lane(1):
                f_txt = self.text.forward(text, train=True)
        lat = self.trunk.latents(seg=rec_seg)
        t = self.decoder.forward(lat, B, h, w, train=True)
        dt = self.decoder._ctx[0].get("b.dt", (B * h * w, 768), BF)
        ops.l1_loss_fwd_bwd(t, rec_img, dt, self.loss_sum, B, h, w, self.rec_weight / (B * 3 * H * W))
        if self.perceptual_weight > 0:
            self.lpips_val = self.lpips.loss_and_grad(t, rec_img, dt, self.perceptual_weight, B, H, W)
        held = None
        pvec = None
        if text is not None:
            d_xnf = self.trunk.d_xnf_buffer()[:Bc * Nc]
            cw = self.clip.ws
            Dt = self.clip.Dt
            f_img = self.clip.image_features(xnf, Bc, Nc)
            img_n, inv_i = self.clip.normalize(f_img, "img")
            if par_fwd:
                main.wait_stream(T)
            else:
                f_txt = self.text.forward(text, train=True)
            txt_n, inv_t = self.clip.normalize(f_txt, "txt")
            Bg = Bc * self.world
            if self.collectives:
                img_all = cw.get("img_all", (Bg, Dt), F32)
                txt_all = cw.get("txt_all", (Bg, Dt), F32)

                def gather():
                    works = [self._all_gather_rows(img_all, img_n, async_op=True), self._all_gather_rows(txt_all, txt_n, async_op=True)]
                    for wk in works:
                        if wk is not None:
                            wk.wait()
                yield gather
            else:
                img_all, txt_all = img_n, txt_n
            d_img_l = cw.get("d_img_l", (Bc, Dt), F32)
            d_txt_l = cw.get("d_txt_l", (Bc, Dt), F32)
            d_img_all = cw.get("d_img_all", (Bg, Dt), F32)
            d_txt_all = cw.get("d_txt_all", (Bg, Dt), F32)
            scratch = cw.get("logits", (2 * Bc * Bg,), F32)
            if st.has("logit_bias"):
                ops.siglip_loss(img_n, txt_all, st.p("logit_scale"), st.p("logit_bias"), Bc, Bg, Dt, self.rank * Bc, self.clip_loss_sum,
                                d_img_l, d_txt_all, st.g("logit_scale"), st.g("logit_bias"), scratch)
                d_txt_l.zero_()
                d_img_all.zero_()
            else:
                ops.clip_loss(img_n, txt_n, img_all, txt_all, st.p("logit_scale"), Bc, Bg, Dt, self.rank * Bc, self.clip_loss_sum,
                              d_img_l, d_txt_l, d_img_all, d_txt_all, st.g("logit_scale"), scratch)
            if self.collectives:
                rs_i = cw.get("rs_i", (Bc, Dt), F32)
                rs_t = cw.get("rs_t", (Bc, Dt), F32)

                def scatter():
                    works = [self._reduce_scatter_rows(rs_i, d_img_all, async_op=True), self._reduce_scatter_rows(rs_t, d_txt_all, async_op=True)]
                    for wk in works:
                        if wk is not None:
                            wk.wait()
                yield scatter
            else:
                rs_i, rs_t = d_img_all, d_txt_all
            ops.reduce_slabs(rs_i, Bc * Dt, 1, d_img_l, Bc * Dt, accumulate=True)
            ops.reduce_slabs(rs_t, Bc * Dt, 1, d_txt_l, Bc * Dt, accumulate=True)
            if self.clip_weight != 1.0:
                d_img_l.mul_(self.clip_weight)
                d_txt_l.mul_(self.clip_weight)
                st.g("logit_scale").mul_(self.clip_weight)
                if st.has("logit_bias"):
                    st.g("logit_bias").mul_(self.clip_weight)
            d_f_txt = self.clip.normalize_bwd(d_txt_l, txt_n, inv_t, "txt")
            if par_bwd:
                T.wait_stream(main)
                held = []
                with torch.cuda.stream(T), OVERLAP.lane(1):
                    was, OVERLAP.enabled = OVERLAP.enabled, False
                    try:
                        for ev in self._tower_backward("text", self.text.backward(d_f_txt), self.text.depth):
                            held += ev
                    finally:
                        OVERLAP.enabled = was
                held.append("text_head")
            else:
                yield from self._tower_backward("text", self.text.backward(d_f_txt), self.text.depth)
                yield ["text_head"]
            d_f_img = self.clip.normalize_bwd(d_img_l, img_n, inv_i, "img")
            pvec = self.clip.image_backward(d_f_img, xnf, d_xnf, Bc, Nc)
            OVERLAP.join()
            if held is not None:
                held.append("clip_head")
            else:
                yield ["clip_head"]
        def join_head():
            if not self._head_keys:
                return []
            main.wait_stream(self._head_stream)
            keys, self._head_keys = self._head_keys, []
            return keys

        dec_gen = self._tower_backward("dec", self.decoder.backward(dt), self.decoder.depth)
        d_lat = None
        while True:
            try:
                ev = next(dec_gen)
            except StopIteration as stop:
                d_lat = stop.value
                break
            if held is not None:
                held += ev
                continue
            yield join_head() + ev
        keys = join_head()
        if held is not None:
            held += keys
        elif keys:
# ... 381 lines not shown
```

Measured before the change: 722.9.

## Fuse AdamW update with bf16 weight prep and narrow step-start gradient zeroing

Adds a tiled kernel that applies AdamW (and EMA teacher) updates and writes the bf16 weight copies and transposes in one pass. This replaces separate flat optimizer launches followed by prep_weights launches, so parameters are read and written once instead of twice. It also learns which gradient ranges are fully overwritten by weight-gradient GEMMs and zeroes only the remaining segments at step start. The cost is extra planning logic, and the fill plan raises an error if the overwritten ranges change between steps.

```diff
diff --git a/include/vtp_hip.h b/include/vtp_hip.h
--- a/include/vtp_hip.h
+++ b/include/vtp_hip.h
@@ -120,6 +120,12 @@
 int vtp_adamw_ema_dev_guarded(float* p, const float* g, float* m, float* v, float* teacher, const void* idx4, const float* group_tab,
                               int ngroups, long n, const float* hyper, const int* skip, void* stream);
 int vtp_ema_dev_guarded(float* t, const float* s, long n, const float* momentum, const int* skip, void* stream);
+int vtp_zero_segs(const void* segs, int n, int n_blocks, float* base, void* stream);
+int vtp_adamw_ema_segs(const void* segs, int n, int n_blocks, float* flat_p, const float* flat_g, float* flat_m, float* flat_v,
+                       const void* idx4, const float* group_tab, int ngroups, const float* hyper, const int* skip, void* stream);
+int vtp_adamw_prep_tiles(const void* descs, const void* plan, int n, int tile_rows, int n_tiles, const void* table, float* flat_p,
+                         const float* flat_g, float* flat_m, float* flat_v, const void* idx4, const float* group_tab, int ngroups,
+                         const float* hyper, const int* skip, void* stream);
 
 int vtp_embed_tokens(const long* ids, const float* table, const float* pos, float* x, int* eot, int B, int T, int D,
                      void* stream);
diff --git a/vtp_amd/_lib.py b/vtp_amd/_lib.py
--- a/vtp_amd/_lib.py
+++ b/vtp_amd/_lib.py
@@ -94,6 +94,9 @@
     "vtp_adamw_dev_guarded": [_P, _P, _P, _P, _P, _P, _P, _I, _L, _P, _P, _P],
     "vtp_adamw_ema_dev_guarded": [_P, _P, _P, _P, _P, _P, _P, _I, _L, _P, _P, _P],
     "vtp_ema_dev_guarded": [_P, _P, _L, _P, _P, _P],
+    "vtp_zero_segs": [_P, _I, _I, _P, _P],
+    "vtp_adamw_ema_segs": [_P, _I, _I, _P, _P, _P, _P, _P, _P, _I, _P, _P, _P],
+    "vtp_adamw_prep_tiles": [_P, _P, _I, _I, _I, _P, _P, _P, _P, _P, _P, _P, _I, _P, _P, _P],
     "vtp_embed_tokens": [_P, _P, _P, _P, _P, _I, _I, _I, _P],
     "vtp_embed_tokens_bwd": [_P, _P, _P, _P, _I, _I, _I, _P],
     "vtp_gather_rows": [_P, _P, _P, _I, _I, _I, _P],
diff --git a/vtp_amd/csrc/elementwise.hip b/vtp_amd/csrc/elementwise.hip
--- a/vtp_amd/csrc/elementwise.hip
+++ b/vtp_amd/csrc/elementwise.hip
@@ -255,16 +255,21 @@
   long tile_start;
 };
 
-__global__ __launch_bounds__(256) void prep_weights_kernel(const PrepDesc* __restrict__ descs, int n, int tile_base) {
-  __shared__ float tile[64][65];
-  const long tile_id = (long)blockIdx.x + tile_base;
+__device__ __forceinline__ int prep_desc_of(const PrepDesc* __restrict__ descs, int n, long tile_id) {
   int lo = 0, hi = n - 1;
   while (lo < hi) {
     const int mid = (lo + hi + 1) >> 1;
     if (descs[mid].tile_start <= tile_id) lo = mid; else hi = mid - 1;
   }
-  const PrepDesc d = descs[lo];
-  const int t = (int)(tile_id - d.tile_start);
+  return lo;
+}
+
+__device__ __forceinline__ bool prep_fast_path(const PrepDesc d) {
+  const bool aligned = ((((uintptr_t)d.src | (uintptr_t)d.src2) & 15) | (((uintptr_t)d.dst | (uintptr_t)d.dstT) & 7)) == 0;
+  return (d.C & 3) == 0 && (d.R & 3) == 0 && aligned;
+}
+
+__device__ __forceinline__ void prep_tile(const PrepDesc d, int t, float (*tile)[65]) {
   const int R = (int)d.R, C = (int)d.C;
   if (d.mode == 2) {
     const int g = t * 256 + threadIdx.x;
@@ -278,8 +283,7 @@
   const int r0 = (t / tiles_c) * 64, c0 = (t % tiles_c) * 64;
   bf16* dst = (bf16*)d.dst;
   bf16* dstT = (bf16*)d.dstT;
-  const bool aligned = ((((uintptr_t)d.src | (uintptr_t)d.src2) & 15) | (((uintptr_t)dst | (uintptr_t)dstT) & 7)) == 0;
-  if ((C & 3) == 0 && (R & 3) == 0 && aligned) {
+  if (prep_fast_path(d)) {
     const int q = threadIdx.x & 15, rr = threadIdx.x >> 4;
 #pragma unroll
     for (int pass = 0; pass < 4; ++pass) {
@@ -329,6 +333,13 @@
   __syncthreads();
   for (int c = ty; c < 64; c += 4)
     if (c0 + c < C && r0 + tx < R) dstT[(size_t)(c0 + c) * R + r0 + tx] = f2bf(tile[tx][c]);
+}
+
+__global__ __launch_bounds__(256) void prep_weights_kernel(const PrepDesc* __restrict__ descs, int n, int tile_base) {
+  __shared__ float tile[64][65];
+  const long tile_id = (long)blockIdx.x + tile_base;
+  const PrepDesc d = descs[prep_desc_of(descs, n, tile_id)];
+  prep_tile(d, (int)(tile_id - d.tile_start), tile);
 }
 
 __global__ __launch_bounds__(256) void swiglu_bwd_kernel(const bf16* __restrict__ dh, const bf16* __restrict__ x12,
@@ -482,16 +493,13 @@
 }
 
 template <bool TABLE>
-__global__ __launch_bounds__(256) void adamw_ema_kernel(float* __restrict__ p, const float* __restrict__ g, float* __restrict__ m,
-                                                        float* __restrict__ v, float* __restrict__ t, long n4,
-                                                        const float* __restrict__ hyper, const uint8_t* __restrict__ idx4,
-                                                        const float2* __restrict__ group_tab, int ngroups,
-                                                        const int* __restrict__ skip) {
-  __shared__ float2 tab[TABLE ? 256 : 1];
-  if (skip && *skip) return;
+__device__ __forceinline__ void adamw_ema_block(float* __restrict__ p, const float* __restrict__ g, float* __restrict__ m,
+                                                float* __restrict__ v, float* __restrict__ t, long n4, long block,
+                                                const float* __restrict__ hyper, const uint8_t* __restrict__ idx4,
+                                                const float2* __restrict__ group_tab, int ngroups, float2* tab) {
   const float lr = hyper[0], b1 = hyper[1], b2 = hyper[2], eps = hyper[3], wd = hyper[4], bc1 = hyper[5], bc2_sqrt = hyper[6], gs = hyper[7];
   const float mom = hyper[9];
-  const long base = blockIdx.x * 1024L + threadIdx.x;
+  const long base = block * 1024L + threadIdx.x;
   float2 row = make_float2(1.f, 1.f);
   if constexpr (TABLE)
     if ((int)threadIdx.x < ngroups) row = group_tab[threadIdx.x];
@@ -539,6 +547,191 @@
     *(f32x4*)(m + 4 * i) = mv[u];
     *(f32x4*)(v + 4 * i) = vv[u];
     if (t) *(f32x4*)(t + 4 * i) = tv[u] * mom + pv[u] * (1.f - mom);
+  }
+}
+
+template <bool TABLE>
+__global__ __launch_bounds__(256) void adamw_ema_kernel(float* __restrict__ p, const float* __restrict__ g, float* __restrict__ m,
+                                                        float* __restrict__ v, float* __restrict__ t, long n4,
+                                                        const float* __restrict__ hyper, const uint8_t* __restrict__ idx4,
+                                                        const float2* __restrict__ group_tab, int ngroups,
+                                                        const int* __restrict__ skip) {
+  __shared__ float2 tab[TABLE ? 256 : 1];
+  if (skip && *skip) return;
+  adamw_ema_block<TABLE>(p, g, m, v, t, n4, blockIdx.x, hyper, idx4, group_tab, ngroups, tab);
+}
+
+struct OptSeg {
+  long lo, n4;
+  long tlo;
+  long block0;
+};
+
+template <bool TABLE>
+__global__ __launch_bounds__(256) void adamw_segs_kernel(const OptSeg* __restrict__ segs, int n, float* __restrict__ fp,
+                                                         const float* __restrict__ fg, float* __restrict__ fm, float* __restrict__ fv,
+                                                         const float* __restrict__ hyper, const uint8_t* __restrict__ idx4,
+                                                         const float2* __restrict__ group_tab, int ngroups,
+                                                         const int* __restrict__ skip) {
+  __shared__ float2 tab[TABLE ? 256 : 1];
+  if (skip && *skip) return;
+  int lo = 0, hi = n - 1;
+  while (lo < hi) {
+    const int mid = (lo + hi + 1) >> 1;
+    if (segs[mid].block0 <= (long)blockIdx.x) lo = mid; else hi = mid - 1;
+  }
+  const OptSeg s = segs[lo];
+  adamw_ema_block<TABLE>(fp + s.lo, fg + s.lo, fm + s.lo, fv + s.lo, s.tlo >= 0 ? fp + s.tlo : nullptr, s.n4, blockIdx.x - s.block0,
+                         hyper, idx4 ? idx4 + s.lo / 4 : nullptr, group_tab, ngroups, tab);
+}
+
+__global__ __launch_bounds__(256) void zero_segs_kernel(const OptSeg* __restrict__ segs, int n, float* __restrict__ base) {
+  int lo = 0, hi = n - 1;
+  while (lo < hi) {
+    const int mid = (lo + hi + 1) >> 1;
+    if (segs[mid].block0 <= (long)blockIdx.x) lo = mid; else hi = mid - 1;
+  }
+  const OptSeg s = segs[lo];
+  const long first = ((long)blockIdx.x - s.block0) * 1024L + threadIdx.x;
+#pragma unroll
+  for (int u = 0; u < 4; ++u) {
+    const long i = first + u * 256;
+    if (i < s.n4) *(f32x4*)(base + s.lo + 4 * i) = (f32x4){0.f, 0.f, 0.f, 0.f};
+  }
+}
+
+template <bool TABLE, int TR, int TC>
+__global__ __launch_bounds__(256) void adamw_prep_tile_kernel(const PrepDesc* __restrict__ descs, const int4* __restrict__ plan, int n,
+                                                              const PrepDesc* __restrict__ table,
+                                                              float* __restrict__ fp, const float* __restrict__ fg,
+                                                              float* __restrict__ fm, float* __restrict__ fv,
+                                                              const float* __restrict__ hyper, const uint8_t* __restrict__ idx4,
+                                                              const float2* __restrict__ group_tab, int ngroups,
+                                                              const int* __restrict__ skip) {
+  static_assert(TR * TC == 4096 && TR % 4 == 0 && TC % 4 == 0 && TR * (TC + 1) <= 64 * 65, "one float4 per thread and pass, four passes");
+  constexpr int QC = TC / 4, RP = 256 / QC;
+  constexpr int QR = TR / 4, CP = 256 / QR;
+  __shared__ float lds[64 * 65];
+  __shared__ float2 tab[TABLE ? 256 : 1];
+  if (skip && *skip) return;
+  int di = 0, hi = n - 1;
+  while (di < hi) {
+    const int mid = (di + hi + 1) >> 1;
+    if (plan[mid].z <= (int)blockIdx.x) di = mid; else hi = mid - 1;
+  }
+  const PrepDesc d = descs[di];
+  const int4 pl = plan[di];
+  const int tl = (int)blockIdx.x - pl.z;
+  const bool has_t = pl.y >= 0;
+  const PrepDesc td = table[has_t ? pl.y : 0];
+  if (!pl.x || d.mode == 2 || !prep_fast_path(d) || (has_t && !prep_fast_path(td))) {
+    if (pl.x) return;
+    prep_tile(d, tl, (float (*)[65])lds);
+    if (has_t) {
+      __syncthreads();
+      prep_tile(td, tl, (float (*)[65])lds);
+    }
+    return;
+  }
+  float (*tile)[TC + 1] = (float (*)[TC + 1])lds;
+  const float lr = hyper[0], b1 = hyper[1], b2 = hyper[2], eps = hyper[3], wd = hyper[4], bc1 = hyper[5], bc2_sqrt = hyper[6], gs = hyper[7];
+  const float mom = hyper[9];
+  float2 row = make_float2(1.f, 1.f);
+  if constexpr (TABLE)
+    if ((int)threadIdx.x < ngroups) row = group_tab[threadIdx.x];
+  const int R = (int)d.R, C = (int)d.C;
+  const int tiles_c = (C + TC - 1) / TC;
+  const int r0 = (tl / tiles_c) * TR, c0 = (tl % tiles_c) * TC;
+  const int q = threadIdx.x % QC, rr = threadIdx.x / QC;
+  const bool okc = c0 + 4 * q < C;
+  const int c = min(c0 + 4 * q, C - 4);
+  f32x4 pv[4], gv[4], mv[4], vv[4], tv[4];
+  long so[4];
+  const long t_off = has_t ? td.src - d.src : 0;
+  int fl[4] = {0, 0, 0, 0};
+  bool ok[4];
+#pragma unroll
+  for (int u = 0; u < 4; ++u) {
+    const int g = r0 + u * RP + rr, gc = min(g, R - 1);
+    ok[u] = g < R && okc;
+    const bool second = d.mode == 1 && (gc & 8);
+    const long j = d.mode == 1 ? (gc >> 4) * 8 + (gc & 7) : gc;
+    so[u] = ((second ? d.src2 : d.src) - fp) + j * C + c;
+    pv[u] = *(const f32x4*)(fp + so[u]);
+    gv[u] = *(const f32x4*)(fg + so[u]);
+    mv[u] = *(const f32x4*)(fm + so[u]);
+    vv[u] = *(const f32x4*)(fv + so[u]);
+  }
+  if (has_t) {
+#pragma unroll
+    for (int u = 0; u < 4; ++u) tv[u] = *(const f32x4*)(fp + so[u] + t_off);
+  }
+  if (idx4) {
+#pragma unroll
+    for (int u = 0; u < 4; ++u) fl[u] = idx4[so[u] >> 2];
+  }
+  if constexpr (TABLE) {
+    if ((int)threadIdx.x < ngroups) tab[threadIdx.x] = fold_group_row(row, lr, wd, bc1);
+    __syncthreads();
+  }
+#pragma unroll
+  for (int u = 0; u < 4; ++u) {
+    float keep, step;
+    if constexpr (TABLE) {
+      const float2 rw = tab[min(fl[u], ngroups - 1)];
+      keep = rw.x, step = rw.y;
+    } else {
+      keep = fl[u] ? 1.f : 1.f - lr * wd, step = lr / bc1;
+    }
+#pragma unroll
+    for (int e = 0; e < 4; ++e) {
+      const float gg = gv[u][e] * gs;
+      pv[u][e] *= keep;
+      mv[u][e] = b1 * mv[u][e] + (1.f - b1) * gg;
+      vv[u][e] = b2 * vv[u][e] + (1.f - b2) * gg * gg;
+      const float denom = sqrtf(vv[u][e]) / bc2_sqrt + eps;
+      pv[u][e] -= step * (mv[u][e] / denom);
+    }
+    if (has_t) tv[u] = tv[u] * mom + pv[u] * (1.f - mom);
+  }
+  bf16* dst = (bf16*)d.dst;
+#pragma unroll
+  for (int u = 0; u < 4; ++u) {
+    const int r = u * RP + rr;
+    if (ok[u]) {
+      *(f32x4*)(fp + so[u]) = pv[u];
+      *(f32x4*)(fm + so[u]) = mv[u];
+      *(f32x4*)(fv + so[u]) = vv[u];
+      if (has_t) *(f32x4*)(fp + so[u] + t_off) = tv[u];
+      if (dst) *(bf16x4*)(dst + (size_t)(r0 + r) * C + c) = __builtin_convertvector(pv[u], bf16x4);
+    }
+#pragma unroll
+    for (int e = 0; e < 4; ++e) tile[r][4 * q + e] = pv[u][e];
+  }
+  const int qT = threadIdx.x % QR, cT = threadIdx.x / QR;
+  for (int who = 0; who < (has_t ? 2 : 1); ++who) {
+    bf16* dT = (bf16*)(who ? td.dstT : d.dstT);
+    if (who) {
+      bf16* tdst = (bf16*)td.dst;
+      __syncthreads();
+#pragma unroll
+      for (int u = 0; u < 4; ++u) {
+        const int r = u * RP + rr;
+        if (ok[u] && tdst) *(bf16x4*)(tdst + (size_t)(r0 + r) * C + c) = __builtin_convertvector(tv[u], bf16x4);
+#pragma unroll
+        for (int e = 0; e < 4; ++e) tile[r][4 * q + e] = tv[u][e];
+      }
+    }
+    if (!dT) continue;
+    __syncthreads();
+#pragma unroll
+    for (int pass = 0; pass < 4; ++pass) {
+      const int cc = pass * CP + cT, r = 4 * qT;
+      if (c0 + cc < C && r0 + r < R) {
+        const f32x4 o = {tile[r][cc], tile[r + 1][cc], tile[r + 2][cc], tile[r + 3][cc]};
+        *(bf16x4*)(dT + (size_t)(c0 + cc) * R + r0 + r) = __builtin_convertvector(o, bf16x4);
+      }
+    }
   }
 }
 
@@ -910,3 +1103,49 @@
   hipLaunchKernelGGL(ema_kernel, dim3(grid_for(n / 4)), dim3(256), 0, (hipStream_t)stream, t, s, n, 0.f, momentum, skip);
   return check_launch("ema_dev_guarded");
 }
+
+extern "C" int vtp_adamw_ema_segs(const void* segs, int n, int n_blocks, float* flat_p, const float* flat_g, float* flat_m,
+                                  float* flat_v, const void* idx4, const float* group_tab, int ngroups, const float* hyper,
+                                  const int* skip, void* stream) {
+  VTP_REQUIRE(segs && n > 0 && n_blocks > 0 && flat_p && flat_g && flat_m && flat_v && hyper, "vtp_adamw_ema_segs: bad argument");
+  VTP_REQUIRE((((uintptr_t)flat_p | (uintptr_t)flat_g | (uintptr_t)flat_m | (uintptr_t)flat_v) & 15) == 0,
+              "vtp_adamw_ema_segs: the flat buffers must be 16-byte aligned");
+  if (group_tab) {
+    VTP_REQUIRE(idx4 && ngroups >= 1 && ngroups <= 256, "vtp_adamw_ema_segs: bad group table (1 <= ngroups <= 256)");
+    hipLaunchKernelGGL(adamw_segs_kernel<true>, dim3(n_blocks), dim3(256), 0, (hipStream_t)stream, (const OptSeg*)segs, n, flat_p, flat_g,
+                       flat_m, flat_v, hyper, (const uint8_t*)idx4, (const float2*)group_tab, ngroups, skip);
+  } else {
+    hipLaunchKernelGGL(adamw_segs_kernel<false>, dim3(n_blocks), dim3(256), 0, (hipStream_t)stream, (const OptSeg*)segs, n, flat_p, flat_g,
+                       flat_m, flat_v, hyper, (const uint8_t*)idx4, (const float2*)nullptr, 0, skip);
+  }
+  return check_launch("adamw_ema_segs");
+}
+
+extern "C" int vtp_adamw_prep_tiles(const void* descs, const void* plan, int n, int tile_rows, int n_tiles, const void* table,
+                                    float* flat_p, const float* flat_g, float* flat_m, float* flat_v, const void* idx4,
+                                    const float* group_tab, int ngroups, const float* hyper, const int* skip, void* stream) {
+  VTP_REQUIRE(descs && plan && table && n > 0 && n_tiles > 0, "vtp_adamw_prep_tiles: bad argument");
+  VTP_REQUIRE(tile_rows == 64 || tile_rows == 32, "vtp_adamw_prep_tiles: tile_rows must be 32 (32 x 128 tiles) or 64 (64 x 64)");
+  VTP_REQUIRE(flat_p && flat_g && flat_m && flat_v && hyper, "vtp_adamw_prep_tiles: null buffer");
+  VTP_REQUIRE((((uintptr_t)flat_p | (uintptr_t)flat_g | (uintptr_t)flat_m | (uintptr_t)flat_v) & 15) == 0,
+              "vtp_adamw_prep_tiles: the flat buffers must be 16-byte aligned");
+  VTP_REQUIRE(!group_tab || (idx4 && ngroups >= 1 && ngroups <= 256), "vtp_adamw_prep_tiles: bad group table (1 <= ngroups <= 256)");
+#define VTP_TILES(TABLE, TR, TC)                                                                                                       \
+  hipLaunchKernelGGL((adamw_prep_tile_kernel<TABLE, TR, TC>), dim3(n_tiles), dim3(256), 0, (hipStream_t)stream, (const PrepDesc*)descs, \
+                     (const int4*)plan, n, (const PrepDesc*)table, flat_p, flat_g, flat_m, flat_v, hyper, (const uint8_t*)idx4,         \
+                     (const float2*)group_tab, group_tab ? ngroups : 0, skip)
+  if (group_tab) {
+    if (tile_rows == 64) VTP_TILES(true, 64, 64); else VTP_TILES(true, 32, 128);
+  } else {
+    if (tile_rows == 64) VTP_TILES(false, 64, 64); else VTP_TILES(false, 32, 128);
+  }
+#undef VTP_TILES
+  return check_launch("adamw_prep_tiles");
+}
+
+extern "C" int vtp_zero_segs(const void* segs, int n, int n_blocks, float* base, void* stream) {
+  VTP_REQUIRE(segs && base && n > 0 && n_blocks > 0, "vtp_zero_segs: bad argument");
+  VTP_REQUIRE(((uintptr_t)base & 15) == 0, "vtp_zero_segs: base must be 16-byte aligned");
+  hipLaunchKernelGGL(zero_segs_kernel, dim3(n_blocks), dim3(256), 0, (hipStream_t)stream, (const OptSeg*)segs, n, base);
+  return check_launch("zero_segs");
+}
diff --git a/vtp_amd/engine.py b/vtp_amd/engine.py
--- a/vtp_amd/engine.py
+++ b/vtp_amd/engine.py
@@ -31,6 +31,9 @@
             out.append(n)
             seen.add(n)
     return out
+
+
+OPT_TILE_ROWS = int(os.environ.get("VTP_OPT_TILE_ROWS", "32"))
 
 
 class ParamStore:
@@ -118,10 +121,16 @@
         rows, tiles = [], 0
         self._desc_src = []
 
+        self._desc_host = []
+        base = self.flat_p.data_ptr()
+
         def add(src, src2, dst, dstT, R, C, mode, name):
             nonlocal tiles
             rows.append([src, src2, dst, dstT, R, C, mode, tiles])
             self._desc_src.append(self.offsets[name][0])
+            fusable = mode in (0, 1) and R % 4 == 0 and C % 4 == 0 and (src | src2) % 16 == 0 and (dst | dstT) % 8 == 0 \
+                and base % 16 == 0 and (mode == 0 or (R % 16 == 0 and src2 == src + (R // 2) * C * 4))
+            self._desc_host.append((self.offsets[name][0], R, C, mode, fusable))
             tiles += (R + 255) // 256 if mode == 2 else ((R + 63) // 64) * ((C + 63) // 64)
 
         for d in self._descs:
@@ -162,6 +171,34 @@
     def prep_runs(self, runs):
         for d0, d1 in runs:
             ops.prep_weights_range(self._desc_dev[d0:], d1 - d0, self._desc_tile0[d0], self._desc_tile0[d1] - self._desc_tile0[d0])
+
+    def opt_tables(self, plan):
+        segs, blocks = [], 0
+        for lo, hi, tl in plan["segs"]:
+            segs.append([lo, (hi - lo) // 4, -1 if tl is None else tl, blocks])
+            blocks += ((hi - lo) // 4 + 1023) // 1024
+        tr = OPT_TILE_ROWS
+        tc = 4096 // tr
+        runs = []
+        for d0, d1, rows in plan["runs"]:
+            out, tiles = [], 0
+            for i, (fused, ti) in zip(range(d0, d1), rows):
+                out.append([fused, ti, tiles, 0])
+                _, R, C, _, _ = self._desc_host[i]
+                tiles += -(-R // tr) * -(-C // tc) if fused else self._desc_tile0[i + 1] - self._desc_tile0[i]
+            runs.append((d0, d1, torch.tensor(out, dtype=torch.int32, device=self.device), tiles))
+        return {"segs": torch.tensor(segs, dtype=torch.int64, device=self.device) if segs else None, "nsegs": len(segs), "blocks": blocks,
+                "runs": runs, "tile_rows": tr, "refresh": plan["refresh"]}
+
+    def opt_runs(self, tables, m, v, hyper, idx4, group_tab, skip):
+        ng = 0 if group_tab is None else group_tab.shape[0]
+        if tables["nsegs"]:
+            ops.adamw_ema_segs(tables["segs"], tables["nsegs"], tables["blocks"], self.flat_p, self.flat_g, m, v, hyper, idx4, group_tab,
+                               ng, skip)
+        for d0, d1, rows, tiles in tables["runs"]:
+            ops.adamw_prep_tiles(self._desc_dev[d0:], rows, d1 - d0, tables["tile_rows"], tiles, self._desc_dev, self.flat_p, self.flat_g,
+                                 m, v, hyper, idx4, group_tab, ng, skip)
+        self.prep_runs(tables["refresh"])
 
     def mark_prepped(self, done=()):
         for hook in getattr(self, "prep_hooks", ()):
@@ -411,6 +448,20 @@
         self.qk_norm = any(b.qn_w is not None for b in self.blocks)
         self.drop_plan = None
         self.wgrad_overwrite = False
+        self.overwrote = []
+        self._overwrite_spent = False
+
+    def arm_wgrad_overwrite(self, on: bool):
+        self.wgrad_overwrite, self.overwrote, self._overwrite_spent = bool(on), [], False
+
+    def overwritten_ranges(self):
+        out = []
+        for lo, hi in sorted(self.overwrote):
+            if out and lo <= out[-1][1]:
+                out[-1] = (out[-1][0], max(out[-1][1], hi))
+            else:
+                out.append((lo, hi))
+        return out
 
     def _rope_plan(self, ws: Workspace, segs, prefix_tokens: int, M: int):
         if self.style != "vit" or all(rp is None for _, _, rp in segs) or (2 * self.D) % 128 or self.qk_norm:
@@ -751,6 +802,7 @@
             dmid = ws.get("b.dmid", (M, D), F32)
         grouped = not drop and M >= 256 and all(b.ls1 is None and b.ls2 is None for b in self.blocks) \
             and ops.wgrad_group_fits(M, max(3 * D, 2 * H if self.swiglu else H)) and D % 8 == 0 and H % 8 == 0
+        overwrite = bool(self.wgrad_overwrite) and not self._overwrite_spent
         par = (lambda i: f".{i & 1}") if grouped else (lambda i: "")
         groups = ws.__dict__.setdefault("_wgrad_groups", {})
         scratch = self.__dict__.setdefault("_wgrad_scratch", {})
@@ -802,13 +854,21 @@
                 yield ("block", i)
                 continue
             extra = [dict(pr, dy=dy_b) for pr in extra_last] if (i == 0 and hold_last and extra_last) else []
-            gkey = (i, bool(self.wgrad_overwrite), len(extra))
+            gkey = (i, overwrite, len(extra))
             grp = groups.get(gkey)
             if grp is None:
                 grp = ops.WgradGroup(M)
+                g0 = self.store.flat_g.data_ptr()
+                grp.overwrites = []
                 for pr in probs + extra:
-                    grp.add(pr["dy"], pr["x"], pr["gw"], pr["gb"], pr["N"], pr["K"], pr["swiglu_h"], accumulate=not self.wgrad_overwrite)
+                    grp.add(pr["dy"], pr["x"], pr["gw"], pr["gb"], pr["N"], pr["K"], pr["swiglu_h"], accumulate=not overwrite)
+                    if overwrite:
+                        lo = (pr["gw"].data_ptr() - g0) // 4
+                        grp.overwrites.append((lo, lo + pr["N"] * pr["K"]))
                 groups[gkey] = grp.finalize(self.store.device, scratch)
+            if overwrite:
+                self.overwrote += grp.overwrites
+                self._overwrite_spent = True
             if pending is not None:
                 yield ("block", pending[0])
             pending = (i, grp)
diff --git a/vtp_amd/ops.py b/vtp_amd/ops.py
--- a/vtp_amd/ops.py
+++ b/vtp_amd/ops.py
@@ -498,6 +498,22 @@
     _lib.check(_lib_().vtp_ema_dev_guarded(_p(t), _p(s), n, _p(momentum_dev), _p(skip), _s()), "vtp_ema_dev_guarded")
 
 
+def adamw_ema_segs(segs, n, n_blocks, flat_p, flat_g, flat_m, flat_v, hyper, idx4=None, group_tab=None, ngroups=0, skip=None):
+    _lib.check(_lib_().vtp_adamw_ema_segs(_p(segs), n, n_blocks, _p(flat_p), _p(flat_g), _p(flat_m), _p(flat_v), _p(idx4), _p(group_tab),
+                                          ngroups, _p(hyper), _p(skip), _s()), "vtp_adamw_ema_segs")
+
+
+def zero_segs(segs, n, n_blocks, base):
+    _lib.check(_lib_().vtp_zero_segs(_p(segs), n, n_blocks, _p(base), _s()), "vtp_zero_segs")
+
+
+def adamw_prep_tiles(descs_run, plan, n, tile_rows, n_tiles, table, flat_p, flat_g, flat_m, flat_v, hyper, idx4=None, group_tab=None,
+                     ngroups=0, skip=None):
+    _lib.check(_lib_().vtp_adamw_prep_tiles(_p(descs_run), _p(plan), n, tile_rows, n_tiles, _p(table), _p(flat_p), _p(flat_g), _p(flat_m),
+                                            _p(flat_v), _p(idx4), _p(group_tab), ngroups, _p(hyper), _p(skip), _s()),
+               "vtp_adamw_prep_tiles")
+
+
 def _f3(v):
     import ctypes
     return (ctypes.c_float * 3)(*[float(x) for x in v])
diff --git a/vtp_amd/train.py b/vtp_amd/train.py
--- a/vtp_amd/train.py
+++ b/vtp_amd/train.py
@@ -190,6 +190,67 @@
             tl = next((tlo + (a - slo) for tlo, slo, shi in pairs if slo <= a and b <= shi), None)
             pieces.append((a, b, tl))
     return pieces
+
+
+def bucket_opt_plan(pieces: Sequence[Tuple[int, int, Optional[int]]], recs: Sequence[Tuple[int, int, int, int, bool]]) -> dict:
+    by_off = {r[0]: i for i, r in enumerate(recs)}
+    shared, order = set(), sorted((r[0], r[0] + r[1] * r[2], i) for i, r in enumerate(recs) if r[3] != 2)
+    top = (0, -1)
+    for lo, hi, i in order:
+        if lo < top[0]:
+            shared |= {top[1], i}
+        top = max(top, (hi, i))
+    rows, fused_src, named = {}, [], set()
+    for i, (off, R, C, mode, fusable) in enumerate(recs):
+        piece = next(((a, b, tl) for a, b, tl in pieces if a <= off < b), None)
+        if piece is None:
+            continue
+        a, b, tl = piece
+        ti = -1 if tl is None else by_off.get(tl + (off - a), -1)
+        if ti >= 0 and recs[ti][1:4] != (R, C, mode):
+            ti = -1
+        n = R * C if mode != 2 else 0
+        fused = fusable and i not in shared and off + n <= b and (tl is None or (ti >= 0 and recs[ti][4] and ti not in shared))
+        if fused:
+            fused_src.append((off, off + n))
+        if ti >= 0:
+            named.add(ti)
+        rows[i] = (int(fused), ti)
+    runs = []
+    for i in sorted(rows):
+        if runs and runs[-1][1] == i:
+            runs[-1][1] = i + 1
+            runs[-1][2].append(rows[i])
+        else:
+            runs.append([i, i + 1, [rows[i]]])
+    fused_src = merge_ranges(fused_src)
+    segs = [(x, y, None if tl is None else tl + (x - a)) for a, b, tl in pieces for x, y in uncovered(a, b, fused_src)]
+    t_ranges = [(tl, tl + b - a) for a, b, tl in pieces if tl is not None]
+    left = [i for i, r in enumerate(recs) if i not in named and any(lo <= r[0] < hi for lo, hi in t_ranges)]
+    refresh = []
+    for i in left:
+        if refresh and refresh[-1][1] == i:
+            refresh[-1][1] = i + 1
+        else:
+            refresh.append([i, i + 1])
+    return {"runs": [tuple(r) for r in runs], "segs": segs, "refresh": [tuple(r) for r in refresh]}
+
+
+def fill_plan(numel: int, nograd: Sequence[Tuple[int, int]], overwritten: Sequence[Tuple[int, int]]):
+    skipped = [(max(lo, 0), min(hi, numel)) for lo, hi in merge_ranges(list(nograd) + list(overwritten)) if max(lo, 0) < min(hi, numel)]
+    return uncovered(0, numel, skipped), skipped
+
+
+def wgrad_overwrite_enabled() -> bool:
+    return os.environ.get("VTP_WGRAD_OVERWRITE", "1") not in ("0", "false", "off")
+
+
+def fill_narrow_enabled() -> bool:
+    return wgrad_overwrite_enabled() and os.environ.get("VTP_ZERO_NARROW", "1") not in ("0", "false", "off")
+
+
+def opt_fused_enabled() -> bool:
+    return os.environ.get("VTP_OPT_FUSED", "1") not in ("0", "false", "off")
 
 
 NO_DECAY_NAMES = ("logit_scale", "logit_bias", "cls_token", "mask_token", "positional_embedding", "storage_tokens")
@@ -410,6 +471,7 @@
         self._opt_stream = self._zero_stream = None
         self._opt_plans = {}
         self._opt_busy = self._zero_busy = False
+        self._fill_plans, self._fill_key, self._fill_used = {}, None, None
         self.head_overlap = os.environ.get("VTP_HEAD_OVERLAP", "1") not in ("0", "false", "off")
         self._head_stream, self._head_keys = None, []
         self._works_prev = []
@@ -673,9 +735,13 @@
         lag = 2 if self.collectives else 1
         lazy_join = not self.collectives and (self.single_graph or not self.use_graphs)
         stacks = [e.stack for e in (self.trunk, self.decoder, getattr(self, "text", None)) if e is not None and hasattr(e, "stack")]
-        if os.environ.get("VTP_WGRAD_OVERWRITE", "1") not in ("0", "false", "off"):
-            for sk in stacks:
-                sk.wgrad_overwrite = True
+        for sk in stacks:
+            sk.arm_wgrad_overwrite(wgrad_overwrite_enabled())
+        self._fill_key = (tuple(images.shape), None if text is None else tuple(text.shape),
+                          None if ssl is None else (tuple(ssl["global"].shape), tuple(ssl["local"].shape)),
+                          None if rec_images is None else tuple(rec_images.shape), self._separate_rec(images, text, rec_images),
+                          tuple(sk.drop_plan is not None for sk in stacks)) if fill_narrow_enabled() else None
+        self._fill_used = None
         try:
             for ev in self._step_body(images, text, ssl, rec_images):
                 if not lazy_join or callable(ev) or "FINAL" in ev:
@@ -692,9 +758,10 @@
                         self._opt_launch(self._opt_queue.pop(0))
                 elif self.overlap_opt:
                     self._opt_queue.append(keys)
+            self._fill_learn([r for sk in stacks for r in sk.overwritten_ranges()])
         finally:
             for sk in stacks:
-                sk.wgrad_overwrite = False
+                sk.arm_wgrad_overwrite(False)
 
     def _opt_plan(self, keys, ema: bool):
         ck = (tuple(keys), ema)
@@ -711,14 +778,21 @@
                     pairs.append((tlo, slo, shi))
             pieces = lane_pieces(rs, pairs)
             runs = st.desc_runs(rs) + st.desc_runs([(tl, tl + b - a) for a, b, tl in pieces if tl is not None])
-            plan = self._opt_plans[ck] = (pieces, runs)
+            fused = st.opt_tables(bucket_opt_plan(pieces, st._desc_host)) if opt_fused_enabled() else None
+            plan = self._opt_plans[ck] = (pieces, runs, fused)
         return plan
 
     def _opt_update(self, keys):
         st = self.store
-        pieces, runs = self._opt_plan(keys, self._opt_ema)
+        pieces, runs, fused = self._opt_plan(keys, self._opt_ema)
         tab = self.group_tab
-        for a, b, tl in pieces:
+        if fused is not None:
+            st.opt_runs(fused, self.m, self.v, self.hyper, self._group4 if tab is not None else self.nodecay4, tab,
+                        self.step_skipped if self._skip else None)
+            pieces_flat = ()
+        else:
+            pieces_flat = pieces
+        for a, b, tl in pieces_flat:
             teacher = None if tl is None else st.flat_p[tl:tl + b - a]
             if self._skip:
                 idx4 = self._group4 if tab is not None else self.nodecay4
@@ -731,7 +805,8 @@
             else:
                 ops.adamw_ema_dev(st.flat_p[a:b], st.flat_g[a:b], self.m[a:b], self.v[a:b], teacher,
                                   b - a, self.hyper, None if self.nodecay4 is None else self.nodecay4[a // 4:b // 4])
-        st.prep_runs(runs)
+        if fused is None:
+            st.prep_runs(runs)
         touched = [(a, b) for a, b, _ in pieces] + [(tl, tl + b - a) for a, b, tl in pieces if tl is not None]
         for hook, deps in getattr(st, "hook_deps", {}).items():
             if hook not in self._hooks_done and all(any(a <= lo and hi <= b for a, b in touched) for lo, hi in deps):
@@ -832,16 +907,48 @@
             torch.cuda.current_stream().wait_stream(self._opt_stream)
             self._opt_busy = False
 
+    def fill_plan(self, key=None):
+        plan = self._fill_plans.get(self._fill_key if key is None else key)
+        return None if plan is None else (plan[0], plan[1])
+
+    def _fill_learn(self, overwritten):
+        key = self._fill_key
+        if key is None:
+            return
+        st = self.store
+        if self._fill_used is None:
+            nograd = [(o, o + (k + 3) // 4 * 4) for n, (o, k) in st.offsets.items() if not st.params[n].requires_grad]
+            zeroed, skipped = fill_plan(st.numel, nograd, overwritten)
+            segs, blocks = [], 0
+            for lo, hi in zeroed:
+                segs.append([lo, (hi - lo) // 4, -1, blocks])
+                blocks += ((hi - lo) // 4 + 1023) // 1024
+            table = torch.tensor(segs, dtype=torch.int64, device=st.device) if segs else None
+            self._fill_plans[key] = (zeroed, skipped, table, len(segs), blocks, merge_ranges(overwritten))
+        elif self._fill_used[5] != merge_ranges(overwritten):
+            del self._fill_plans[key]
+            raise RuntimeError("step-start fill: the weight-gradient launches of this step wrote other ranges than the ones its fill left "
+                               f"out ({len(self._fill_used[5])} ranges planned, {len(merge_ranges(overwritten))} written); the gradients of "
+                               "this step are not valid")
+
+    def _zero_grads(self):
+        plan = self._fill_plans.get(self._fill_key) if self._fill_key is not None else None
+        self._fill_used = plan
+        if plan is None:
+            self.store.zero_grad()
+        elif plan[3]:
+            ops.zero_segs(plan[2], plan[3], plan[4], self.store.flat_g)
+
     def _zero_grads_async(self):
         if not (self.overlap_opt and OVERLAP.enabled):
-            self.store.zero_grad()
+            self._zero_grads()
             return
         main = torch.cuda.current_stream()
         if self._zero_stream is None:
             self._zero_stream = torch.cuda.Stream()
         self._zero_stream.wait_stream(main)
         with torch.cuda.stream(self._zero_stream):
-            self.store.zero_grad()
+            self._zero_grads()
         self._zero_busy = True
 
     def _zero_join(self):
```

Measured after the change: 723.2 (median of 3 runs). Within noise of the previous version (+0.1%).
